# liudabao001/JABD-Joint-Attention-Based-Detector-for-small-face-detection

Hardware: AMD Instinct MI355X
Metric: images/sec at 1024x1024 bs32 (1/2/4/8 GPU); boxes/sec NMS (higher is better)
Workload: dtype fp32; 1 GPU; C2: JABD-MobileNetV3 RetinaFace (nets/retinaface_r.py) eval forward, weights_init weights; global_batch=32, image_size=1024, parallelism=replicas x1

## Files before the change

include/jabd.h:

```cpp
#ifndef JABD_H_
#define JABD_H_

#include <stddef.h>
#include <stdint.h>

#ifdef __cplusplus
extern "C" {
#endif

typedef void* jabd_stream_t;

enum {
  JABD_OK = 0,
  JABD_EINVAL = 1,
  JABD_EHIP = 2,
  JABD_EWS = 3,
};

const char* jabd_version(void);
int64_t jabd_abi_struct_size(int32_t which);
int jabd_last_error(char* buf, size_t len);

int jabd_launch_log_reset(void);
int64_t jabd_launch_log_count(void);
// ... 55 lines not shown
                          int64_t num_priors, float threshold, float var0,
                          float var1, float* loc_t, int64_t* conf_t,
                          float* landm_t, void* ws, size_t ws_bytes,
                          jabd_stream_t stream);

int jabd_match_iou_f32(const float* targets, const int64_t* offsets,
                       int64_t batch, int64_t max_gt, const float* priors,
                       int64_t num_priors, float threshold, float var0,
                       float var1, float* loc_t, int64_t* conf_t,
                       float* landm_t, void* ws, size_t ws_bytes,
                       jabd_stream_t stream);

int jabd_letterbox_f32(const float* src, int64_t batch, int ih, int iw,
                       float* dst, int h, int w, float fill,
                       const float* mean3, int nchw, jabd_stream_t stream);

int jabd_correct_boxes_f32(float* rows, int64_t n, int input_h, int input_w,
                           int image_h, int image_w, int letterbox,
                           int to_pixels, jabd_stream_t stream);

int jabd_augment_workspace_size(int ih, int nw, size_t* bytes);
int jabd_augment_u8(const uint8_t* src, int ih, int iw, int nw, int nh, int h,
                    int w, int dx, int dy, int flip, double hue, float sat,
                    float val, float* dst, void* ws, size_t ws_bytes,
                    jabd_stream_t stream);

int jabd_wider_eval_workspace_size(int64_t total_preds, int64_t total_gts,
                                   size_t* bytes);
int jabd_wider_eval_f64(const double* pred, const int64_t* pred_offsets,
                        const double* gt, const uint8_t* ignore,
                        const int64_t* gt_offsets, int64_t num_images,
                        int64_t total_preds, int64_t total_gts,
                        double iou_thresh, int thresh_num, double* pr_curve,
                        void* ws, size_t ws_bytes, jabd_stream_t stream);

int jabd_upsample_bicubic_ac_f32(const float* x, int64_t batch, int H, int W,
                                 int C, float* y, int OH, int OW,
                                 jabd_stream_t stream);
int jabd_upsample_bicubic_ac_bwd_f32(const float* grad_y, int64_t batch, int H,
                                     int W, int C, float* grad_x, int OH, int OW,
                                     jabd_stream_t stream);

int jabd_nlm_attn_fwd_f32(const float* q, const float* kp, const float* vp, int32_t B,
                          int32_t P, int32_t S, int32_t ch, float* ctx, float* lse,
                          jabd_stream_t stream);
int jabd_nlm_attn_bwd_f32(const float* q, const float* kp, const float* vp, const float* ctx,
                          const float* lse, const float* dctx, int32_t B, int32_t P, int32_t S,
                          int32_t ch, float* dq, float* pmat, float* dsmat,
                          jabd_stream_t stream);
int64_t jabd_nlm_attn_dkv_ws_floats(int32_t B, int32_t P, int32_t S, int32_t ch);
int jabd_nlm_attn_dkv_f32(const float* dsmat, const float* pmat, const float* q,
                          const float* dctx, int32_t B, int32_t P, int32_t S, int32_t ch,
                          float* ws, int64_t ws_floats, float* dk, float* dv,
                          jabd_stream_t stream);
int jabd_add3_f32(const float* a, const float* b, const float* c, int64_t n, float* y,
                  jabd_stream_t stream);

int64_t jabd_beca_ws_floats(int64_t batch, int64_t pixels, int C);
int jabd_beca_fwd_f32(const float* x, int64_t batch, int64_t pixels, int C,
                      const float* w, int k, float* y, float* stats, float* part,
                      int64_t part_floats, jabd_stream_t stream);
int jabd_beca_bwd_f32(const float* x, const float* grad_y, int64_t batch,
                      int64_t pixels, int C, const float* w, int k,
                      const float* stats, float* grad_x, float* grad_w, float* ws,
                      float* part, int64_t part_floats, jabd_stream_t stream);

int jabd_multibox_workspace_size(int64_t batch, int64_t num_priors, size_t* bytes);
int jabd_multibox_loss_fwd_f32(const float* loc, const float* conf,
                               const float* landm, const float* loc_t,
                               const int64_t* conf_t, const float* landm_t,
                               int64_t batch, int64_t num_priors, int neg_pos,
                               float* sums, int64_t* counts, uint8_t* sel,
                               void* ws, size_t ws_bytes, jabd_stream_t stream);
int jabd_multibox_loss_bwd_f32(const float* loc, const float* conf,
                               const float* landm, const float* loc_t,
                               const int64_t* conf_t, const float* landm_t,
                               const uint8_t* sel, int64_t batch,
                               int64_t num_priors, const float* gout,
                               const int64_t* counts,
                               float* grad_loc, float* grad_conf,
                               float* grad_landm, jabd_stream_t stream);
int jabd_multibox_diou_loss_fwd_f32(const float* loc, const float* conf,
                                    const float* landm, const float* loc_t,
                                    const int64_t* conf_t, const float* landm_t,
                                    const float* priors, float var0, float var1,
                                    int64_t batch, int64_t num_priors, int neg_pos,
                                    float* sums, int64_t* counts, uint8_t* sel,
                                    void* ws, size_t ws_bytes, jabd_stream_t stream);
int jabd_multibox_diou_loss_bwd_f32(const float* loc, const float* conf,
                                    const float* landm, const float* loc_t,
                                    const int64_t* conf_t, const float* landm_t,
                                    const float* priors, float var0, float var1,
                                    const uint8_t* sel, int64_t batch,
                                    int64_t num_priors, const float* gout,
                                    const int64_t* counts, float* grad_loc,
                                    float* grad_conf, float* grad_landm,
                                    jabd_stream_t stream);
int jabd_multibox_iou_loss_fwd_f32(const float* loc, const float* conf,
                                   const float* landm, const float* loc_t,
                                   const int64_t* conf_t, const float* landm_t,
                                   const float* priors, float var0, float var1,
                                   int64_t batch, int64_t num_priors, int neg_pos,
                                   float* sums, int64_t* counts, uint8_t* sel,
                                   void* ws, size_t ws_bytes, int32_t kind,
                                   jabd_stream_t stream);
int jabd_multibox_iou_loss_bwd_f32(const float* loc, const float* conf,
                                   const float* landm, const float* loc_t,
                                   const int64_t* conf_t, const float* landm_t,
                                   const float* priors, float var0, float var1,
                                   const uint8_t* sel, int64_t batch,
                                   int64_t num_priors, const float* gout,
                                   const int64_t* counts, float* grad_loc,
                                   float* grad_conf, float* grad_landm,
                                   int32_t kind, jabd_stream_t stream);
int jabd_iou_rows_fwd_f32(const float* pred, const float* priors,
                          const float* truth, int64_t n, float var0, float var1,
                          int32_t kind, float* val, jabd_stream_t stream);
int jabd_iou_rows_bwd_f32(const float* pred, const float* priors,
                          const float* truth, int64_t n, float var0, float var1,
                          int32_t kind, const float* gval, float* gpred,
                          jabd_stream_t stream);
int jabd_multibox_loss_finalize_f32(const float* sums, const int64_t* counts,
                                    float* loss, jabd_stream_t stream);

enum {
  JABD_ACT_NONE = 0,
  JABD_ACT_RELU = 1,
  JABD_ACT_LEAKY = 2,
  JABD_ACT_HSWISH = 3,
  JABD_ACT_HSIGMOID = 4,
  JABD_ACT_SIGMOID = 5,
};

typedef struct jabd_conv_args {
  const float* x; int64_t x_bs; int32_t x_ps, x_c0;
  int32_t B, H, W, Cin;
  const float* x2; int64_t x2_bs; int32_t x2_ps, Cin2;
  int32_t x2_W, x2_stride;
  const float* ascale; int64_t ascale_bs;
  const void* w; const float* bias;
  const float* res; int64_t res_bs; int32_t res_ps, res_c0;
  float* y; int64_t y_bs; int32_t y_ps, y_c0;
  int32_t OH, OW, Cout, Ntiles, tn, Kc;
  int32_t KH, KW, stride, pad;
  int32_t act; float slope;
  int32_t nchw_in, tconv;
  int32_t flags, reserved1;
  int64_t M;
  const void* w32; int32_t ntiles32, tn32;
  float* y2; int64_t y2_bs; int32_t y2_ps, y2_c0, nsplit, act2; float slope2; int32_t reserved2;
  void* ws; int64_t ws_bytes;
} jabd_conv_args;
int64_t jabd_conv_workspace_size(const jabd_conv_args* args);
int jabd_conv_pack_tn(int cout);
int jabd_conv_pack_tn32(int cout);
int jabd_conv_pack_f32(const float* w, int32_t cout, int32_t cin, int32_t kh, int32_t kw,
                       int32_t transposed, int32_t Kc, int32_t Ntiles, float* wp, int32_t K8,
                       int32_t NT32, float* wp32, jabd_stream_t stream);
int jabd_conv_pack_multi_f32(const int64_t* jobs, const int64_t* starts, int32_t njobs,
                             int64_t total, jabd_stream_t stream);
int jabd_conv2d_nhwc_f32(const jabd_conv_args* args, jabd_stream_t stream);
int64_t jabd_conv1x1_bn_stats_nblk(const jabd_conv_args* args);
int64_t jabd_conv_bn_bwd_part_floats(const jabd_conv_args* args);
int jabd_conv_bn_bwd_sums_f32(const jabd_conv_args* args, const float* x, int32_t x_ps,
                              const float* mean, const float* invstd, const float* gamma,
                              const float* beta, int32_t act, float slope, float* part,
                              int64_t part_floats, jabd_stream_t stream);
int jabd_conv_bn_bwd_sums_res_f32(const jabd_conv_args* args, const float* x, int32_t x_ps,
                                  const float* mask, int32_t mask_ps, const float* mean,
                                  const float* invstd, float* part, int64_t part_floats,
                                  jabd_stream_t stream);
int jabd_bn_act_bwd_rows_f32(float* part, const float* dy, const float* x, int64_t M,
                             int32_t C, const float* mean, const float* invstd,
                             const float* gamma, const float* beta, int32_t act, float slope,
                             float* dgamma, float* dbeta, float* dx, jabd_stream_t stream);
int64_t jabd_conv_bn_stats_part_floats(const jabd_conv_args* args);
int jabd_conv_bn_stats_f32(const jabd_conv_args* args, float* part, int64_t part_floats,
                           float* mean, float* invstd, float* running_mean, float* running_var,
                           float momentum, float eps, jabd_stream_t stream);
int jabd_conv1x1_bn_stats_f32(const jabd_conv_args* args, float* part, int64_t nblk,
                              float* shift, jabd_stream_t stream);

int jabd_stem_nchw_f32(const float* x, int32_t B, int32_t H, int32_t W, const float* w,
                       const float* bias, int32_t act, float* y, jabd_stream_t stream);

typedef struct jabd_dw_args {
  const float* x; int64_t x_bs; int32_t x_ps, reserved0;
  int32_t B, H, W, C;
  const float* w; const float* bias;
  float* y; int64_t y_bs; int32_t y_ps, reserved1;
  int32_t OH, OW, k, stride, pad, act;
  float slope; int32_t nblk;
  float* part;
} jabd_dw_args;
int64_t jabd_dw_nblk(int64_t B, int64_t OH, int64_t OW, int64_t C);
int jabd_dwconv_nhwc_f32(const jabd_dw_args* args, jabd_stream_t stream);
int64_t jabd_dwconv_stats_nblk(int64_t B, int64_t OH, int64_t OW, int64_t C);
int jabd_dwconv_stats_f32(const jabd_dw_args* args, float* stats_part, float* shift,
                          jabd_stream_t stream);
int jabd_dwconv_bnin_stats_f32(const jabd_dw_args* args, const float* mean, const float* invstd,
                               const float* gamma, const float* beta, int32_t act, float slope,
                               float* stats_part, float* shift, jabd_stream_t stream);

typedef struct jabd_expdw_args {
  const float* x; int64_t x_bs; int32_t x_ps, Cin;
  int32_t B, H, W, E;
  const void* we; const float* be; int32_t Ntiles, Kc;
  const float* wd; const float* bd;
  int32_t k, stride, act, nblk;
  float* y; int64_t y_bs; int32_t y_ps, OH, OW, reserved0;
  float* part;
  const float* sw; const float* sb; float* sy; int64_t sy_bs; int32_t sy_ps, reserved1;
  const void* pw; const float* pb; const float* pg; const float* pres; int32_t pg_bs, pact;
} jabd_expdw_args;
int64_t jabd_expand_dw_nblk(int32_t OH, int32_t OW, int32_t k, int32_t stride);
int jabd_expand_dw_nhwc_f32(const jabd_expdw_args* args, jabd_stream_t stream);
int jabd_expand_dw_select(int32_t form);

int jabd_channel_sum_f32(const float* x, int64_t x_bs, int32_t x_ps, int64_t B, int64_t HW,
                         int64_t C, int64_t nblk, float* part, jabd_stream_t stream);
int jabd_partial_reduce_f32(const float* part, int64_t nblk, int64_t B, int64_t C, int64_t nsplit,
                            float* out, jabd_stream_t stream);
int jabd_eca_gate_f32(const float* part, int64_t nblk, int64_t B, int64_t C, int64_t hw,
                      const float* w1d, int32_t k, int32_t gate, float* scale, float* mean_out,
                      jabd_stream_t stream);

int jabd_nlm_pool_f32(const float* src, int64_t src_bs, int32_t src_ps, int32_t B, int32_t hs,
                      int32_t ws, int32_t C, int32_t h, int32_t w, const float* wk,
                      const float* bk, const float* wv, const float* bv, int32_t ch,
                      const int32_t* sizes, int32_t nsizes, float* kpool, float* vpool,
                      float* kv_ws, jabd_stream_t stream);
int jabd_nlm_apply_f32(const float* src, int64_t src_bs, int32_t src_ps, int32_t B, int32_t hs,
                       int32_t ws, int32_t C, int32_t h, int32_t w, const float* wq,
                       const float* bq, const float* kpool, const float* vpool, int32_t S,
                       int32_t ch, const float* wW, const float* bW, const float* lateral,
                       float* out, float* q_out, float* ctx_out, jabd_stream_t stream);

int jabd_maxpool_nhwc_f32(const float* x, int32_t B, int32_t H, int32_t W, int32_t C,
                          int32_t k, int32_t stride, int32_t pad, float* y,
                          jabd_stream_t stream);
int64_t jabd_ssh_tail_weight_floats(void);
int jabd_ssh_tail_heads_f32(const float* c33, int64_t c33_bs, int32_t c33_ps, const float* t,
                            int64_t t_bs, int32_t B, int32_t H, int32_t W, const float* wb,
                            float leaky, int64_t A, int64_t a_off, int32_t softmax, float* loc,
                            float* conf, float* landm, jabd_stream_t stream);
int jabd_heads_f32(const float* x, int64_t x_bs, int32_t x_ps, int32_t B, int32_t HW,
                   int32_t C, const float* wt, const float* bias, int64_t A, int64_t a_off,
                   int32_t softmax, float* loc, float* conf, float* landm,
                   jabd_stream_t stream);
int jabd_heads_scatter_f32(const float* y, int32_t B, int64_t HW, int64_t A, int64_t a_off,
                           int32_t softmax, float* loc, float* conf, float* landm,
                           jabd_stream_t stream);

#define JABD_WINDOW_MAX 32
typedef struct jabd_window_copy {
  const float* src;
  float* dst;
  int32_t s0, s1, s2;
  int32_t d0, d1, d2;
  int32_t off2;
  float fill;
  float scale;
  int32_t reserved;
} jabd_window_copy;
int jabd_window_copy_multi_f32(int32_t n, const jabd_window_copy* descs, jabd_stream_t stream);
int jabd_transpose_f32(const float* src, int32_t rows, int32_t cols, float* dst,
                       jabd_stream_t stream);
int jabd_colsum_f32(const float* part, int64_t rows, int32_t C, float* out,
                    jabd_stream_t stream);
#define JABD_SUM_MAX 8
int jabd_sum_multi_f32(int32_t n_in, const float* const* in, int64_t n, float* out,
                       jabd_stream_t stream);
int jabd_weighted_sum3_f32(const float* a, const float* b, const float* c, float wa, float* out,
                           jabd_stream_t stream);
int jabd_conv_w2d_f32(const float* w, int32_t cout, int32_t cin, int32_t taps, float* out,
                      jabd_stream_t stream);
int jabd_heads_wpack_f32(float* wb, float* wc, float* wl, const float* bb, const float* bc,
                         const float* bl, int32_t C, int32_t half, int32_t q, int32_t qp,
                         float* wt, int32_t Cf, float* bias, int32_t dir, jabd_stream_t stream);

int64_t jabd_bn_nblk(int64_t M, int32_t C);
int jabd_bn_stats_final_f32(const float* shift, const float* part, int64_t nblk, int64_t M,
                            int32_t C, float* mean, float* invstd, float* running_mean,
                            float* running_var, float momentum, float eps, jabd_stream_t stream);
int jabd_bn_stats_f32(const float* x, int32_t ldx, int64_t M, int32_t C, float* part,
                      float* mean, float* invstd, float* running_mean, float* running_var,
                      float momentum, float eps, jabd_stream_t stream);
int jabd_bn_act_fwd_f32(const float* x, int32_t ldx, int64_t M, int32_t C, const float* mean,
                        const float* invstd, const float* gamma, const float* beta,
                        const float* res, int32_t ldr, int32_t act, float slope, float* y,
                        int32_t ldy, int32_t yc0, jabd_stream_t stream);
int jabd_bn_act_bwd_f32(const float* dy, int32_t lddy, int32_t dyc0, const float* x, int32_t ldx,
                        const float* res, int32_t ldr, int64_t M, int32_t C, const float* mean,
                        const float* invstd, const float* gamma, const float* beta, int32_t act,
                        float slope, float* part, float* dgamma, float* dbeta, float* dx,
                        float* dres, jabd_stream_t stream);
int64_t jabd_bn_sum_nblk(int64_t hw, int32_t C);
int jabd_bn_act_fwd_sum_f32(const float* x, int64_t M, int32_t C, const float* mean,
                            const float* invstd, const float* gamma, const float* beta,
                            int32_t act, float slope, float* y, int64_t hw, float* part,
                            jabd_stream_t stream);
int jabd_bn_act_bwd_ex_f32(const float* dy, int32_t lddy, int32_t dyc0, const float* x,
                           int32_t ldx, const float* res, int32_t ldr, int64_t M, int32_t C,
                           const float* mean, const float* invstd, const float* gamma,
                           const float* beta, int32_t act, float slope, const float* dys,
                           const float* dya, int64_t hw, float* part, float* dgamma,
// ... 102 lines not shown
```

jabd-joint-attention-based-detector-for-small-face-detection_amd/csrc/abi.cpp:

```cpp
#include <string.h>

#include "common.h"

namespace jabd {
static thread_local char g_err[512] = {0};

void set_error(const char* fmt, ...) {
  va_list ap;
  va_start(ap, fmt);
  vsnprintf(g_err, sizeof(g_err), fmt, ap);
  va_end(ap);
}

thread_local LaunchLog g_launch_log = {};
}

extern "C" int jabd_launch_log_reset(void) {
  jabd::g_launch_log.count = 0;
  return JABD_OK;
}

extern "C" int64_t jabd_launch_log_count(void) { return jabd::g_launch_log.count; }

static bool launch_log_kept(int32_t i) {
  const int64_t n = jabd::g_launch_log.count;
  return i >= 0 && i < n && i >= n - jabd::kLaunchLogCap;
}

extern "C" const char* jabd_launch_log_name(int32_t i) {
  return launch_log_kept(i) ? jabd::g_launch_log.name[i & (jabd::kLaunchLogCap - 1)] : nullptr;
}

extern "C" int jabd_launch_log_tag(int32_t i) {
  return launch_log_kept(i) ? jabd::g_launch_log.tag[i & (jabd::kLaunchLogCap - 1)] : 0;
}

extern "C" const char* jabd_version(void) { return "jabd-mi355x 0.1.0 (gfx950)"; }

extern "C" int jabd_last_error(char* buf, size_t len) {
  if (!buf || len == 0) return JABD_EINVAL;
  strncpy(buf, jabd::g_err, len - 1);
  buf[len - 1] = 0;
  return JABD_OK;
}

extern "C" int64_t jabd_abi_struct_size(int32_t which) {
  switch (which) {
    case 0: return (int64_t)sizeof(jabd_conv_args);
    case 1: return (int64_t)sizeof(jabd_dw_args);
    case 2: return (int64_t)sizeof(jabd_expdw_args);
    case 3: return (int64_t)sizeof(jabd_window_copy);
    default: return -1;
  }
}
```

jabd-joint-attention-based-detector-for-small-face-detection_amd/csrc/conv.hip:

```cpp
#include <limits.h>
#include <stdlib.h>

#include <algorithm>

#include "common.h"
#include "conv_args.h"

namespace jabd {

typedef float f32x4 __attribute__((ext_vector_type(4)));

__device__ __forceinline__ float act_apply(float v, int act, float slope) {
  switch (act) {
    case ACT_RELU: return relu_f(v);
    case ACT_LEAKY: return v > 0.f ? v : v * slope;
    case ACT_HSWISH: return hswish_f(v);
    case ACT_HSIGMOID: return hsigmoid_f(v);
    case ACT_SIGMOID: return 1.f / (1.f + expf(-v));
    default: return v;
  }
}

__device__ __forceinline__ void wave_lds_sync() {
  asm volatile("s_waitcnt lgkmcnt(0)" ::: "memory");
// ... 504 lines not shown
  constexpr int LDW = 16 * TN + 4;
  float* sm = c3_lds + wave * 16 * LDW;
#pragma unroll
  for (int t = 0; t < TM; ++t) {
    const int oh = oh0 + wave * TM + t, ow = ow0 + j;
    const bool pv = oh < p.OH && ow < p.OW;
#pragma unroll
    for (int u = 0; u < TN; ++u)
      *reinterpret_cast<f32x4*>(sm + j * LDW + 16 * u + 4 * g) = acc[t][u];
    const int64_t pix = (int64_t)oh * p.OW + ow;
    const long long yoff = pv ? (long long)((int64_t)b * p.y_bs + pix * p.y_ps + p.y_c0) : -1;
    const long long y2off = p.y2 ? (long long)((int64_t)b * p.y2_bs + pix * p.y2_ps + p.y2_c0) : 0;
    wave_lds_sync();
#pragma unroll
    for (int f0 = 0; f0 < 16 * 4 * TN; f0 += 64) {
      const int f = f0 + lane;
      const int q = f / (4 * TN), c4 = f - q * (4 * TN);
      const long long yo = __shfl(yoff, q);
      const long long y2o = __shfl(y2off, q);
      const int n0 = nb * TN * 16 + 4 * c4;
      if (yo >= 0 && n0 < p.Cout) {
        float4 v = *reinterpret_cast<const float4*>(sm + q * LDW + 4 * c4);
        if (p.bias) {
          const float4 bb = *reinterpret_cast<const float4*>(p.bias + n0);
          v.x += bb.x; v.y += bb.y; v.z += bb.z; v.w += bb.w;
        }
        if (p.y2 && n0 >= p.nsplit) {
          v.x = act_apply(v.x, p.act2, p.slope2);
          v.y = act_apply(v.y, p.act2, p.slope2);
          v.z = act_apply(v.z, p.act2, p.slope2);
          v.w = act_apply(v.w, p.act2, p.slope2);
          *reinterpret_cast<float4*>(p.y2 + y2o + (n0 - p.nsplit)) = v;
        } else {
          v.x = act_apply(v.x, p.act, p.slope);
          v.y = act_apply(v.y, p.act, p.slope);
          v.z = act_apply(v.z, p.act, p.slope);
          v.w = act_apply(v.w, p.act, p.slope);
          *reinterpret_cast<float4*>(p.y + yo + n0) = v;
        }
      }
    }
    wave_lds_sync();
  }
}

static size_t conv3x3_lds(const ConvArgs& a, int tm) {
  const size_t lds_in = (size_t)(4 * tm + 2) * k3IC * (a.Cin + 4) * sizeof(float);
  const size_t lds_epi = (size_t)4 * 16 * (16 * a.tn + 4) * sizeof(float);
  return std::max(lds_in, lds_epi);
}

static bool conv3x3_tile_pick(const ConvLayer& L, int& tm) {
  static const int on = env_digit("JABD_CONV3X3_TILE", 1);
  static const int rows = env_digit("JABD_CONV3X3_TM") == 4 ? 4 : 2;
  const ConvArgs& a = L.a;
  if (on == 0 || (on == 2 && a.tconv)) return false;
  if (L.is1x1 || a.KH != 3 || a.KW != 3 || a.stride != 1 || a.pad != 1 || a.nchw_in || a.x2 ||
      a.res || !L.vec4 || !L.v4out || a.Cin > 64 || a.tn > 3 || (a.ascale && a.ascale_bs % 4))
    return false;
  tm = rows;
  if (tm == 4 && (int64_t)a.B * cdiv(a.OH, 16) * cdiv(a.OW, k3Cols) < 1024) tm = 2;
  return conv3x3_lds(a, tm) <= 64 * 1024;
}

static int launch_conv3x3_tile(const ConvArgs& a, int tm, hipStream_t st) {
  const int tn = a.tn;
  const int rows = 4 * tm;
  const int tiles_w = (int)cdiv(a.OW, k3Cols), tiles_h = (int)cdiv(a.OH, rows);
  const int tiles_img = tiles_w * tiles_h;
  const int64_t grid = (int64_t)a.B * tiles_img * (a.Ntiles / tn);
  JABD_REQUIRE(grid < (int64_t)0x7fffffff, "conv3x3: grid too large");
  const size_t lds = conv3x3_lds(a, tm);
#define C3_CASE(TN_, TM_)                                                                    \
  if (tn == TN_ && tm == TM_) {                                                              \
    conv3x3_tile_kernel<TN_, TM_><<<(unsigned)grid, 256, lds, st>>>(a, tiles_w, tiles_img);  \
    return check_launch("conv3x3_tile", 100 * TM_ + TN_);                                    \
  }
  C3_CASE(1, 2) C3_CASE(2, 2) C3_CASE(3, 2) C3_CASE(1, 4) C3_CASE(2, 4) C3_CASE(3, 4)
#undef C3_CASE
  return -1;
}

template <int TM, int TN>
static int launch_1x1(const ConvArgs& a, hipStream_t st) {
  const int64_t grid = cdiv(a.M, (int64_t)4 * 16 * TM) * (a.Ntiles / TN);
  JABD_REQUIRE(grid < (int64_t)0x7fffffff, "conv: grid too large");
  const int x2 = !a.x2 ? 0 : (a.x2_stride == 1 ? 1 : 2);
  const bool as = a.ascale != nullptr;
#define C1_CASE(X2_, AS_)                                                    \
  if (x2 == X2_ && as == AS_) {                                              \
    conv1x1_kernel<TM, TN, X2_, AS_><<<(unsigned)grid, 256, 0, st>>>(a);     \
    return check_launch("conv1x1", 100 * TM + TN);                           \
  }
  C1_CASE(0, false) C1_CASE(0, true) C1_CASE(1, false) C1_CASE(1, true)
  C1_CASE(2, false) C1_CASE(2, true)
#undef C1_CASE
  return JABD_EINVAL;
}

template <int TM, int TN>
static int launch_conv(const ConvArgs& a, bool vec4, hipStream_t st) {
  const int64_t rows_per_blk = 4 * 16 * TM;
  const int64_t mblk = cdiv(a.M, rows_per_blk);
  const int64_t nblk = a.Ntiles / TN;
  const int64_t grid = mblk * nblk;
  JABD_REQUIRE(grid < (int64_t)0x7fffffff, "conv: grid too large");
  if (vec4)
    conv_gemm_kernel<TM, TN, true><<<(unsigned)grid, 256, 0, st>>>(a);
  else
    conv_gemm_kernel<TM, TN, false><<<(unsigned)grid, 256, 0, st>>>(a);
  return check_launch("conv_gemm", 100 * TM + TN);
}

}

using namespace jabd;

namespace jabd {
template <bool FAST>
static int dispatch_conv(const ConvArgs& a, int tn, int tm, bool vec4, hipStream_t st) {
#define DC(TM_, TN_)                                                         \
  if (tm == TM_ && tn == TN_)                                                \
    return FAST ? launch_1x1<TM_, TN_>(a, st) : launch_conv<TM_, TN_>(a, vec4, st);
  DC(4, 1) DC(2, 1) DC(1, 1) DC(4, 2) DC(2, 2) DC(1, 2) DC(4, 3) DC(2, 3) DC(1, 3)
  DC(4, 4) DC(2, 4) DC(1, 4) DC(4, 5) DC(2, 5) DC(1, 5) DC(2, 8) DC(1, 8)
#undef DC
  return -1;
}
}

extern "C" int jabd_conv_pack_tn(int cout) {
  int tiles = (cout + 15) / 16;
  if (tiles <= 5) return tiles;
  int best = 4, waste = 1 << 30;
  for (int tn : {4, 5, 8}) {
    int grp = (tiles + tn - 1) / tn;
    int w = grp * tn - tiles;
    if (w < waste || (w == waste && tn > best)) { waste = w; best = tn; }
  }
  return best;
}

static bool conv_generic_only() {
  static const bool v = env_digit("JABD_CONV_GENERIC") == 1;
  return v;
}

namespace jabd {
bool stem7_ok(const ConvArgs& a);
int stem7_fwd_launch(const ConvArgs& a, hipStream_t st);
bool m32s_pick(const ConvLayer& L, int form, int& TN, int& KS);
bool m32_tile_pick(const ConvLayer& L, int& tm, int& tn, int& ks);
int conv_m32s_launch(const ConvLayer& L, const ConvRoute& r, hipStream_t st);
int conv_m32_tile_launch(const ConvLayer& L, const ConvRoute& r, hipStream_t st);
int64_t conv_m32_ksplit_bytes(const ConvArgs& a, int ks);
int conv_m32_stats_dispatch(const ConvLayer& L, bool kxk, float* part, const BnEpi& bb,
                            hipStream_t st);
int64_t bn_rows_sum_doubles(int64_t M, int C);
int64_t bn_rows_chunk_doubles(int64_t M, int C);
int bn_rows_final_launch(const float* rows, int ldc, int64_t M, int C, double* chunks,
                         float* mean, float* invstd, float* rmean, float* rvar, float momentum,
                         float eps, hipStream_t st);
bool conv1x1_stream_serves(const ConvArgs& a, bool stats);
int conv1x1_stream_dispatch(const ConvArgs& a, hipStream_t st, StreamStats* ss = nullptr);
}

static bool use_conv32(const ConvLayer& L) {
  static const int v = env_digit("JABD_CONV32");
  const ConvArgs& a = L.a;
  if (!L.w32(1, INT_MAX)) return false;
  if (v == 0 || v == 1) return v == 1;
  if (L.is1x1 && !a.x2 && !a.ascale && !a.y2 && !a.tconv && (a.Cin == 64 || a.Cin == 128) &&
      a.Cout >= 64)
    return true;
  if (a.KH * a.KW > 1) return a.Cout >= 64 && L.Ktot >= 288;
  return a.Cout >= 96 && L.Ktot >= 96;
}

static int conv_setup(const jabd_conv_args* args, ConvLayer& L) {
  JABD_REQUIRE(args, "conv: null args");
  ConvArgs& a = L.a;
  a = *args;
  JABD_REQUIRE(a.x && a.w && a.y, "conv: null pointer");
  JABD_REQUIRE(a.B > 0 && a.Cin > 0 && a.Cout > 0 && a.KH > 0 && a.KW > 0 && a.stride > 0,
               "conv: bad shape");
  if (a.tconv) {
    JABD_REQUIRE(a.H == (a.OH + 2 * a.pad - a.KH) / a.stride + 1 &&
                     a.W == (a.OW + 2 * a.pad - a.KW) / a.stride + 1 && !a.nchw_in && !a.x2,
                 "conv: transposed-conv size mismatch");
  } else {
    JABD_REQUIRE(a.OH == (a.H + 2 * a.pad - a.KH) / a.stride + 1 &&
                     a.OW == (a.W + 2 * a.pad - a.KW) / a.stride + 1,
                 "conv: output size mismatch");
  }
  L.is1x1 = a.KH == 1 && a.KW == 1 && a.stride == 1 && a.pad == 0;
  JABD_REQUIRE(!a.y2 || (a.nsplit > 0 && a.nsplit % 4 == 0 && a.nsplit < a.Cout &&
                         a.y2_ps % 4 == 0 && a.y2_c0 % 4 == 0 && a.y2_bs % 4 == 0 &&
                         (reinterpret_cast<uintptr_t>(a.y2) & 15) == 0 && !a.res && !a.tconv),
               "conv: split output needs nsplit %% 4 == 0, 16-byte aligned y2, no residual");
  JABD_REQUIRE(!a.x2 || ((a.KH * a.KW * a.Cin) % 4 == 0 && a.Cin2 % 4 == 0 && a.x2_ps % 4 == 0 &&
                         a.x2_stride > 0 && !a.nchw_in),
               "conv: K-concat needs K and Cin2 multiples of 4");
  L.Ktot = a.KH * a.KW * a.Cin + (a.x2 ? a.Cin2 : 0);
  JABD_REQUIRE(a.Kc == (L.Ktot + 15) / 16, "conv: Kc=%d, expected %d", a.Kc, (L.Ktot + 15) / 16);
  const int tiles = (a.Cout + 15) / 16;
  JABD_REQUIRE(a.Ntiles >= tiles, "conv: Ntiles=%d < %d", a.Ntiles, tiles);
  a.M = (int64_t)a.B * a.OH * a.OW;
  JABD_REQUIRE(a.M < (int64_t)0x7fffffff, "conv: B*OH*OW must be < 2^31");
  {
    const uintptr_t al = reinterpret_cast<uintptr_t>(a.y) | reinterpret_cast<uintptr_t>(a.bias) |
                         reinterpret_cast<uintptr_t>(a.res);
    L.v4out = a.Cout % 4 == 0 && a.y_ps % 4 == 0 && a.y_c0 % 4 == 0 && a.y_bs % 4 == 0 &&
              (!a.res || (a.res_ps % 4 == 0 && a.res_c0 % 4 == 0 && a.res_bs % 4 == 0)) &&
              (al & 15) == 0;
    a.flags = L.v4out ? 1 : 0;
    JABD_REQUIRE(!a.y2 || L.v4out, "conv: split output needs the vector epilogue layout");
  }
  L.vec4 = !a.nchw_in && a.Cin % 4 == 0 && a.x_ps % 4 == 0 && a.x_c0 % 4 == 0 &&
           (reinterpret_cast<uintptr_t>(a.x) & 15) == 0;
  JABD_REQUIRE(a.tn > 0 && a.Ntiles % a.tn == 0, "conv: Ntiles %% tn != 0");
  const int64_t OHW = L.OHW = (int64_t)a.OH * a.OW;
  L.rows_contig = a.y_bs == OHW * a.y_ps && (!a.res || a.res_bs == OHW * a.res_ps);
  const int64_t maxps = std::max<int64_t>(std::max<int64_t>(a.x_ps, a.y_ps),
                                          std::max<int64_t>(a.res ? a.res_ps : 0,
                                                            a.x2 ? a.x2_ps : 0));
  L.fast1x1 =
      L.is1x1 && !a.tconv && L.vec4 && L.v4out && !a.y2 && a.x_bs == OHW * a.x_ps &&
      L.rows_contig && (!a.ascale || a.ascale_bs % 4 == 0) &&
      (!a.x2 || (a.x2_stride == 1 ? (a.x2_W == a.OW && a.x2_bs == OHW * a.x2_ps)
                                  : (a.x2_stride > 1 && a.x2_bs % a.x2_ps == 0 &&
                                     a.x2_bs * a.B < ((int64_t)1 << 31)))) &&
      (a.M + 64) * (maxps + 16) < ((int64_t)1 << 31) && !conv_generic_only();
  return 0;
}

static int conv_generic_tm(const ConvLayer& L) {
  const ConvArgs& a = L.a;
  const int tn = a.tn;
  const int64_t nblk_n = a.Ntiles / tn;
  auto grid_for = [&](int tm) { return cdiv(a.M, (int64_t)64 * tm) * nblk_n; };
  const int K = L.Ktot;
  const int tm_max = tn == 8 ? 2 : (K <= 32 ? 2 : (K <= 160 ? 1 : (K <= 400 ? 2 : 4)));
  int tm = tm_max;
  while (tm > 1 && grid_for(tm) < 1024) tm >>= 1;
  static const int ftm = (int)env_int("JABD_CONV_TM", 0);
  if (ftm == 1 || ftm == 2 || (ftm == 4 && tn != 8)) tm = ftm;
  return tm;
}

static ConvRoute conv_route(const ConvLayer& L) {
  const ConvArgs& a = L.a;
  ConvRoute r{kFamGemm, 0, a.tn, 1};
  static const bool stem7_on = env_digit("JABD_STEM7") != 0;
  if (stem7_on && stem7_ok(a) && L.v4out && (a.act == ACT_NONE || a.act == ACT_RELU) &&
      a.Ntiles >= 4 && !conv_generic_only()) {
    r.family = kFamStem7;
    return r;
  }
  if (use_conv32(L)) {
    if (L.fast1x1 && m32s_pick(L, 0, r.tn, r.ks)) {
      r.family = kFamM32Stream;
      return r;
    }
    if (m32_tile_pick(L, r.tm, r.tn, r.ks)) {
      r.family = L.is1x1 ? kFamM32Tile : kFamM32Kxk;
      return r;
    }
    r = ConvRoute{kFamGemm, 0, a.tn, 1};
  }
  if (L.fast1x1 && !a.reserved1 && conv1x1_stream_serves(a, false)) {
    r.family = kFamStream;
    return r;
  }
  if (conv3x3_tile_pick(L, r.tm)) {
    r.family = kFamTile3x3;
    return r;
  }
  r.tm = conv_generic_tm(L);
  r.family = L.fast1x1 ? kFamConv1x1 : kFamGemm;
  return r;
}

extern "C" int64_t jabd_conv_workspace_size(const jabd_conv_args* args) {
  ConvLayer L;
  if (!args || conv_setup(args, L) != JABD_OK) return 0;
  const ConvRoute r = conv_route(L);
  const bool tile = r.family == kFamM32Tile || r.family == kFamM32Kxk;
  return tile ? conv_m32_ksplit_bytes(L.a, r.ks) : 0;
}

static bool conv_stats_form(const ConvLayer& L) {
  const ConvArgs& a = L.a;
  return !a.ascale && !a.x2 && !a.res && conv_route(L).family == kFamStream &&
         conv1x1_stream_serves(a, true);
}

extern "C" int64_t jabd_conv1x1_bn_stats_nblk(const jabd_conv_args* args) {
  ConvLayer L;
  if (conv_setup(args, L) != JABD_OK || !conv_stats_form(L)) return 0;
  jabd::StreamStats ss{nullptr, nullptr, 0, true};
  if (jabd::conv1x1_stream_dispatch(L.a, nullptr, &ss) != 0) return 0;
  return ss.nblk;
}

extern "C" int jabd_conv1x1_bn_stats_f32(const jabd_conv_args* args, float* part, int64_t nblk,
                                         float* shift, jabd_stream_t stream) {
  ConvLayer L;
  if (const int e = conv_setup(args, L)) return e;
  JABD_REQUIRE(conv_stats_form(L),
               "conv1x1_bn_stats: layer not served by the streaming statistics form");
  jabd::StreamStats ss{part, shift, nblk, false};
  const int r = jabd::conv1x1_stream_dispatch(L.a, as_stream(stream), &ss);
  JABD_REQUIRE(r >= 0, "conv1x1_bn_stats: no streaming kernel for this shape");
  return r;
}

static bool conv_m32_epi_form(const ConvLayer& L, bool kxk) {
  const ConvArgs& a = L.a;
  if (conv_generic_only() || a.bias || a.ascale || a.x2 || a.y2 || a.act != ACT_NONE ||
      a.nchw_in || !L.v4out || !L.w32(1, 4))
    return false;
  return kxk ? L.kxk32() : L.fast1x1;
}

static bool conv_m32_stats_form(const ConvLayer& L, bool& kxk) {
  static const bool on = env_digit("JABD_CONV_STATS32") != 0;
  kxk = !L.is1x1;
  return on && !L.a.res && !L.a.tconv && L.a.Cout % 4 == 0 && conv_m32_epi_form(L, kxk);
}

static int64_t conv_stats_rows_floats(const ConvArgs& a) {
  return (cdiv(a.M, (int64_t)32) * 2 * a.ntiles32 * 32 + 1) & ~(int64_t)1;
}
static int64_t conv_stats_part_floats(const ConvArgs& a) {
  return conv_stats_rows_floats(a) + 2 * bn_rows_chunk_doubles(a.M, a.Cout);
}

extern "C" int64_t jabd_conv_bn_stats_part_floats(const jabd_conv_args* args) {
  ConvLayer L;
  bool kxk = false;
  if (conv_setup(args, L) != JABD_OK || !conv_m32_stats_form(L, kxk)) return 0;
  return conv_stats_part_floats(L.a);
}

extern "C" int jabd_conv_bn_stats_f32(const jabd_conv_args* args, float* part, int64_t part_floats,
                                      float* mean, float* invstd, float* running_mean,
                                      float* running_var, float momentum, float eps,
                                      jabd_stream_t stream) {
  ConvLayer L;
  bool kxk = false;
  if (const int e = conv_setup(args, L)) return e;
  const ConvArgs& a = L.a;
  JABD_REQUIRE(conv_m32_stats_form(L, kxk),
               "conv_bn_stats: layer not served by the 32x32 statistics form");
  JABD_REQUIRE(part && mean && invstd && part_floats >= conv_stats_part_floats(a),
               "conv_bn_stats: part holds %lld floats, %lld needed", (long long)part_floats,
               (long long)conv_stats_part_floats(a));
  JABD_REQUIRE(((uintptr_t)part & 15) == 0, "conv_bn_stats: part must be 16-byte aligned");
  hipStream_t st = as_stream(stream);
  const int r = conv_m32_stats_dispatch(L, kxk, part, BnEpi{}, st);
  if (r != JABD_OK) return r < 0 ? JABD_EINVAL : r;
  return bn_rows_final_launch(part, a.ntiles32 * 32, a.M, a.Cout,
                              reinterpret_cast<double*>(part + conv_stats_rows_floats(a)), mean,
                              invstd, running_mean, running_var, momentum, eps, st);
}

static bool conv_m32_bb_form(const ConvLayer& L, bool with_res, bool& kxk) {
  static const bool on = env_digit("JABD_CONV_BNBWD32") != 0;
  const ConvArgs& a = L.a;
  kxk = !(L.is1x1 && !a.tconv);
  if (!on || (with_res ? kxk : a.res != nullptr) || a.Cout % 32 || a.ntiles32 * 32 != a.Cout ||
      (a.tconv && a.stride != 1))
    return false;
  return conv_m32_epi_form(L, kxk);
}

static int64_t conv_bb_part_floats(const ConvArgs& a) {
  return cdiv(a.M, (int64_t)32) * 2 * a.Cout + 2 * bn_rows_sum_doubles(a.M, a.Cout);
}

static int conv_bb_check(const ConvLayer& L, bool with_res, const char* who, const float* part,
                         int64_t part_floats, bool& kxk) {
  JABD_REQUIRE(conv_m32_bb_form(L, with_res, kxk),
               "%s: layer not served by the 32x32 BatchNorm-backward form%s", who,
               with_res ? " (1x1 / stride-1 only)" : "");
  const int64_t need = conv_bb_part_floats(L.a);
  JABD_REQUIRE(part && part_floats >= need && ((uintptr_t)part & 15) == 0,
               "%s: part holds %lld floats, %lld needed (16-byte aligned)", who,
               (long long)part_floats, (long long)need);
  return JABD_OK;
}

extern "C" int64_t jabd_conv_bn_bwd_part_floats(const jabd_conv_args* args) {
  ConvLayer L;
  bool kxk = false;
  if (conv_setup(args, L) != JABD_OK || !conv_m32_bb_form(L, false, kxk)) return 0;
  return conv_bb_part_floats(L.a);
}

extern "C" int jabd_conv_bn_bwd_sums_f32(const jabd_conv_args* args, const float* x, int32_t x_ps,
                                         const float* mean, const float* invstd,
                                         const float* gamma, const float* beta, int32_t act,
                                         float slope, float* part, int64_t part_floats,
                                         jabd_stream_t stream) {
  ConvLayer L;
  bool kxk = false;
  if (const int e = conv_setup(args, L)) return e;
  if (const int e = conv_bb_check(L, false, "conv_bn_bwd_sums", part, part_floats, kxk)) return e;
  JABD_REQUIRE(x && mean && invstd && gamma && beta && x_ps % 4 == 0 && x_ps >= L.a.Cout &&
                   (act == ACT_NONE || act == ACT_RELU || act == ACT_LEAKY),
               "conv_bn_bwd_sums: bad BatchNorm arguments");
  BnEpi bb{x, mean, invstd, gamma, beta, part, x_ps, act, slope};
  const int r = conv_m32_stats_dispatch(L, kxk, nullptr, bb, as_stream(stream));
  return r < 0 ? JABD_EINVAL : r;
}

extern "C" int jabd_conv_bn_bwd_sums_res_f32(const jabd_conv_args* args, const float* x,
                                             int32_t x_ps, const float* mask, int32_t mask_ps,
                                             const float* mean, const float* invstd, float* part,
                                             int64_t part_floats, jabd_stream_t stream) {
  ConvLayer L;
  bool kxk = false;
  if (const int e = conv_setup(args, L)) return e;
  if (const int e = conv_bb_check(L, true, "conv_bn_bwd_sums_res", part, part_floats, kxk))
    return e;
  JABD_REQUIRE(x && mask && mean && invstd && x_ps % 4 == 0 && x_ps >= L.a.Cout &&
                   mask_ps % 4 == 0 && mask_ps >= L.a.Cout,
               "conv_bn_bwd_sums_res: bad BatchNorm arguments");
  BnEpi bb{x, mean, invstd, nullptr, nullptr, part, x_ps, ACT_NONE, 0.f, mask, mask_ps};
  const int r = conv_m32_stats_dispatch(L, false, nullptr, bb, as_stream(stream));
  return r < 0 ? JABD_EINVAL : r;
}

extern "C" int jabd_conv2d_nhwc_f32(const jabd_conv_args* args, jabd_stream_t stream) {
  ConvLayer L;
  if (const int e = conv_setup(args, L)) return e;
  const ConvArgs& a = L.a;
  hipStream_t st = as_stream(stream);
  ConvRoute r = conv_route(L);
  int e = -1;
  switch (r.family) {
    case kFamStem7: return stem7_fwd_launch(a, st);
    case kFamM32Stream: e = conv_m32s_launch(L, r, st); break;
    case kFamM32Tile:
    case kFamM32Kxk: e = conv_m32_tile_launch(L, r, st); break;
    case kFamStream: e = conv1x1_stream_dispatch(a, st); break;
    case kFamTile3x3: e = launch_conv3x3_tile(a, r.tm, st); break;
    case kFamConv1x1:
    case kFamGemm: break;
  }
  if (e >= 0) return e;
  if (r.family != kFamConv1x1 && r.family != kFamGemm) r.tm = conv_generic_tm(L);
  e = L.fast1x1 ? dispatch_conv<true>(a, a.tn, r.tm, L.vec4, st) : -1;
  if (e < 0) e = dispatch_conv<false>(a, a.tn, r.tm, L.vec4, st);
  if (e >= 0) return e;
  set_error("conv: unsupported tn=%d", a.tn);
  return JABD_EINVAL;
}

namespace jabd {
constexpr int kStemOut = 16;
constexpr int kStemThreads = 128;
#ifndef STEM_ROWS
#define STEM_ROWS 2
#endif
constexpr int kStemRows = STEM_ROWS;

template <int ACT>
__global__ __launch_bounds__(kStemThreads) void stem_kernel(const float* __restrict__ x, int H,
                                                            int W, int OH, int OW,
                                                            const float* __restrict__ w,
                                                            const float* __restrict__ bias,
                                                            float* __restrict__ y) {
  __shared__ float4 st[kStemThreads / 64][64 * kStemOut / 4 + 64 / 8];
  const int b = blockIdx.z, oh0 = blockIdx.y * kStemRows;
  const int lane = threadIdx.x & 63, wave = threadIdx.x >> 6;
  const int ow0 = blockIdx.x * kStemThreads + wave * 64;
  const int ow = ow0 + lane;
  const bool pv = ow < OW;
  const float* xb = x + (int64_t)b * 3 * H * W;
  const int64_t HW = (int64_t)H * W;
  constexpr int IR = 2 * kStemRows + 1;
  float v[IR][9];
#pragma unroll
  for (int r = 0; r < IR; ++r) {
    const int ih = 2 * oh0 - 1 + r;
#pragma unroll
    for (int kw = 0; kw < 3; ++kw) {
      const int iw = 2 * ow - 1 + kw;
      const bool ok = pv && ih >= 0 && ih < H && iw >= 0 && iw < W;
      const float* xp = xb + (ok ? (int64_t)ih * W + iw : 0);
#pragma unroll
      for (int ci = 0; ci < 3; ++ci) {
        const float t = xp[ci * HW];
        v[r][kw * 3 + ci] = ok ? t : 0.f;
      }
    }
  }
  auto f = [](float u) {
    return ACT == ACT_HSWISH ? hswish_f(u) : ACT == ACT_RELU ? relu_f(u) : u;
  };
  float4* sw = st[wave];
#pragma unroll
  for (int ro = 0; ro < kStemRows; ++ro) {
    const int oh = oh0 + ro;
    if (oh >= OH) break;
    float o[kStemOut];
#pragma unroll
    for (int n = 0; n < kStemOut; ++n) o[n] = bias[n];
#pragma unroll
    for (int tp = 0; tp < 27; ++tp) {
      asm volatile("" ::: "memory");
      const float* wr = w + tp * kStemOut;
      const float xv = v[2 * ro + tp / 9][tp % 9];
#pragma unroll
      for (int n = 0; n < kStemOut; ++n) o[n] = fmaf(wr[n], xv, o[n]);
    }
#pragma unroll
    for (int q = 0; q < kStemOut / 4; ++q)
      sw[4 * lane + (lane >> 3) + q] =
          make_float4(f(o[4 * q]), f(o[4 * q + 1]), f(o[4 * q + 2]), f(o[4 * q + 3]));
    asm volatile("s_waitcnt lgkmcnt(0)" ::: "memory");
    float4* yw = reinterpret_cast<float4*>(y + (((int64_t)b * OH + oh) * OW + ow0) * kStemOut);
    const int npx = min(64, OW - ow0);
#pragma unroll
    for (int q = 0; q < kStemOut / 4; ++q) {
      const int i = q * 64 + lane;
      const int p = i >> 2;
      if (p < npx) yw[i] = sw[i + (p >> 3)];
    }
    asm volatile("s_waitcnt lgkmcnt(0)" ::: "memory");
  }
}
}

extern "C" int jabd_stem_nchw_f32(const float* x, int32_t B, int32_t H, int32_t W,
                                  const float* w, const float* bias, int32_t act, float* y,
                                  jabd_stream_t stream) {
  JABD_REQUIRE(x && w && bias && y && B > 0 && H > 0 && W > 0, "stem: bad args");
  const int OH = (H + 2 - 3) / 2 + 1, OW = (W + 2 - 3) / 2 + 1;
  dim3 g((unsigned)cdiv(OW, kStemThreads), (unsigned)cdiv(OH, kStemRows), (unsigned)B);
  JABD_REQUIRE(act == ACT_HSWISH || act == ACT_RELU || act == ACT_NONE, "stem: act %d", act);
  hipStream_t st = as_stream(stream);
  if (act == ACT_HSWISH)
    stem_kernel<ACT_HSWISH><<<g, kStemThreads, 0, st>>>(x, H, W, OH, OW, w, bias, y);
  else if (act == ACT_RELU)
    stem_kernel<ACT_RELU><<<g, kStemThreads, 0, st>>>(x, H, W, OH, OW, w, bias, y);
  else
    stem_kernel<ACT_NONE><<<g, kStemThreads, 0, st>>>(x, H, W, OH, OW, w, bias, y);
  return check_launch("stem");
}
```

jabd-joint-attention-based-detector-for-small-face-detection_amd/csrc/conv32.hip:

```cpp
#include <stdlib.h>

#include <algorithm>
#include <type_traits>

#include "common.h"
#include "conv_args.h"

namespace jabd {

typedef float f32x16 __attribute__((ext_vector_type(16)));

__device__ __forceinline__ float act32(float v, int act, float slope) {
  switch (act) {
    case ACT_RELU: return relu_f(v);
    case ACT_LEAKY: return v > 0.f ? v : v * slope;
    case ACT_HSWISH: return hswish_f(v);
    case ACT_HSIGMOID: return hsigmoid_f(v);
    case ACT_SIGMOID: return 1.f / (1.f + expf(-v));
    default: return v;
  }
}

constexpr int kBK = 32;

__device__ __forceinline__ void wave_lds_sync32() {
  asm volatile("s_waitcnt lgkmcnt(0)" ::: "memory");
  __builtin_amdgcn_wave_barrier();
}
constexpr int kG = kBK / 8;
constexpr int kGateLds = 1024;

constexpr int kEpiPitch = 36;
enum { kEpiRt = 0, kEpiNone = 1, kEpiRes = 2 };
template <int TN, bool ST, bool BB, int EPI = kEpiRt>
__device__ __forceinline__ void m32_epilogue_tm1(const ConvArgs& p, const f32x16 (&acc)[TN],
                                                 int pm, int om, int nb, int srow, float* ep,
                                                 float* __restrict__ part, const BnEpi& bb,
                                                 int lane, int ch0 = 0) {
  const bool has_bias = EPI == kEpiRt && p.bias;
  const bool has_res = EPI == kEpiRes || (EPI == kEpiRt && p.res);
  const int h = lane >> 5, j = lane & 31;
  const int ep_px = lane >> 3, ep_q = lane & 7;
  int mrow[4], prow[4];
#pragma unroll
  for (int r = 0; r < 4; ++r) {
    prow[r] = __shfl(pm, ep_px + 8 * r);
    mrow[r] = __shfl(om, ep_px + 8 * r);
  }
#pragma unroll
  for (int u = 0; u < TN; ++u) {
    const int nb0 = (nb * TN + u) * 32 + ch0;
    if (nb0 >= p.Cout) break;
    const int n = nb0 + 4 * ep_q;
    float4 ss = make_float4(0.f, 0.f, 0.f, 0.f), sq = ss, sh = ss;
    float4 bmu = sh, bis = sh, bgm = sh, bbt = sh;
    float4 bx[4], bmk[4];
    if constexpr (BB) {
      if (n < p.Cout) {
        bmu = *reinterpret_cast<const float4*>(bb.mean + n);
        bis = *reinterpret_cast<const float4*>(bb.invstd + n);
        if (!bb.mask) {
          bgm = *reinterpret_cast<const float4*>(bb.gamma + n);
          bbt = *reinterpret_cast<const float4*>(bb.beta + n);
        }
      }
#pragma unroll
      for (int r = 0; r < 4; ++r)
        bx[r] = (prow[r] >= 0 && n < p.Cout)
                    ? *reinterpret_cast<const float4*>(bb.x + (int64_t)mrow[r] * bb.x_ps + n)
                    : sh;
      if (bb.mask) {
#pragma unroll
        for (int r = 0; r < 4; ++r)
          bmk[r] = (prow[r] >= 0 && n < p.Cout)
                       ? *reinterpret_cast<const float4*>(bb.mask + (int64_t)mrow[r] * bb.mask_ps + n)
                       : sh;
      }
    }
#pragma unroll
    for (int c = 0; c < 4; ++c)
      *reinterpret_cast<float4*>(ep + j * kEpiPitch + 8 * c + 4 * h) =
          make_float4(acc[u][4 * c], acc[u][4 * c + 1], acc[u][4 * c + 2],
                      acc[u][4 * c + 3]);
    wave_lds_sync32();
    if constexpr (ST) sh = *reinterpret_cast<const float4*>(ep + 4 * ep_q);
#pragma unroll
    for (int r = 0; r < 4; ++r) {
      const int px = ep_px + 8 * r;
      if (prow[r] < 0 || n >= p.Cout) continue;
      float4 v = *reinterpret_cast<const float4*>(ep + px * kEpiPitch + 4 * ep_q);
      if (BB && bb.mask) {
        if (p.res) {
          const float4 rr = *reinterpret_cast<const float4*>(p.res + (int64_t)mrow[r] * p.res_ps +
                                                             p.res_c0 + n);
          v.x += rr.x; v.y += rr.y; v.z += rr.z; v.w += rr.w;
        }
        v.x *= bmk[r].x > 0.f ? 1.f : 0.f;
        v.y *= bmk[r].y > 0.f ? 1.f : 0.f;
        v.z *= bmk[r].z > 0.f ? 1.f : 0.f;
        v.w *= bmk[r].w > 0.f ? 1.f : 0.f;
        const float xh0 = (bx[r].x - bmu.x) * bis.x, xh1 = (bx[r].y - bmu.y) * bis.y;
        const float xh2 = (bx[r].z - bmu.z) * bis.z, xh3 = (bx[r].w - bmu.w) * bis.w;
        ss.x += v.x; ss.y += v.y; ss.z += v.z; ss.w += v.w;
        sq.x += v.x * xh0; sq.y += v.y * xh1; sq.z += v.z * xh2; sq.w += v.w * xh3;
        *reinterpret_cast<float4*>(p.y + (int64_t)mrow[r] * p.y_ps + p.y_c0 + n) = v;
        continue;
      }
      if constexpr (BB) {
        const float xv[4] = {bx[r].x, bx[r].y, bx[r].z, bx[r].w};
        const float mu[4] = {bmu.x, bmu.y, bmu.z, bmu.w}, is[4] = {bis.x, bis.y, bis.z, bis.w};
        const float gm[4] = {bgm.x, bgm.y, bgm.z, bgm.w}, bt[4] = {bbt.x, bbt.y, bbt.z, bbt.w};
        const float gv[4] = {v.x, v.y, v.z, v.w};
        float dzs[4], dzx[4];
#pragma unroll
        for (int e = 0; e < 4; ++e) {
          const float xh = (xv[e] - mu[e]) * is[e];
          const float z = fmaf(xh, gm[e], bt[e]);
          const float d = bb.act == ACT_RELU ? (z > 0.f ? 1.f : 0.f)
                          : bb.act == ACT_LEAKY ? (z > 0.f ? 1.f : bb.slope) : 1.f;
          dzs[e] = gv[e] * d;
          dzx[e] = dzs[e] * xh;
        }
        ss.x += dzs[0]; ss.y += dzs[1]; ss.z += dzs[2]; ss.w += dzs[3];
        sq.x += dzx[0]; sq.y += dzx[1]; sq.z += dzx[2]; sq.w += dzx[3];
      }
      if constexpr (ST) {
        const float dx = v.x - sh.x, dy = v.y - sh.y, dz = v.z - sh.z, dw = v.w - sh.w;
        ss.x += dx; ss.y += dy; ss.z += dz; ss.w += dw;
        sq.x = fmaf(dx, dx, sq.x); sq.y = fmaf(dy, dy, sq.y);
        sq.z = fmaf(dz, dz, sq.z); sq.w = fmaf(dw, dw, sq.w);
      }
      if (has_bias) {
        const float4 bb = *reinterpret_cast<const float4*>(p.bias + n);
        v.x += bb.x; v.y += bb.y; v.z += bb.z; v.w += bb.w;
      }
      if (has_res) {
        const float4 rr = *reinterpret_cast<const float4*>(p.res + (int64_t)mrow[r] * p.res_ps +
                                                           p.res_c0 + n);
        v.x += rr.x; v.y += rr.y; v.z += rr.z; v.w += rr.w;
      }
      if constexpr (EPI == kEpiRt) {
        v.x = act32(v.x, p.act, p.slope);
        v.y = act32(v.y, p.act, p.slope);
        v.z = act32(v.z, p.act, p.slope);
        v.w = act32(v.w, p.act, p.slope);
      }
      *reinterpret_cast<float4*>(p.y + (int64_t)mrow[r] * p.y_ps + p.y_c0 + n) = v;
    }
    if constexpr (BB) {
#pragma unroll
      for (int off = 8; off <= 32; off <<= 1) {
        ss.x += __shfl_xor(ss.x, off); ss.y += __shfl_xor(ss.y, off);
        ss.z += __shfl_xor(ss.z, off); ss.w += __shfl_xor(ss.w, off);
        sq.x += __shfl_xor(sq.x, off); sq.y += __shfl_xor(sq.y, off);
        sq.z += __shfl_xor(sq.z, off); sq.w += __shfl_xor(sq.w, off);
      }
      if (ep_px == 0 && (int64_t)srow * 32 < p.M && n < p.Cout) {
        const int ldc = p.Ntiles * 32;
        float* pr = bb.rows + (int64_t)srow * 2 * ldc + n;
// ... 84 lines not shown
  if constexpr (KXK) {
#pragma unroll
    for (int t = 0; t < TM; ++t) {
      const int m = pm[t] >= 0 ? pm[t] : 0;
      const int SHW = SH * SW;
      const int b = m / SHW, r = m - b * SHW;
      const int i = r / SW, jj = r - i * SW;
      poh[t] = phase >= 0 ? 2 * i + ph : i;
      pow_[t] = phase >= 0 ? 2 * jj + pw : jj;
      pbase[t] = (int64_t)b * p.x_bs + p.x_c0;
      if (pm[t] >= 0) om[t] = (b * p.OH + poh[t]) * p.OW + pow_[t];
    }
  }
  const int cps = p.Cin / kBK;
  const int x2_pix = (p.x2 && p.x2_stride != 1) ? (int)(p.x2_bs / p.x2_ps) : 0;
  const float4* wg = reinterpret_cast<const float4*>(p.w);
  const float* sc = AS ? p.ascale + (int64_t)img * p.ascale_bs : nullptr;

  const float* xa[TM];
  const float* xb[TM];
  if constexpr (FAST) {
#pragma unroll
    for (int t = 0; t < TM; ++t) {
      const int ml = pm[t] >= 0 ? pm[t] : m_lo;
      xa[t] = p.x + (int64_t)ml * p.x_ps + p.x_c0;
      xb[t] = SRC == kSrcTwo ? p.x2 + (int64_t)ml * p.x2_ps - p.Cin : xa[t];
    }
  }
  auto load_a = [&](int s, float4 (&a)[TM][kG]) {
    if constexpr (FAST) {
#pragma unroll
      for (int t = 0; t < TM; ++t)
#pragma unroll
        for (int q = 0; q < kG; ++q) {
          const int k4 = min(s * kBK + 8 * q + 4 * h, Kt - 4);
          const float* src = (SRC == kSrcTwo && k4 >= p.Cin) ? xb[t] + k4 : xa[t] + k4;
          a[t][q] = *reinterpret_cast<const float4*>(src);
        }
      return;
    }
    if constexpr (KXK) {
      const int tl = s / cps, ci0 = (s - tl * cps) * kBK;
      const int khi = tl / nkw;
      const int kh = kh0 + (phase >= 0 ? 2 : 1) * khi;
      const int kw = kw0 + (phase >= 0 ? 2 : 1) * (tl - khi * nkw);
#pragma unroll
      for (int t = 0; t < TM; ++t) {
        const int ih = p.tconv ? (poh[t] + p.pad - kh) >> (phase >= 0 ? 1 : 0)
                               : poh[t] * p.stride - p.pad + kh;
        const int iw = p.tconv ? (pow_[t] + p.pad - kw) >> (phase >= 0 ? 1 : 0)
                               : pow_[t] * p.stride - p.pad + kw;
        const bool ok = pm[t] >= 0 && ih >= 0 && ih < p.H && iw >= 0 && iw < p.W;
        const float* src = p.x + pbase[t] + ((int64_t)ih * p.W + iw) * p.x_ps + ci0 + 4 * h;
#pragma unroll
        for (int q = 0; q < kG; ++q)
          a[t][q] = ok ? *reinterpret_cast<const float4*>(src + 8 * q)
                       : make_float4(0.f, 0.f, 0.f, 0.f);
      }
      return;
    }
#pragma unroll
    for (int t = 0; t < TM; ++t)
#pragma unroll
      for (int q = 0; q < kG; ++q) {
        const int k4 = s * kBK + 8 * q + 4 * h;
        const int m = pm[t];
        float4 r = make_float4(0.f, 0.f, 0.f, 0.f);
        if (m >= 0) {
          if (k4 < p.Cin) {
            r = *reinterpret_cast<const float4*>(p.x + (int64_t)m * p.x_ps + p.x_c0 + k4);
          } else if (k4 < Kt) {
            int qq = m;
            if (p.x2_stride != 1) {
              const int b = m / OHW, rr = m - b * OHW;
              const int oh = rr / p.OW, ow = rr - oh * p.OW;
              qq = b * x2_pix + (oh * p.x2_stride) * p.x2_W + ow * p.x2_stride;
            }
            r = *reinterpret_cast<const float4*>(p.x2 + (int64_t)qq * p.x2_ps + (k4 - p.Cin));
          }
        }
        a[t][q] = r;
      }
  };
  const bool gate_lds = FAST || (AS && p.Cin <= kGateLds);
  auto zero_tail = [&](int s, float4 (&a)[TM][kG]) {
    if (!FAST || (s + 1) * kBK <= Kt) return;
#pragma unroll
    for (int t = 0; t < TM; ++t)
#pragma unroll
      for (int q = 0; q < kG; ++q)
        if (s * kBK + 8 * q + 4 * h >= Kt) a[t][q] = make_float4(0.f, 0.f, 0.f, 0.f);
  };
  auto load_b = [&](int s, float4 (&b)[NBT]) {
    if (KXK && phase >= 0) {
      const int tl = s / cps, khi = tl / nkw;
      const int tap = (kh0 + 2 * khi) * p.KW + kw0 + 2 * (tl - khi * nkw);
      s = tap * cps + (s - tl * cps);
    }
#pragma unroll
    for (int i = 0; i < NBT; ++i) {
      const int f = i * 256 + threadIdx.x;
      float4 v = make_float4(0.f, 0.f, 0.f, 0.f);
      if (f < NB4) {
        const int g = f / (TN * 64), rem = f - g * (TN * 64);
        const int u = rem >> 6, l = rem & 63;
        const int k8 = s * kG + g;
        v = wg[((int64_t)k8 * p.Ntiles + nb * TN + u) * 64 + l];
        if (!FAST && sc && !gate_lds) {
          int k0 = 8 * k8 + 4 * (l >> 5);
          if (KXK) k0 -= (s / cps) * p.Cin;
          if (k0 < p.Cin) {
            const float4 s4 = *reinterpret_cast<const float4*>(sc + k0);
            v.x *= s4.x; v.y *= s4.y; v.z *= s4.z; v.w *= s4.w;
          }
        }
      }
      b[i] = v;
    }
  };
  auto store_b = [&](int buf, int s, const float4 (&b)[NBT]) {
    if (KXK && phase >= 0) {
      const int tl = s / cps, khi = tl / nkw;
      const int tap = (kh0 + 2 * khi) * p.KW + kw0 + 2 * (tl - khi * nkw);
      s = tap * cps + (s - tl * cps);
    }
#pragma unroll
    for (int i = 0; i < NBT; ++i) {
      const int f = i * 256 + threadIdx.x;
      if (f < NB4) {
        float4 v = b[i];
        if (gate_lds) {
          const int g = f / (TN * 64), l = f & 63;
          int k0 = 8 * (s * kG + g) + 4 * (l >> 5);
          if (KXK) k0 -= (s / cps) * p.Cin;
          if (k0 < p.Cin) {
            const float4 s4 = *reinterpret_cast<const float4*>(sGate + k0);
            v.x *= s4.x; v.y *= s4.y; v.z *= s4.z; v.w *= s4.w;
          }
        }
        sB[buf][f] = v;
      }
    }
  };

  f32x16 acc[TM][TN];
#pragma unroll
  for (int t = 0; t < TM; ++t)
#pragma unroll
    for (int u = 0; u < TN; ++u)
#pragma unroll
      for (int r = 0; r < 16; ++r) acc[t][u][r] = 0.f;

  float4 a_cur[TM][kG], a_nxt[TM][kG], b_nxt[NBT];
  if (gate_lds) {
    for (int i = threadIdx.x; i < p.Cin; i += 256) sGate[i] = sc[i];
    __syncthreads();
  }
  if (S > s_beg) {
    load_a(s_beg, a_cur);
    load_b(s_beg, b_nxt);
    store_b(s_beg & 1, s_beg, b_nxt);
    zero_tail(s_beg, a_cur);
  }
  __syncthreads();
  for (int s = s_beg; s < S; ++s) {
    const bool more = s + 1 < S;
    if (more) {
      load_a(s + 1, a_nxt);
      load_b(s + 1, b_nxt);
    }
    const float4* bs = sB[s & 1];
#pragma unroll
    for (int q = 0; q < kG; ++q) {
      float4 bw[TN];
#pragma unroll
      for (int u = 0; u < TN; ++u) bw[u] = bs[(q * TN + u) * 64 + lane];
#pragma unroll
      for (int t = 0; t < TM; ++t)
#pragma unroll
        for (int u = 0; u < TN; ++u)
          acc[t][u] = __builtin_amdgcn_mfma_f32_32x32x2f32(bw[u].x, a_cur[t][q].x, acc[t][u], 0, 0, 0);
#pragma unroll
      for (int t = 0; t < TM; ++t)
#pragma unroll
        for (int u = 0; u < TN; ++u)
          acc[t][u] = __builtin_amdgcn_mfma_f32_32x32x2f32(bw[u].y, a_cur[t][q].y, acc[t][u], 0, 0, 0);
#pragma unroll
      for (int t = 0; t < TM; ++t)
#pragma unroll
        for (int u = 0; u < TN; ++u)
          acc[t][u] = __builtin_amdgcn_mfma_f32_32x32x2f32(bw[u].z, a_cur[t][q].z, acc[t][u], 0, 0, 0);
#pragma unroll
      for (int t = 0; t < TM; ++t)
#pragma unroll
        for (int u = 0; u < TN; ++u)
          acc[t][u] = __builtin_amdgcn_mfma_f32_32x32x2f32(bw[u].w, a_cur[t][q].w, acc[t][u], 0, 0, 0);
    }
    if (more) {
      store_b((s + 1) & 1, s + 1, b_nxt);
#pragma unroll
      for (int t = 0; t < TM; ++t)
#pragma unroll
        for (int q = 0; q < kG; ++q) a_cur[t][q] = a_nxt[t][q];
      zero_tail(s + 1, a_cur);
    }
    __syncthreads();
  }

  if (ks > 1) {
    const int npad = p.Ntiles * 32;
    float* pb = part + (int64_t)blockIdx.y * p.M * npad;
#pragma unroll
    for (int t = 0; t < TM; ++t) {
      if (pm[t] < 0) continue;
      float* prow = pb + (int64_t)om[t] * npad;
#pragma unroll
      for (int u = 0; u < TN; ++u)
#pragma unroll
        for (int c = 0; c < 4; ++c) {
          const int n = (nb * TN + u) * 32 + 8 * c + 4 * h;
          *reinterpret_cast<float4*>(prow + n) = make_float4(
              acc[t][u][4 * c], acc[t][u][4 * c + 1], acc[t][u][4 * c + 2], acc[t][u][4 * c + 3]);
        }
    }
    return;
  }
  if constexpr (TM == 1) {
    float* ep = reinterpret_cast<float*>(sB_) + wave * 32 * kEpiPitch;
    const int srow = mb * 4 + wave;
    m32_epilogue_tm1<TN, ST, BB, (ST || BB) ? kEpiNone : EPI>(p, acc[0], pm[0], om[0], nb, srow,
                                                                ep, part, bb, lane);
    return;
  }
#pragma unroll
  for (int t = 0; t < TM; ++t) {
    const int m = om[t];
    if (pm[t] < 0) continue;
    float* yrow = p.y + (int64_t)m * p.y_ps + p.y_c0;
    const float* rrow = p.res ? p.res + (int64_t)m * p.res_ps + p.res_c0 : nullptr;
#pragma unroll
    for (int u = 0; u < TN; ++u)
#pragma unroll
      for (int c = 0; c < 4; ++c) {
        const int n = (nb * TN + u) * 32 + 8 * c + 4 * h;
        if (n >= p.Cout) continue;
        float4 v = make_float4(acc[t][u][4 * c], acc[t][u][4 * c + 1], acc[t][u][4 * c + 2],
                               acc[t][u][4 * c + 3]);
        if (p.bias) {
          const float4 bb = *reinterpret_cast<const float4*>(p.bias + n);
          v.x += bb.x; v.y += bb.y; v.z += bb.z; v.w += bb.w;
        }
        if (rrow) {
          const float4 rr = *reinterpret_cast<const float4*>(rrow + n);
          v.x += rr.x; v.y += rr.y; v.z += rr.z; v.w += rr.w;
        }
        v.x = act32(v.x, p.act, p.slope);
        v.y = act32(v.y, p.act, p.slope);
        v.z = act32(v.z, p.act, p.slope);
        v.w = act32(v.w, p.act, p.slope);
        *reinterpret_cast<float4*>(yrow + n) = v;
      }
  }

}

__global__ __launch_bounds__(256) void m32_ksplit_reduce(const ConvArgs p, int ks,
                                                         const float* __restrict__ part) {
  const int npad = p.Ntiles * 32, c4n = (p.Cout + 3) >> 2;
  const int64_t i = blockIdx.x * (int64_t)blockDim.x + threadIdx.x;
  if (i >= p.M * c4n) return;
  const int64_t m = i / c4n;
  const int n = (int)(i - m * c4n) * 4;
  float4 v = *reinterpret_cast<const float4*>(part + m * npad + n);
  for (int y = 1; y < ks; ++y) {
    const float4 q = *reinterpret_cast<const float4*>(part + ((int64_t)y * p.M + m) * npad + n);
    v.x += q.x; v.y += q.y; v.z += q.z; v.w += q.w;
  }
  if (p.bias) {
    const float4 bb = *reinterpret_cast<const float4*>(p.bias + n);
    v.x += bb.x; v.y += bb.y; v.z += bb.z; v.w += bb.w;
  }
  if (p.res) {
    const float4 rr = *reinterpret_cast<const float4*>(p.res + m * p.res_ps + p.res_c0 + n);
    v.x += rr.x; v.y += rr.y; v.z += rr.z; v.w += rr.w;
  }
  v.x = act32(v.x, p.act, p.slope);
  v.y = act32(v.y, p.act, p.slope);
  v.z = act32(v.z, p.act, p.slope);
  v.w = act32(v.w, p.act, p.slope);
  *reinterpret_cast<float4*>(p.y + m * p.y_ps + p.y_c0 + n) = v;
}

template <int TN, bool AS, bool X2>
__global__ __launch_bounds__(512) void conv1x1_m32w8_kernel(const ConvArgs p, int mtiles_img,
                                                            int per_img) {
  constexpr int TNL = (TN + 1) / 2, TNH = TN - TNL;
  constexpr int NB4 = kG * TN * 64;
  constexpr int NBT = (NB4 + 511) / 512;
  constexpr int kEpi4 = 8 * 32 * kEpiPitch / 4;
  constexpr int SB4 = kEpi4 > 2 * NB4 ? kEpi4 : 2 * NB4;
  __shared__ float4 sB_[SB4];
  float4 (*sB)[NB4] = reinterpret_cast<float4 (*)[NB4]>(sB_);
  __shared__ __attribute__((aligned(16))) float sGate[AS ? kGateLds : 4];
  const int lane = threadIdx.x & 63;
  const int wave = __builtin_amdgcn_readfirstlane(threadIdx.x >> 6);
  const int row = wave & 3, half = wave >> 2;
  const int h = lane >> 5, j = lane & 31;
  const int nblk_n = p.Ntiles / TN;
  const int bid = blockIdx.x;
  const int nb = bid % nblk_n, mb = bid / nblk_n;
  const int OHW = p.OH * p.OW;
  int img = 0, m_lo, m_hi;
  if (per_img) {
    img = mb / mtiles_img;
    m_lo = img * OHW + (mb - img * mtiles_img) * 128;
    m_hi = min(img * OHW + OHW, (int)p.M);
  } else {
    m_lo = mb * 128;
    m_hi = (int)p.M;
  }
  const int m = m_lo + row * 32 + j;
  const int pm = m < m_hi ? m : -1;
  const int ml = pm >= 0 ? m : m_lo;
  const int Kt = p.Cin + (X2 ? p.Cin2 : 0);
  const int S = (Kt + kBK - 1) / kBK;
  const float4* wg = reinterpret_cast<const float4*>(p.w) + (int64_t)nb * TN * 64;
  const float* xa = p.x + (int64_t)ml * p.x_ps + p.x_c0;
  const float* xb = X2 ? p.x2 + (int64_t)ml * p.x2_ps - p.Cin : xa;

  auto load_a = [&](int s, float4 (&a)[kG]) {
#pragma unroll
    for (int q = 0; q < kG; ++q) {
      const int k4 = min(s * kBK + 8 * q + 4 * h, Kt - 4);
      const float* src = (X2 && k4 >= p.Cin) ? xb + k4 : xa + k4;
      a[q] = *reinterpret_cast<const float4*>(src);
    }
  };
  auto load_b = [&](int s, float4 (&b)[NBT]) {
#pragma unroll
    for (int i = 0; i < NBT; ++i) {
      const int f = i * 512 + threadIdx.x;
      if ((i + 1) * 512 <= NB4 || wave < (NB4 - i * 512) / 64) {
        const int g = f / (TN * 64), rem = f - g * (TN * 64);
        b[i] = wg[(int64_t)(s * kG + g) * p.Ntiles * 64 + rem];
      }
    }
  };
  auto store_b = [&](int buf, int s, const float4 (&b)[NBT]) {
#pragma unroll
    for (int i = 0; i < NBT; ++i) {
      const int f = i * 512 + threadIdx.x;
      if ((i + 1) * 512 <= NB4 || wave < (NB4 - i * 512) / 64) {
        float4 v = b[i];
        if constexpr (AS) {
          const int g = f / (TN * 64), l = f & 63;
          const int k0 = 8 * (s * kG + g) + 4 * (l >> 5);
          if (k0 < p.Cin) {
            const float4 s4 = *reinterpret_cast<const float4*>(sGate + k0);
            v.x *= s4.x; v.y *= s4.y; v.z *= s4.z; v.w *= s4.w;
          }
        }
        sB[buf][f] = v;
      }
    }
  };

  f32x16 acc[TNL];
#pragma unroll
  for (int u = 0; u < TNL; ++u)
#pragma unroll
    for (int r = 0; r < 16; ++r) acc[u][r] = 0.f;

  float4 a_cur[kG], a_nxt[kG], b_nxt[NBT];
  load_a(0, a_cur);
  load_b(0, b_nxt);
  if constexpr (AS) {
    const float* sc = p.ascale + (int64_t)img * p.ascale_bs;
    for (int i = threadIdx.x; i < p.Cin; i += 512) sGate[i] = sc[i];
    __syncthreads();
  }
  store_b(0, 0, b_nxt);
  auto zero_tail = [&](int s, float4 (&a)[kG]) {
    if ((s + 1) * kBK <= Kt) return;
#pragma unroll
    for (int q = 0; q < kG; ++q)
      if (s * kBK + 8 * q + 4 * h >= Kt) a[q] = make_float4(0.f, 0.f, 0.f, 0.f);
  };
  zero_tail(0, a_cur);
  __syncthreads();
  for (int s = 0; s < S; ++s) {
    const bool more = s + 1 < S;
    if (more) {
      load_a(s + 1, a_nxt);
      load_b(s + 1, b_nxt);
    }
    const float4* bs = sB[s & 1];
    auto mma = [&](auto nu_, auto u0_) {
      constexpr int NU = decltype(nu_)::value, U0 = decltype(u0_)::value;
#pragma unroll
      for (int q = 0; q < kG; ++q) {
        float4 bw[NU];
#pragma unroll
        for (int u = 0; u < NU; ++u) bw[u] = bs[(q * TN + U0 + u) * 64 + lane];
#pragma unroll
        for (int u = 0; u < NU; ++u)
          acc[u] = __builtin_amdgcn_mfma_f32_32x32x2f32(bw[u].x, a_cur[q].x, acc[u], 0, 0, 0);
#pragma unroll
        for (int u = 0; u < NU; ++u)
          acc[u] = __builtin_amdgcn_mfma_f32_32x32x2f32(bw[u].y, a_cur[q].y, acc[u], 0, 0, 0);
#pragma unroll
        for (int u = 0; u < NU; ++u)
          acc[u] = __builtin_amdgcn_mfma_f32_32x32x2f32(bw[u].z, a_cur[q].z, acc[u], 0, 0, 0);
#pragma unroll
        for (int u = 0; u < NU; ++u)
          acc[u] = __builtin_amdgcn_mfma_f32_32x32x2f32(bw[u].w, a_cur[q].w, acc[u], 0, 0, 0);
      }
    };
    if (half == 0)
      mma(std::integral_constant<int, TNL>{}, std::integral_constant<int, 0>{});
    else
      mma(std::integral_constant<int, TNH>{}, std::integral_constant<int, TNL>{});
    if (more) {
      store_b((s + 1) & 1, s + 1, b_nxt);
#pragma unroll
      for (int q = 0; q < kG; ++q) a_cur[q] = a_nxt[q];
      zero_tail(s + 1, a_cur);
    }
    __syncthreads();
  }

  float* ep = reinterpret_cast<float*>(sB_) + wave * 32 * kEpiPitch;
  if (half == 0)
    m32_epilogue_tm1<TNL, false, false, kEpiRt>(
        p, reinterpret_cast<const f32x16(&)[TNL]>(acc), pm, pm, 0, 0, ep, nullptr, BnEpi{}, lane,
        nb * TN * 32);
  else
    m32_epilogue_tm1<TNH, false, false, kEpiRt>(
        p, reinterpret_cast<const f32x16(&)[TNH]>(acc), pm, pm, 0, 0, ep, nullptr, BnEpi{}, lane,
        (nb * TN + TNL) * 32);
}

template <int TN, int KS, bool ST, bool BB, int EPI>
__global__ __launch_bounds__(256) void conv1x1_m32s_kernel(const ConvArgs p, int nblk_n,
                                                            float* __restrict__ part,
                                                            const BnEpi bb) {
  constexpr int NW4 = KS * kG * TN * 64;
  extern __shared__ __attribute__((aligned(16))) float4 m32s_lds[];
  const int lane = threadIdx.x & 63;
  const int wave = __builtin_amdgcn_readfirstlane(threadIdx.x >> 6);
  const int h = lane >> 5, j = lane & 31;
  const int xcd = blockIdx.x & 7, rr = blockIdx.x >> 3;
  const int nb = rr % nblk_n, wgm = (rr / nblk_n) * 8 + xcd;
  const int gm = gridDim.x / nblk_n;
  {
    const float4* wg = reinterpret_cast<const float4*>(p.w);
    for (int f = threadIdx.x; f < NW4; f += 256) {
      const int k8 = f / (TN * 64), rem = f - k8 * (TN * 64);
      m32s_lds[f] = wg[((int64_t)k8 * p.Ntiles + nb * TN + (rem >> 6)) * 64 + (rem & 63)];
    }
  }
  __syncthreads();
  float* ep = reinterpret_cast<float*>(m32s_lds + NW4) + wave * 32 * kEpiPitch;
  const int64_t ntiles = (p.M + 31) >> 5;
  const int64_t step = (int64_t)gm * 4;
  const float* xb = p.x + p.x_c0 + 4 * h;
  auto load = [&](int64_t T, int s, int q) {
    const int64_t m = T * 32 + j;
    return m < p.M ? *reinterpret_cast<const float4*>(xb + m * p.x_ps + s * kBK + 8 * q)
                   : make_float4(0.f, 0.f, 0.f, 0.f);
  };
  float4 a[KS][kG];
  int64_t T = (int64_t)wgm * 4 + wave;
#pragma unroll
  for (int s = 0; s < KS; ++s)
#pragma unroll
    for (int q = 0; q < kG; ++q) a[s][q] = load(T, s, q);
  for (; T < ntiles; T += step) {
    const int64_t Tn = T + step;
    f32x16 acc[TN];
#pragma unroll
    for (int u = 0; u < TN; ++u)
#pragma unroll
      for (int r = 0; r < 16; ++r) acc[u][r] = 0.f;
#pragma unroll
    for (int s = 0; s < KS; ++s)
#pragma unroll
      for (int q = 0; q < kG; ++q) {
        float4 bw[TN];
#pragma unroll
        for (int u = 0; u < TN; ++u) bw[u] = m32s_lds[((s * kG + q) * TN + u) * 64 + lane];
#pragma unroll
        for (int u = 0; u < TN; ++u)
          acc[u] = __builtin_amdgcn_mfma_f32_32x32x2f32(bw[u].x, a[s][q].x, acc[u], 0, 0, 0);
#pragma unroll
        for (int u = 0; u < TN; ++u)
          acc[u] = __builtin_amdgcn_mfma_f32_32x32x2f32(bw[u].y, a[s][q].y, acc[u], 0, 0, 0);
#pragma unroll
        for (int u = 0; u < TN; ++u)
          acc[u] = __builtin_amdgcn_mfma_f32_32x32x2f32(bw[u].z, a[s][q].z, acc[u], 0, 0, 0);
#pragma unroll
        for (int u = 0; u < TN; ++u)
          acc[u] = __builtin_amdgcn_mfma_f32_32x32x2f32(bw[u].w, a[s][q].w, acc[u], 0, 0, 0);
        a[s][q] = load(Tn, s, q);
      }
    const int64_t m = T * 32 + j;
    const int pm = m < p.M ? (int)m : -1;
    m32_epilogue_tm1<TN, ST, BB, EPI>(p, acc, pm, pm, nb, (int)T, ep, part, bb, lane);
  }
}

static int m32_ksplit(const ConvArgs& a, bool kxk, int64_t grid) {
  if (a.tconv || a.Cout % 4 || a.Cin % kBK || grid >= 256) return 1;
  const int Kt = kxk ? a.KH * a.KW * a.Cin : a.Cin + (a.x2 ? a.Cin2 : 0);
  const int S = (Kt + kBK - 1) / kBK;
  int ks = (int)std::min<int64_t>(8, (512 + grid - 1) / grid);
  ks = std::min(ks, S / 4);
  return ks >= 2 ? ks : 1;
}
static int64_t m32_ksplit_bytes(const ConvArgs& a, int ks) {
  return ks > 1 ? (int64_t)ks * a.B * a.OH * a.OW * a.ntiles32 * 32 * (int64_t)sizeof(float) : 0;
}
static int64_t m32_grid(const ConvArgs& a, int TM, int TN) {
  const int64_t BM = 4 * 32 * TM;
  const int64_t OHW = (int64_t)a.OH * a.OW;
  const int64_t mtiles = a.ascale ? cdiv(OHW, BM) * a.B : cdiv(a.M, BM);
  return mtiles * (a.ntiles32 / TN);
}

static bool m32_w8(const ConvArgs& a, int64_t grid) {
  static const bool off = env_digit("JABD_M32_W8") == 0;
  if (off || a.tconv || (a.ascale && a.Cin > kGateLds) || (a.x2 && a.x2_stride != 1))
    return false;
  static int ncu = 0;
  if (ncu <= 0) {
    int dev = 0;
    if (hipGetDevice(&dev) != hipSuccess ||
        hipDeviceGetAttribute(&ncu, hipDeviceAttributeMultiprocessorCount, dev) != hipSuccess)
      ncu = 0;
  }
  return grid < 2 * (int64_t)ncu;
}

template <int TM, int TN, bool KXK, bool AS>
static int launch_m32_as(const ConvArgs& a, int ks, hipStream_t st) {
  constexpr int BM = 4 * 32 * TM;
  const int64_t OHW = (int64_t)a.OH * a.OW;
  const int per_img = a.ascale != nullptr;
  const int64_t mt_img = cdiv(OHW, BM);
  if (KXK && a.tconv && a.stride == 2) {
    JABD_REQUIRE(!per_img, "conv32: phase mode without ascale");
    for (int ph = 0; ph < 2; ++ph)
      for (int pw = 0; pw < 2; ++pw) {
        const int64_t Mp = (int64_t)a.B * ((a.OH - ph + 1) / 2) * ((a.OW - pw + 1) / 2);
        if (Mp <= 0) continue;
        const int64_t grid = cdiv(Mp, BM) * (a.Ntiles / TN);
        JABD_REQUIRE(grid < (int64_t)0x7fffffff, "conv32: grid too large");
        conv1x1_m32_kernel<TM, TN, KXK, AS><<<(unsigned)grid, 256, 0, st>>>(a, (int)mt_img, 0,
                                                                        2 * ph + pw, 1, nullptr,
                                                                        BnEpi{});
        if (int e = check_launch("conv1x1_m32", 100 * TM + TN)) return e;
      }
    return JABD_OK;
  }
  const int64_t grid = m32_grid(a, TM, TN);
  JABD_REQUIRE(grid < (int64_t)0x7fffffff, "conv32: grid too large");
  if (ks > 1 && a.ws && a.ws_bytes >= m32_ksplit_bytes(a, ks)) {
    float* part = static_cast<float*>(a.ws);
    conv1x1_m32_kernel<TM, TN, KXK, AS><<<dim3((unsigned)grid, (unsigned)ks), 256, 0, st>>>(
        a, (int)mt_img, per_img, -1, ks, part, BnEpi{});
    if (int e = check_launch("conv1x1_m32 (split K)", 100 * TM + TN)) return e;
    const int64_t n4 = a.M * ((a.Cout + 3) / 4);
    m32_ksplit_reduce<<<(unsigned)cdiv(n4, 256), 256, 0, st>>>(a, ks, part);
    return check_launch("m32_ksplit_reduce");
  }
  if constexpr (TM == 1 && TN >= 5 && !KXK) {
    if (m32_w8(a, grid)) {
      if (a.x2)
        conv1x1_m32w8_kernel<TN, AS, true><<<(unsigned)grid, 512, 0, st>>>(a, (int)mt_img, per_img);
      else
        conv1x1_m32w8_kernel<TN, AS, false><<<(unsigned)grid, 512, 0, st>>>(a, (int)mt_img, per_img);
      return check_launch("conv1x1_m32", 100 * TM + TN);
    }
  }
  auto kern = conv1x1_m32_kernel<TM, TN, KXK, AS>;
  if constexpr (TM == 1 && !AS) {
    if (!a.bias && a.act == ACT_NONE)
      kern = a.res ? conv1x1_m32_kernel<1, TN, KXK, false, false, false, kEpiRes>
                   : conv1x1_m32_kernel<1, TN, KXK, false, false, false, kEpiNone>;
  }
  if constexpr (AS && !KXK) {
    if (a.Cin <= kGateLds && (!a.x2 || a.x2_stride == 1))
      kern = a.x2 ? conv1x1_m32_kernel<TM, TN, false, true, false, false, kEpiRt, kSrcTwo>
                  : conv1x1_m32_kernel<TM, TN, false, true, false, false, kEpiRt, kSrcOne>;
  }
  kern<<<(unsigned)grid, 256, 0, st>>>(a, (int)mt_img, per_img, -1, 1, nullptr, BnEpi{});
  return check_launch("conv1x1_m32", 100 * TM + TN);
}

template <int TM, int TN, bool KXK>
static int launch_m32(const ConvArgs& a, int ks, hipStream_t st) {
  if (a.ascale) return launch_m32_as<TM, TN, KXK, true>(a, ks, st);
  return launch_m32_as<TM, TN, KXK, false>(a, ks, st);
}

static bool m32s_on() {
  static const bool on = env_digit("JABD_M32S") != 0;
  return on;
}

template <int TN, int KS, bool ST, bool BB, int EPI>
static int launch_m32s(const ConvArgs& a, float* part, const BnEpi& bb, hipStream_t st) {
  auto kern = conv1x1_m32s_kernel<TN, KS, ST, BB, EPI>;
  const size_t lds = (size_t)KS * kG * TN * 64 * 16 + (size_t)4 * 32 * kEpiPitch * 4;
  static int slots = 0;
  if (slots <= 0) {
    int dev = 0, ncu = 0, occ = 0;
    JABD_HIP(hipGetDevice(&dev));
    JABD_HIP(hipDeviceGetAttribute(&ncu, hipDeviceAttributeMultiprocessorCount, dev));
    JABD_HIP(hipOccupancyMaxActiveBlocksPerMultiprocessor(&occ, kern, 256, lds));
    JABD_REQUIRE(occ >= 1, "conv32 stream: no resident workgroup (%zu B LDS)", lds);
    slots = ncu * occ;
  }
  const int nblk_n = a.Ntiles / TN;
  const int64_t ntiles = cdiv(a.M, (int64_t)32);
  int64_t gm = std::min<int64_t>(cdiv(ntiles, 4), slots / nblk_n);
  gm = std::max<int64_t>(8, gm / 8 * 8);
  kern<<<(unsigned)(gm * nblk_n), 256, lds, st>>>(a, nblk_n, part, bb);
  return check_launch("conv1x1_m32s", 100 * KS + TN);
}

bool m32s_pick(const ConvLayer& L, int form, int& TN, int& KS) {
  const ConvArgs& a = L.a;
  if (!m32s_on() || !L.is1x1 || a.tconv || a.nchw_in || a.x2 || a.ascale || a.y2 ||
      a.Cin % kBK || a.M >= ((int64_t)1 << 31) - 64)
    return false;
  KS = a.Cin / kBK;
  if (KS != 2 && KS != 4) return false;
  static const int ks4 = (int)env_int("JABD_M32S_KS4", 1);
  static const int ks2 = (int)env_int("JABD_M32S_KS2", 7);
  if (!(((KS == 4 ? ks4 : ks2) >> form) & 1)) return false;
  TN = a.tn32;
  while (KS * TN > 8 && TN % 2 == 0) TN /= 2;
  return TN >= 1 && KS * TN <= 8 && a.ntiles32 % TN == 0;
}

static int m32s_launch(const ConvArgs& a, int TN, int KS, int form, float* part, const BnEpi& bb,
                       hipStream_t st) {
  const bool plain_none = !a.bias && !a.res && a.act == ACT_NONE;
  const bool plain_res = !a.bias && a.res && a.act == ACT_NONE;
#define M32S(TN_, KS_)                                                                 \
  if (TN == TN_ && KS == KS_)                                                          \
  return form == 1   ? launch_m32s<TN_, KS_, true, false, kEpiNone>(a, part, bb, st)   \
         : form == 2 ? launch_m32s<TN_, KS_, false, true, kEpiNone>(a, part, bb, st)   \
         : plain_none ? launch_m32s<TN_, KS_, false, false, kEpiNone>(a, part, bb, st) \
         : plain_res  ? launch_m32s<TN_, KS_, false, false, kEpiRes>(a, part, bb, st)  \
                      : launch_m32s<TN_, KS_, false, false, kEpiRt>(a, part, bb, st);
  M32S(1, 2) M32S(2, 2) M32S(3, 2) M32S(4, 2) M32S(1, 4) M32S(2, 4)
#undef M32S
  return -1;
}

template <int TN, bool KXK>
static int launch_m32_stats(const ConvArgs& a, float* part, const BnEpi& bb, hipStream_t st) {
  const int64_t grid = cdiv(a.M, (int64_t)128) * (a.Ntiles / TN);
  JABD_REQUIRE(grid < (int64_t)0x7fffffff, "conv32 stats: grid too large");
  if (bb.rows) {
    conv1x1_m32_kernel<1, TN, KXK, false, false, true><<<(unsigned)grid, 256, 0, st>>>(
        a, (int)cdiv((int64_t)a.OH * a.OW, 128), 0, -1, 1, nullptr, bb);
    return check_launch("conv1x1_m32 (BN backward sums)", 100 + TN);
  }
  conv1x1_m32_kernel<1, TN, KXK, false, true><<<(unsigned)grid, 256, 0, st>>>(
      a, (int)cdiv((int64_t)a.OH * a.OW, 128), 0, -1, 1, part, BnEpi{});
  return check_launch("conv1x1_m32 (BN statistics)", 100 + TN);
}

int conv_m32_stats_dispatch(const ConvLayer& L, bool kxk, float* part, const BnEpi& bb,
                            hipStream_t st) {
  const ConvArgs a = L.view32();
  const int form = bb.rows ? 2 : 1;
  int tn, ks;
  if (!kxk && m32s_pick(L, form, tn, ks)) return m32s_launch(a, tn, ks, form, part, bb, st);
#define MS(TN_) return kxk ? launch_m32_stats<TN_, true>(a, part, bb, st) : launch_m32_stats<TN_, false>(a, part, bb, st);
  switch (a.tn32) {
    case 1: MS(1)
    case 2: MS(2)
    case 3: MS(3)
    case 4: MS(4)
    default: return -1;
  }
#undef MS
}

}

using namespace jabd;

static int m32_tm(const ConvArgs& a) {
  static const int ftm = (int)env_int("JABD_M32_TM", 0);
  if (a.tn32 > 4) return 1;
  if (ftm == 1 || ftm == 2) return ftm;
  return (!a.ascale || a.M < 65536) ? 1 : 2;
}

static int m32_tn_launch(const ConvArgs& a) {
  static const bool off = env_digit("JABD_M32_TN1") == 0;
  if (off || a.tn32 <= 1 || a.tconv || !a.ascale) return a.tn32;
  return m32_grid(a, m32_tm(a), a.tn32) >= 256 ? a.tn32 : 1;
}

namespace jabd {
bool m32_tile_pick(const ConvLayer& L, int& tm, int& tn, int& ks) {
  const ConvArgs& a = L.a;
  if (!L.w32(1, 7)) return false;
  if (L.is1x1 ? !L.fast1x1
              : !(L.v4out && !a.x2 && !a.y2 && L.kxk32() &&
                  (!a.tconv || a.stride == 1 || (a.stride == 2 && !a.ascale))))
    return false;
  tn = m32_tn_launch(a);
  tm = (tn == 1 && a.tn32 > 1) ? 1 : m32_tm(a);
  ks = m32_ksplit(a, !L.is1x1, m32_grid(a, tm, tn));
  return true;
}

int64_t conv_m32_ksplit_bytes(const ConvArgs& a, int ks) { return m32_ksplit_bytes(a, ks); }

int conv_m32s_launch(const ConvLayer& L, const ConvRoute& r, hipStream_t st) {
  return m32s_launch(L.view32(), r.tn, r.ks, 0, nullptr, BnEpi{}, st);
}

int conv_m32_tile_launch(const ConvLayer& L, const ConvRoute& r, hipStream_t st) {
  const ConvArgs a = L.view32();
  const bool kxk = !L.is1x1;
#define M32(TM_, TN_)             \
  if (r.tm == TM_ && r.tn == TN_) \
    return kxk ? launch_m32<TM_, TN_, true>(a, r.ks, st) : launch_m32<TM_, TN_, false>(a, r.ks, st);
  M32(1, 1) M32(1, 2) M32(1, 3) M32(1, 4) M32(2, 1) M32(2, 2) M32(2, 3) M32(2, 4)
  M32(1, 5) M32(1, 6) M32(1, 7)
#undef M32
  return -1;
}
}

extern "C" int jabd_conv_pack_tn32(int cout) {
  const int nt = (cout + 31) / 32;
  if (nt <= 4) return nt;
  if (nt % 4 == 0) return 4;
  int best = 4, waste = (nt + 3) / 4 * 4 - nt;
  for (int tn : {5, 6, 7}) {
    const int w = (nt + tn - 1) / tn * tn - nt;
    if (w < waste) { waste = w; best = tn; }
  }
  return best;
}

namespace jabd {

__device__ __forceinline__ float w2d_at(const float* __restrict__ w, int cout, int cin, int khw,
                                        int transposed, int k, int n) {
  const int cinp = transposed ? cout : cin;
  const int ncols = transposed ? cin : cout;
  if (k >= khw * cinp || n >= ncols) return 0.f;
  const int tap = k / cinp, c = k - tap * cinp;
  const int co = transposed ? c : n, ci = transposed ? n : c;
  return w[((int64_t)co * cin + ci) * khw + tap];
}

__device__ __forceinline__ void pack_store16(const float* __restrict__ w, int cout, int cin,
                                             int khw, int tr, int Ntiles, float* __restrict__ wp,
                                             int64_t i) {
  const int lane = (int)(i & 63);
  const int64_t r = i >> 6;
  const int nt = (int)(r % Ntiles), kc = (int)(r / Ntiles);
  const int g = lane >> 4, j = lane & 15;
  float4 v;
  v.x = w2d_at(w, cout, cin, khw, tr, 16 * kc + 4 * g + 0, 16 * nt + j);
  v.y = w2d_at(w, cout, cin, khw, tr, 16 * kc + 4 * g + 1, 16 * nt + j);
  v.z = w2d_at(w, cout, cin, khw, tr, 16 * kc + 4 * g + 2, 16 * nt + j);
  v.w = w2d_at(w, cout, cin, khw, tr, 16 * kc + 4 * g + 3, 16 * nt + j);
  reinterpret_cast<float4*>(wp)[i] = v;
}

__device__ __forceinline__ void pack_store32(const float* __restrict__ w, int cout, int cin,
                                             int khw, int tr, int NT32, float* __restrict__ wp32,
                                             int64_t i) {
  const int lane = (int)(i & 63);
  const int64_t r = i >> 6;
  const int nt = (int)(r % NT32), k8 = (int)(r / NT32);
  const int h = lane >> 5, j = lane & 31;
  float4 v;
  v.x = w2d_at(w, cout, cin, khw, tr, 8 * k8 + 4 * h + 0, 32 * nt + j);
  v.y = w2d_at(w, cout, cin, khw, tr, 8 * k8 + 4 * h + 1, 32 * nt + j);
  v.z = w2d_at(w, cout, cin, khw, tr, 8 * k8 + 4 * h + 2, 32 * nt + j);
  v.w = w2d_at(w, cout, cin, khw, tr, 8 * k8 + 4 * h + 3, 32 * nt + j);
  reinterpret_cast<float4*>(wp32)[i] = v;
}

__global__ __launch_bounds__(256) void pack_w_kernel(const float* __restrict__ w, int cout,
                                                     int cin, int khw, int transposed, int Kc,
                                                     int Ntiles, float* __restrict__ wp, int K8,
                                                     int NT32, float* __restrict__ wp32) {
  const int64_t i = blockIdx.x * (int64_t)blockDim.x + threadIdx.x;
  const int64_t n16 = (int64_t)Kc * Ntiles * 64;
  if (i < n16)
    pack_store16(w, cout, cin, khw, transposed, Ntiles, wp, i);
  else if (wp32 && i - n16 < (int64_t)K8 * NT32 * 64)
    pack_store32(w, cout, cin, khw, transposed, NT32, wp32, i - n16);
}

constexpr int kPackMaxJobs = 1024;
__global__ __launch_bounds__(256) void pack_w_multi_kernel(const int64_t* __restrict__ jobs,
                                                           const int64_t* __restrict__ starts,
                                                           int njobs, int64_t total) {
  __shared__ int64_t st[kPackMaxJobs + 1];
  for (int t = threadIdx.x; t <= njobs; t += blockDim.x) st[t] = starts[t];
  __syncthreads();
  const int64_t i = blockIdx.x * (int64_t)blockDim.x + threadIdx.x;
  if (i >= total) return;
  int lo = 0, hi = njobs - 1;
  while (lo < hi) {
    const int mid = (lo + hi + 1) >> 1;
    if (st[mid] <= i) lo = mid; else hi = mid - 1;
  }
  const int64_t* jb = jobs + (int64_t)lo * 11;
  const float* w = reinterpret_cast<const float*>(jb[0]);
  float* wp = reinterpret_cast<float*>(jb[1]);
  float* wp32 = reinterpret_cast<float*>(jb[2]);
  const int cout = (int)jb[3], cin = (int)jb[4], khw = (int)jb[5], tr = (int)jb[6];
  const int Kc = (int)jb[7], Ntiles = (int)jb[8], NT32 = (int)jb[10];
  const int64_t r0 = i - st[lo];
  const int64_t n16 = (int64_t)Kc * Ntiles * 64;
  if (r0 < n16)
    pack_store16(w, cout, cin, khw, tr, Ntiles, wp, r0);
  else
    pack_store32(w, cout, cin, khw, tr, NT32, wp32, r0 - n16);
}

}

extern "C" int jabd_conv_pack_multi_f32(const int64_t* jobs, const int64_t* starts,
                                        int32_t njobs, int64_t total, jabd_stream_t stream) {
  using namespace jabd;
  if (njobs <= 0 || total <= 0) return JABD_OK;
  JABD_REQUIRE(jobs && starts && njobs <= kPackMaxJobs, "conv_pack_multi: bad args (njobs %d)",
               njobs);
  pack_w_multi_kernel<<<(unsigned)cdiv(total, 256), 256, 0, as_stream(stream)>>>(jobs, starts,
                                                                                njobs, total);
  return check_launch("conv_pack_multi");
}

extern "C" int jabd_conv_pack_f32(const float* w, int32_t cout, int32_t cin, int32_t kh,
                                  int32_t kw, int32_t transposed, int32_t Kc, int32_t Ntiles,
                                  float* wp, int32_t K8, int32_t NT32, float* wp32,
                                  jabd_stream_t stream) {
  using namespace jabd;
  JABD_REQUIRE(w && wp && cout > 0 && cin > 0 && kh > 0 && kw > 0 && Kc > 0 && Ntiles > 0 &&
                   (!wp32 || (K8 > 0 && NT32 > 0)),
               "conv_pack: bad args");
  const int cinp = transposed ? cout : cin, ncols = transposed ? cin : cout;
  JABD_REQUIRE(16 * Kc >= kh * kw * cinp && 16 * Ntiles >= ncols &&
                   (!wp32 || (8 * K8 >= kh * kw * cinp && 32 * NT32 >= ncols)),
               "conv_pack: tile counts do not cover the weight");
  const int64_t tot = (int64_t)Kc * Ntiles * 64 + (wp32 ? (int64_t)K8 * NT32 * 64 : 0);
  pack_w_kernel<<<(unsigned)cdiv(tot, 256), 256, 0, as_stream(stream)>>>(
      w, cout, cin, kh * kw, transposed, Kc, Ntiles, wp, K8, NT32, wp32);
  return check_launch("conv_pack");
}
```

jabd-joint-attention-based-detector-for-small-face-detection_amd/csrc/head.hip:

```cpp
#include <stdlib.h>

#include <algorithm>

#include "common.h"
#include "conv_args.h"

namespace jabd {

constexpr int kSumThreads = 256;

__device__ __forceinline__ void channel_sum_body(const float* __restrict__ x, int64_t x_bs,
                                                 int x_ps, int64_t HW, int C, int64_t per_blk,
                                                 int64_t nblk, float* __restrict__ part,
                                                 float* red) {
  const int b = blockIdx.y;
  const int64_t p0 = blockIdx.x * per_blk;
  const int64_t p1 = min(p0 + per_blk, HW);
  const float* xb = x + (int64_t)b * x_bs;
  const int rows = kSumThreads / C > 0 ? kSumThreads / C : 1;
  for (int c0 = 0; c0 < C; c0 += kSumThreads) {
    const int c = c0 + (threadIdx.x % min(C, kSumThreads));
    const int r = threadIdx.x / min(C, kSumThreads);
    const int nrows = C >= kSumThreads ? 1 : rows;
    float s = 0.f;
    if (r < nrows && c < C) {
      float s4[4] = {0.f, 0.f, 0.f, 0.f};
      int64_t q = p0 + r;
      for (; q + 3 * nrows < p1; q += 4 * nrows) {
#pragma unroll
        for (int u = 0; u < 4; ++u) s4[u] += xb[(q + u * nrows) * x_ps + c];
      }
      for (; q < p1; q += nrows) s4[0] += xb[q * x_ps + c];
      s = (s4[0] + s4[1]) + (s4[2] + s4[3]);
    }
    __syncthreads();
    if (r < nrows && c < C) red[r * min(C, kSumThreads) + (c - c0)] = s;
    __syncthreads();
    if (threadIdx.x < min(C - c0, kSumThreads)) {
      float t = 0.f;
      for (int q = 0; q < nrows; ++q) t += red[q * min(C, kSumThreads) + threadIdx.x];
      part[((int64_t)b * nblk + blockIdx.x) * C + c0 + threadIdx.x] = t;
    }
    __syncthreads();
  }
}

__global__ __launch_bounds__(kSumThreads) void channel_sum_kernel(
    const float* __restrict__ x, int64_t x_bs, int x_ps, int64_t HW, int C, int64_t per_blk,
    int64_t nblk, float* __restrict__ part) {
  __shared__ float red[kSumThreads];
  channel_sum_body(x, x_bs, x_ps, HW, C, per_blk, nblk, part, red);
}

struct CsumMulti {
  const float* x[4];
  int64_t x_bs[4], HW[4], per[4], nblk[4];
  int x_ps[4], C[4];
  float* part[4];
};
__global__ __launch_bounds__(kSumThreads) void channel_sum_multi_kernel(const CsumMulti d) {
  __shared__ float red[kSumThreads];
  const int z = blockIdx.z;
  if (blockIdx.x >= d.nblk[z]) return;
  channel_sum_body(d.x[z], d.x_bs[z], d.x_ps[z], d.HW[z], d.C[z], d.per[z], d.nblk[z], d.part[z],
                   red);
}

__global__ __launch_bounds__(256) void eca_gate_kernel(const float* __restrict__ part,
                                                       int64_t nblk, int C, float inv_hw,
                                                       const float* __restrict__ w1d, int k,
                                                       int gate, float* __restrict__ scale,
                                                       float* __restrict__ mean_out) {
  __shared__ float mean[256];
  const int h = (k - 1) / 2;
  const int oc = blockDim.x - 2 * h;
  const int b = blockIdx.y, t = threadIdx.x;
  const int c = blockIdx.x * oc - h + t;
  float m = 0.f;
  if (c >= 0 && c < C) {
    const float* pb = part + (int64_t)b * nblk * C + c;
    float s0 = 0.f, s1 = 0.f, s2 = 0.f, s3 = 0.f;
    int64_t r = 0;
    for (; r + 3 < nblk; r += 4) {
      s0 += pb[r * C];
      s1 += pb[(r + 1) * C];
      s2 += pb[(r + 2) * C];
      s3 += pb[(r + 3) * C];
    }
    for (; r < nblk; ++r) s0 += pb[r * C];
    m = ((s0 + s1) + (s2 + s3)) * inv_hw;
  }
  mean[t] = m;
  __syncthreads();
  if (t >= h && t < h + oc && c < C) {
    float y = 0.f;
    for (int q = 0; q < k; ++q) y = fmaf(w1d[q], mean[t - h + q], y);
    const float g = gate == ACT_SIGMOID ? 1.f / (1.f + expf(-y))
                                        : fminf(fmaxf(y + 3.f, 0.f), 6.f) * (1.f / 6.f);
    scale[(int64_t)b * C + c] = g;
    if (mean_out) mean_out[(int64_t)b * C + c] = m;
  }
}

constexpr int kGateOC = 248;
__device__ __forceinline__ void eca_gate4_body(const float* __restrict__ part, int nblk, int C,
                                               float inv_hw, const float* __restrict__ w1d,
                                               int k, int gate, float* __restrict__ scale,
                                               float* __restrict__ mean_out, float4* red,
                                               float* mean) {
  const int b = blockIdx.y, t = threadIdx.x;
  const int cs = blockIdx.x * kGateOC;
  const int ce = min(C, cs + kGateOC);
  const int nq = (ce - cs + 8) >> 2;
  const int RG = 256 / nq;
  const int rg = t / nq, q = t - rg * nq;
  const int c = cs - 4 + 4 * q;
  float4 s = make_float4(0.f, 0.f, 0.f, 0.f);
  if (rg < RG && c >= 0 && c < C) {
    const float* pb = part + (int64_t)b * nblk * C + c;
    float4 a[8];
#pragma unroll
    for (int u = 0; u < 8; ++u) a[u] = make_float4(0.f, 0.f, 0.f, 0.f);
    int r = rg;
    for (; r + 7 * RG < nblk; r += 8 * RG) {
#pragma unroll
      for (int u = 0; u < 8; ++u) {
        const float4 v = *reinterpret_cast<const float4*>(pb + (int64_t)(r + u * RG) * C);
        a[u].x += v.x; a[u].y += v.y; a[u].z += v.z; a[u].w += v.w;
      }
    }
    for (; r < nblk; r += RG) {
      const float4 v = *reinterpret_cast<const float4*>(pb + (int64_t)r * C);
      a[0].x += v.x; a[0].y += v.y; a[0].z += v.z; a[0].w += v.w;
    }
#pragma unroll
    for (int u = 0; u < 8; ++u) {
      s.x += a[u].x; s.y += a[u].y; s.z += a[u].z; s.w += a[u].w;
    }
  }
  red[t] = s;
  __syncthreads();
  if (t < nq) {
    float4 m = make_float4(0.f, 0.f, 0.f, 0.f);
    for (int g = 0; g < RG; ++g) {
      const float4 v = red[g * nq + t];
      m.x += v.x; m.y += v.y; m.z += v.z; m.w += v.w;
    }
    const bool in = c >= 0 && c < C;
    mean[4 * t + 0] = in ? m.x * inv_hw : 0.f;
    mean[4 * t + 1] = in ? m.y * inv_hw : 0.f;
    mean[4 * t + 2] = in ? m.z * inv_hw : 0.f;
    mean[4 * t + 3] = in ? m.w * inv_hw : 0.f;
  }
  __syncthreads();
  const int h = (k - 1) / 2;
  const int co = cs + t;
  if (co < ce) {
    float y = 0.f;
    for (int j = 0; j < k; ++j) y = fmaf(w1d[j], mean[t + 4 - h + j], y);
    const float g = gate == ACT_SIGMOID ? 1.f / (1.f + expf(-y))
                                        : fminf(fmaxf(y + 3.f, 0.f), 6.f) * (1.f / 6.f);
    scale[(int64_t)b * C + co] = g;
    if (mean_out) mean_out[(int64_t)b * C + co] = mean[t + 4];
  }
}

__global__ __launch_bounds__(256) void eca_gate4_kernel(const float* __restrict__ part,
                                                        int nblk, int C, float inv_hw,
                                                        const float* __restrict__ w1d, int k,
                                                        int gate, float* __restrict__ scale,
                                                        float* __restrict__ mean_out) {
  __shared__ float4 red[256];
  __shared__ float mean[kGateOC + 8];
  eca_gate4_body(part, nblk, C, inv_hw, w1d, k, gate, scale, mean_out, red, mean);
}

struct GateMulti {
  const float* part[4];
  const float* w1d[4];
  float* scale[4];
  int nblk[4], C[4], k[4];
  float inv_hw[4];
  int gate;
};
__global__ __launch_bounds__(256) void eca_gate4_multi_kernel(const GateMulti d) {
  __shared__ float4 red[256];
  __shared__ float mean[kGateOC + 8];
  const int z = blockIdx.z;
  if ((int)blockIdx.x * kGateOC >= d.C[z]) return;
  eca_gate4_body(d.part[z], d.nblk[z], d.C[z], d.inv_hw[z], d.w1d[z], d.k[z], d.gate,
                 d.scale[z], nullptr, red, mean);
}

__global__ __launch_bounds__(256) void partial_reduce_kernel(const float* __restrict__ part,
                                                             int nblk, int C, int R,
                                                             float* __restrict__ out) {
  const int s = blockIdx.x, b = blockIdx.y, nsplit = gridDim.x;
  const int r0 = s * R, r1 = min(nblk, r0 + R);
  const float* pb = part + (int64_t)b * nblk * C;
  float* ob = out + ((int64_t)b * nsplit + s) * C;
  if ((C & 3) == 0) {
    const int C4 = C >> 2;
    for (int c4 = threadIdx.x; c4 < C4; c4 += blockDim.x) {
      float4 a = make_float4(0.f, 0.f, 0.f, 0.f);
      for (int r = r0; r < r1; ++r) {
        const float4 v = reinterpret_cast<const float4*>(pb + (int64_t)r * C)[c4];
        a.x += v.x; a.y += v.y; a.z += v.z; a.w += v.w;
      }
      reinterpret_cast<float4*>(ob)[c4] = a;
    }
  } else {
    for (int c = threadIdx.x; c < C; c += blockDim.x) {
      float a = 0.f;
      for (int r = r0; r < r1; ++r) a += pb[(int64_t)r * C + c];
      ob[c] = a;
    }
  }
}

__device__ __forceinline__ int nearest_src(int dst, int in, int out) {
  if (out == in) return dst;
  if (out == 2 * in) return dst >> 1;
  const float scale = (float)in / (float)out;
  const int s = (int)floorf((float)dst * scale);
  return s < in - 1 ? s : in - 1;
}

struct NlmSizes {
  int n;
  int v[8];
};

template <int CH>
__global__ __launch_bounds__(256) void nlm_kv_kernel(const float* __restrict__ src, int64_t src_bs,
                                                     int src_ps, int hsws, int C,
                                                     const float* __restrict__ wk,
                                                     const float* __restrict__ bk,
                                                     const float* __restrict__ wv,
                                                     const float* __restrict__ bv,
                                                     float* __restrict__ kv) {
  extern __shared__ float sw[];
  for (int t = threadIdx.x; t < CH * C; t += blockDim.x) {
    sw[t] = wk[t];
    sw[CH * C + t] = wv[t];
  }
  __syncthreads();
  const int b = blockIdx.y;
  const int pix = blockIdx.x * blockDim.x + threadIdx.x;
  if (pix >= hsws) return;
  const float* xp = src + (int64_t)b * src_bs + (int64_t)pix * src_ps;
  float o[2 * CH];
#pragma unroll
  for (int q = 0; q < CH; ++q) { o[q] = bk[q]; o[CH + q] = bv[q]; }
  for (int c = 0; c < C; c += 4) {
    const float4 x = *reinterpret_cast<const float4*>(xp + c);
#pragma unroll
    for (int q = 0; q < 2 * CH; ++q) {
      const float* w = sw + q * C + c;
      o[q] = fmaf(w[0], x.x, o[q]);
      o[q] = fmaf(w[1], x.y, o[q]);
      o[q] = fmaf(w[2], x.z, o[q]);
      o[q] = fmaf(w[3], x.w, o[q]);
    }
  }
  float* dst = kv + ((int64_t)b * hsws + pix) * (2 * CH);
#pragma unroll
  for (int q = 0; q < 2 * CH; ++q) dst[q] = o[q];
}

template <int CH>
__global__ __launch_bounds__(256) void nlm_pool_kernel(const float* __restrict__ kv, int hs, int ws,
                                                       int h, int w, const NlmSizes sizes, int S,
                                                       float* __restrict__ kpool,
                                                       float* __restrict__ vpool) {
  const int s = blockIdx.x, b = blockIdx.y;
  int base = 0, lvl = 0;
  for (; lvl < sizes.n; ++lvl) {
    const int n = sizes.v[lvl] * sizes.v[lvl];
    if (s < base + n) break;
    base += n;
  }
  const int sz = sizes.v[lvl];
  const int bi = (s - base) / sz, bj = (s - base) % sz;
  const int h0 = (bi * h) / sz, h1 = ((bi + 1) * h + sz - 1) / sz;
  const int w0 = (bj * w) / sz, w1 = ((bj + 1) * w + sz - 1) / sz;
  const int rw = w1 - w0;
  const int npix = (h1 - h0) * rw;
  const float* kb = kv + (int64_t)b * hs * ws * (2 * CH);
  float a[2 * CH];
#pragma unroll
  for (int q = 0; q < 2 * CH; ++q) a[q] = 0.f;
  for (int p = threadIdx.x; p < npix; p += blockDim.x) {
    const int i = h0 + p / rw, jx = w0 + p % rw;
    const float* v = kb + ((int64_t)nearest_src(i, hs, h) * ws + nearest_src(jx, ws, w)) * (2 * CH);
#pragma unroll
    for (int q = 0; q < 2 * CH; ++q) a[q] += v[q];
  }
#pragma unroll
  for (int q = 0; q < 2 * CH; ++q)
#pragma unroll
    for (int m = 32; m >= 1; m >>= 1) a[q] += __shfl_xor(a[q], m);
  __shared__ float red[4][2 * CH];
  const int lane = threadIdx.x & 63, wave = threadIdx.x >> 6;
  if (lane < 2 * CH) {
    float v = a[0];
#pragma unroll
    for (int q = 1; q < 2 * CH; ++q) v = lane == q ? a[q] : v;
    red[wave][lane] = v;
  }
  __syncthreads();
  if (threadIdx.x < 2 * CH) {
    const int q = threadIdx.x;
    const float t = (red[0][q] + red[1][q]) + (red[2][q] + red[3][q]);
    const float avg = t / (float)npix;
    if (q < CH) kpool[((int64_t)b * S + s) * CH + q] = avg;
    else vpool[((int64_t)b * S + s) * CH + (q - CH)] = avg;
  }
// ... 480 lines not shown
```

jabd-joint-attention-based-detector-for-small-face-detection_amd/jabd_amd/_lib.py:

```python
import ctypes
import os
import threading

import torch

_HERE = os.path.dirname(os.path.abspath(__file__))
LIB_PATH = os.environ.get("JABD_LIB") or os.path.join(_HERE, "libjabd.so")

c_i64 = ctypes.c_int64
c_int = ctypes.c_int
c_f32 = ctypes.c_float
c_f64 = ctypes.c_double
c_size = ctypes.c_size_t
c_vp = ctypes.c_void_p
c_sizep = ctypes.POINTER(ctypes.c_size_t)

c_i32 = ctypes.c_int32
c_fp = ctypes.POINTER(ctypes.c_float)


class ConvArgs(ctypes.Structure):
    _fields_ = [
        ("x", c_vp), ("x_bs", c_i64), ("x_ps", c_i32), ("x_c0", c_i32),
        ("B", c_i32), ("H", c_i32), ("W", c_i32), ("Cin", c_i32),
        ("x2", c_vp), ("x2_bs", c_i64), ("x2_ps", c_i32), ("Cin2", c_i32),
        ("x2_W", c_i32), ("x2_stride", c_i32),
        ("ascale", c_vp), ("ascale_bs", c_i64),
        ("w", c_vp), ("bias", c_vp),
        ("res", c_vp), ("res_bs", c_i64), ("res_ps", c_i32), ("res_c0", c_i32),
        ("y", c_vp), ("y_bs", c_i64), ("y_ps", c_i32), ("y_c0", c_i32),
        ("OH", c_i32), ("OW", c_i32), ("Cout", c_i32), ("Ntiles", c_i32), ("tn", c_i32),
        ("Kc", c_i32),
        ("KH", c_i32), ("KW", c_i32), ("stride", c_i32), ("pad", c_i32),
        ("act", c_i32), ("slope", c_f32),
        ("nchw_in", c_i32), ("tconv", c_i32),
        ("flags", c_i32), ("reserved1", c_i32),
        ("M", c_i64),
        ("w32", c_vp), ("ntiles32", c_i32), ("tn32", c_i32),
        ("y2", c_vp), ("y2_bs", c_i64), ("y2_ps", c_i32), ("y2_c0", c_i32), ("nsplit", c_i32),
        ("act2", c_i32), ("slope2", c_f32), ("reserved2", c_i32),
        ("ws", c_vp), ("ws_bytes", c_i64),
    ]


class DwArgs(ctypes.Structure):
    _fields_ = [
        ("x", c_vp), ("x_bs", c_i64), ("x_ps", c_i32), ("reserved0", c_i32),
        ("B", c_i32), ("H", c_i32), ("W", c_i32), ("C", c_i32),
        ("w", c_vp), ("bias", c_vp),
        ("y", c_vp), ("y_bs", c_i64), ("y_ps", c_i32), ("reserved1", c_i32),
        ("OH", c_i32), ("OW", c_i32), ("k", c_i32), ("stride", c_i32), ("pad", c_i32),
        ("act", c_i32),
        ("slope", c_f32), ("nblk", c_i32),
        ("part", c_vp),
    ]


class ExpDwArgs(ctypes.Structure):
    _fields_ = [
        ("x", c_vp), ("x_bs", c_i64), ("x_ps", c_i32), ("Cin", c_i32),
        ("B", c_i32), ("H", c_i32), ("W", c_i32), ("E", c_i32),
        ("we", c_vp), ("be", c_vp), ("Ntiles", c_i32), ("Kc", c_i32),
        ("wd", c_vp), ("bd", c_vp),
        ("k", c_i32), ("stride", c_i32), ("act", c_i32), ("nblk", c_i32),
        ("y", c_vp), ("y_bs", c_i64), ("y_ps", c_i32), ("OH", c_i32), ("OW", c_i32),
        ("reserved0", c_i32),
        ("part", c_vp),
        ("sw", c_vp), ("sb", c_vp), ("sy", c_vp), ("sy_bs", c_i64), ("sy_ps", c_i32),
        ("reserved1", c_i32),
        ("pw", c_vp), ("pb", c_vp), ("pg", c_vp), ("pres", c_vp), ("pg_bs", c_i32), ("pact", c_i32),
    ]


class WindowCopy(ctypes.Structure):
    _fields_ = [
        ("src", c_vp), ("dst", c_vp),
        ("s0", c_i32), ("s1", c_i32), ("s2", c_i32),
        ("d0", c_i32), ("d1", c_i32), ("d2", c_i32),
        ("off2", c_i32), ("fill", c_f32), ("scale", c_f32), ("reserved", c_i32),
    ]


WINDOW_MAX = 32


SIGNATURES = {
    "jabd_version": [],
    "jabd_abi_struct_size": [c_i32],
    "jabd_last_error": [ctypes.c_char_p, c_size],
    "jabd_launch_log_reset": [],
    "jabd_launch_log_count": [],
    "jabd_launch_log_name": [c_i32],
    "jabd_launch_log_tag": [c_i32],
    "jabd_decode_f32": [c_vp, c_vp, c_i64, c_i64, c_f32, c_f32, c_vp, c_vp],
    "jabd_decode_landm_f32": [c_vp, c_vp, c_i64, c_i64, c_f32, c_vp, c_vp],
    "jabd_nms_workspace_size": [c_i64, c_i64, c_sizep],
    "jabd_batched_nms_f32": [c_vp, c_i64, c_i64, c_vp, c_i64, c_i64, c_vp, c_i64, c_i64,
                             c_f64, c_f32, c_vp, c_vp, c_vp, c_size, c_vp],
    "jabd_batched_nms_ex_f32": [c_vp, c_i64, c_i64, c_vp, c_i64, c_i64, c_vp, c_i64, c_i64,
                                c_f64, c_f32, c_vp, c_vp, c_vp, c_size, c_vp,
                                c_i32, c_f64, c_i64],
    "jabd_nms_pair_stats": [c_vp, c_size, c_i64, c_i64, c_vp, c_vp, c_vp, c_vp],
    "jabd_sort_workspace_size": [c_i64, c_i32, c_sizep],
    "jabd_sort_u64": [c_vp, c_vp, c_vp, c_vp, c_i64, c_i32, c_i32, c_i32, c_vp, c_size, c_vp],
    "jabd_scan_workspace_size": [c_i64, c_sizep],
    "jabd_scan_excl_i32": [c_vp, c_vp, c_i64, c_vp, c_size, c_vp],
    "jabd_detect_workspace_size": [c_i64, c_i64, c_sizep],
    "jabd_detect_f32": [c_vp, c_vp, c_vp, c_vp, c_i64, c_i64, c_f32, c_f32, c_f32, c_f64,
                        c_vp, c_vp, c_vp, c_size, c_vp],
    "jabd_detect_ex_f32": [c_vp, c_vp, c_vp, c_vp, c_i64, c_i64, c_f32, c_f32, c_f32, c_f64,
                           c_vp, c_vp, c_vp, c_size, c_vp, c_i32, c_f64, c_i64],
    "jabd_match_workspace_size": [c_i64, c_i64, c_sizep],
    "jabd_match_encode_f32": [c_vp, c_vp, c_i64, c_i64, c_vp, c_i64, c_f32, c_f32, c_f32,
                              c_vp, c_vp, c_vp, c_vp, c_size, c_vp],
    "jabd_multibox_workspace_size": [c_i64, c_i64, c_sizep],
    "jabd_multibox_loss_fwd_f32": [c_vp, c_vp, c_vp, c_vp, c_vp, c_vp, c_i64, c_i64, c_int,
                                   c_vp, c_vp, c_vp, c_vp, c_size, c_vp],
    "jabd_multibox_loss_bwd_f32": [c_vp, c_vp, c_vp, c_vp, c_vp, c_vp, c_vp, c_i64, c_i64,
                                   c_vp, c_vp, c_vp, c_vp, c_vp, c_vp],
    "jabd_multibox_loss_finalize_f32": [c_vp, c_vp, c_vp, c_vp],
    "jabd_letterbox_f32": [c_vp, c_i64, c_int, c_int, c_vp, c_int, c_int, c_f32, c_vp, c_int,
                           c_vp],
    "jabd_correct_boxes_f32": [c_vp, c_i64, c_int, c_int, c_int, c_int, c_int, c_int, c_vp],
    "jabd_augment_workspace_size": [c_int, c_int, c_sizep],
    "jabd_augment_u8": [c_vp, c_int, c_int, c_int, c_int, c_int, c_int, c_int, c_int, c_int,
                        c_f64, c_f32, c_f32, c_vp, c_vp, c_size, c_vp],
    "jabd_wider_eval_workspace_size": [c_i64, c_i64, c_sizep],
    "jabd_wider_eval_f64": [c_vp, c_vp, c_vp, c_vp, c_vp, c_i64, c_i64, c_i64, c_f64, c_int,
                            c_vp, c_vp, c_size, c_vp],
    "jabd_upsample_bicubic_ac_f32": [c_vp, c_i64, c_int, c_int, c_int, c_vp, c_int, c_int, c_vp],
    "jabd_upsample_bicubic_ac_bwd_f32": [c_vp, c_i64, c_int, c_int, c_int, c_vp, c_int, c_int,
                                         c_vp],
    "jabd_nlm_attn_fwd_f32": [c_vp, c_vp, c_vp, c_i32, c_i32, c_i32, c_i32, c_vp, c_vp, c_vp],
    "jabd_nlm_attn_bwd_f32": [c_vp, c_vp, c_vp, c_vp, c_vp, c_vp, c_i32, c_i32, c_i32, c_i32,
                              c_vp, c_vp, c_vp, c_vp],
    "jabd_window_copy_multi_f32": [c_i32, ctypes.POINTER(WindowCopy), c_vp],
    "jabd_transpose_f32": [c_vp, c_i32, c_i32, c_vp, c_vp],
    "jabd_colsum_f32": [c_vp, c_i64, c_i32, c_vp, c_vp],
    "jabd_sum_multi_f32": [c_i32, ctypes.POINTER(c_vp), c_i64, c_vp, c_vp],
    "jabd_weighted_sum3_f32": [c_vp, c_vp, c_vp, c_f32, c_vp, c_vp],
    "jabd_conv_w2d_f32": [c_vp, c_i32, c_i32, c_i32, c_vp, c_vp],
    "jabd_heads_wpack_f32": [c_vp, c_vp, c_vp, c_vp, c_vp, c_vp, c_i32, c_i32, c_i32, c_i32,
                             c_vp, c_i32, c_vp, c_i32, c_vp],
    "jabd_nlm_attn_dkv_ws_floats": [c_i32, c_i32, c_i32, c_i32],
    "jabd_nlm_attn_dkv_f32": [c_vp, c_vp, c_vp, c_vp, c_i32, c_i32, c_i32, c_i32, c_vp, c_i64,
                              c_vp, c_vp, c_vp],
    "jabd_add3_f32": [c_vp, c_vp, c_vp, c_i64, c_vp, c_vp],
    "jabd_beca_ws_floats": [c_i64, c_i64, c_int],
    "jabd_conv_pack_multi_f32": [c_vp, c_vp, c_i32, c_i64, c_vp],
    "jabd_ssh_tail_weight_floats": [],
    "jabd_ssh_tail_heads_f32": [c_vp, c_i64, c_i32, c_vp, c_i64, c_i32, c_i32, c_i32, c_vp, c_f32,
                                c_i64, c_i64, c_i32, c_vp, c_vp, c_vp, c_vp],
    "jabd_conv_pack_f32": [c_vp, c_i32, c_i32, c_i32, c_i32, c_i32, c_i32, c_i32, c_vp, c_i32,
                           c_i32, c_vp, c_vp],
    "jabd_beca_fwd_f32": [c_vp, c_i64, c_i64, c_int, c_vp, c_int, c_vp, c_vp, c_vp, c_i64, c_vp],
    "jabd_beca_bwd_f32": [c_vp, c_vp, c_i64, c_i64, c_int, c_vp, c_int, c_vp, c_vp, c_vp, c_vp,
                          c_vp, c_i64, c_vp],
    "jabd_match_iou_f32": [c_vp, c_vp, c_i64, c_i64, c_vp, c_i64, c_f32, c_f32, c_f32,
                           c_vp, c_vp, c_vp, c_vp, c_size, c_vp],
    "jabd_multibox_diou_loss_fwd_f32": [c_vp, c_vp, c_vp, c_vp, c_vp, c_vp, c_vp, c_f32, c_f32,
                                        c_i64, c_i64, c_int, c_vp, c_vp, c_vp, c_vp, c_size,
                                        c_vp],
    "jabd_multibox_diou_loss_bwd_f32": [c_vp, c_vp, c_vp, c_vp, c_vp, c_vp, c_vp, c_f32, c_f32,
                                        c_vp, c_i64, c_i64, c_vp, c_vp, c_vp, c_vp, c_vp, c_vp],
    "jabd_multibox_iou_loss_fwd_f32": [c_vp, c_vp, c_vp, c_vp, c_vp, c_vp, c_vp, c_f32, c_f32,
                                       c_i64, c_i64, c_int, c_vp, c_vp, c_vp, c_vp, c_size,
                                       c_i32, c_vp],
    "jabd_multibox_iou_loss_bwd_f32": [c_vp, c_vp, c_vp, c_vp, c_vp, c_vp, c_vp, c_f32, c_f32,
                                       c_vp, c_i64, c_i64, c_vp, c_vp, c_vp, c_vp, c_vp, c_i32,
                                       c_vp],
    "jabd_iou_rows_fwd_f32": [c_vp, c_vp, c_vp, c_i64, c_f32, c_f32, c_i32, c_vp, c_vp],
    "jabd_iou_rows_bwd_f32": [c_vp, c_vp, c_vp, c_i64, c_f32, c_f32, c_i32, c_vp, c_vp, c_vp],
    "jabd_conv_pack_tn": [c_int],
    "jabd_conv_pack_tn32": [c_int],
    "jabd_conv2d_nhwc_f32": [ctypes.POINTER(ConvArgs), c_vp],
    "jabd_conv1x1_bn_stats_nblk": [ctypes.POINTER(ConvArgs)],
    "jabd_conv1x1_bn_stats_f32": [ctypes.POINTER(ConvArgs), c_vp, c_i64, c_vp, c_vp],
    "jabd_conv_workspace_size": [ctypes.POINTER(ConvArgs)],
    "jabd_conv_bn_stats_part_floats": [ctypes.POINTER(ConvArgs)],
    "jabd_conv_bn_bwd_part_floats": [ctypes.POINTER(ConvArgs)],
    "jabd_conv_bn_bwd_sums_f32": [ctypes.POINTER(ConvArgs), c_vp, c_i32, c_vp, c_vp, c_vp, c_vp,
                                  c_i32, c_f32, c_vp, c_i64, c_vp],
    "jabd_conv_bn_bwd_sums_res_f32": [ctypes.POINTER(ConvArgs), c_vp, c_i32, c_vp, c_i32, c_vp,
                                      c_vp, c_vp, c_i64, c_vp],
    "jabd_bn_act_bwd_rows_f32": [c_vp, c_vp, c_vp, c_i64, c_i32, c_vp, c_vp, c_vp, c_vp, c_i32,
                                 c_f32, c_vp, c_vp, c_vp, c_vp],
    "jabd_conv_bn_stats_f32": [ctypes.POINTER(ConvArgs), c_vp, c_i64, c_vp, c_vp, c_vp, c_vp,
                               c_f32, c_f32, c_vp],
    "jabd_stem_nchw_f32": [c_vp, c_i32, c_i32, c_i32, c_vp, c_vp, c_i32, c_vp, c_vp],
    "jabd_dw_nblk": [c_i64, c_i64, c_i64, c_i64],
    "jabd_dwconv_nhwc_f32": [ctypes.POINTER(DwArgs), c_vp],
    "jabd_dwconv_stats_nblk": [c_i64, c_i64, c_i64, c_i64],
    "jabd_dwconv_stats_f32": [ctypes.POINTER(DwArgs), c_vp, c_vp, c_vp],
    "jabd_dwconv_bnin_stats_f32": [ctypes.POINTER(DwArgs), c_vp, c_vp, c_vp, c_vp, c_i32, c_f32,
                                   c_vp, c_vp, c_vp],
    "jabd_bn_stats_final_f32": [c_vp, c_vp, c_i64, c_i64, c_i32, c_vp, c_vp, c_vp, c_vp, c_f32,
                                c_f32, c_vp],
    "jabd_expand_dw_nblk": [c_i32, c_i32, c_i32, c_i32],
    "jabd_expand_dw_nhwc_f32": [ctypes.POINTER(ExpDwArgs), c_vp],
    "jabd_expand_dw_select": [c_i32],
    "jabd_channel_sum_f32": [c_vp, c_i64, c_i32, c_i64, c_i64, c_i64, c_i64, c_vp, c_vp],
    "jabd_partial_reduce_f32": [c_vp, c_i64, c_i64, c_i64, c_i64, c_vp, c_vp],
    "jabd_eca_gate_f32": [c_vp, c_i64, c_i64, c_i64, c_i64, c_vp, c_i32, c_i32, c_vp, c_vp,
                          c_vp],
    "jabd_nlm_pool_f32": [c_vp, c_i64, c_i32, c_i32, c_i32, c_i32, c_i32, c_i32, c_i32, c_vp,
                          c_vp, c_vp, c_vp, c_i32, ctypes.POINTER(c_i32), c_i32, c_vp, c_vp,
                          c_vp, c_vp],
    "jabd_nlm_apply_f32": [c_vp, c_i64, c_i32, c_i32, c_i32, c_i32, c_i32, c_i32, c_i32, c_vp,
                           c_vp, c_vp, c_vp, c_i32, c_i32, c_vp, c_vp, c_vp, c_vp, c_vp, c_vp,
                           c_vp],
    "jabd_maxpool_nhwc_f32": [c_vp, c_i32, c_i32, c_i32, c_i32, c_i32, c_i32, c_i32, c_vp, c_vp],
    "jabd_heads_scatter_f32": [c_vp, c_i32, c_i64, c_i64, c_i64, c_i32, c_vp, c_vp, c_vp, c_vp],
    "jabd_heads_f32": [c_vp, c_i64, c_i32, c_i32, c_i32, c_i32, c_vp, c_vp, c_i64, c_i64, c_i32,
                       c_vp, c_vp, c_vp, c_vp],
    "jabd_bn_nblk": [c_i64, c_i32],
    "jabd_bn_stats_f32": [c_vp, c_i32, c_i64, c_i32, c_vp, c_vp, c_vp, c_vp, c_vp, c_f32, c_f32,
                          c_vp],
    "jabd_bn_act_fwd_f32": [c_vp, c_i32, c_i64, c_i32, c_vp, c_vp, c_vp, c_vp, c_vp, c_i32,
                            c_i32, c_f32, c_vp, c_i32, c_i32, c_vp],
    "jabd_bn_act_bwd_f32": [c_vp, c_i32, c_i32, c_vp, c_i32, c_vp, c_i32, c_i64, c_i32, c_vp,
                            c_vp, c_vp, c_vp, c_i32, c_f32, c_vp, c_vp, c_vp, c_vp, c_vp, c_vp],
    "jabd_conv_wgrad_part_floats": [ctypes.POINTER(ConvArgs)],
    "jabd_conv_wgrad_f32": [ctypes.POINTER(ConvArgs), c_vp, c_vp, c_vp],
    "jabd_eca_pool_gate_multi_f32": [c_i32, c_i64, c_vp, c_vp, c_vp, c_vp, c_vp, c_vp, c_vp, c_vp,
                                     c_vp, c_i32, c_vp, c_vp],
    "jabd_bn_sum_nblk": [c_i64, c_i32],
    "jabd_bn_act_fwd_sum_f32": [c_vp, c_i64, c_i32, c_vp, c_vp, c_vp, c_vp, c_i32, c_f32, c_vp,
                                c_i64, c_vp, c_vp],
    "jabd_conv_wgrad_eca_part_floats": [ctypes.POINTER(ConvArgs)],
    "jabd_conv_wgrad_eca_f32": [ctypes.POINTER(ConvArgs), c_vp, c_vp, c_vp, c_vp, c_vp, c_vp],
    "jabd_eca_gate_bwd_f32": [c_vp, c_i32, c_i64, c_i64, c_i32, c_vp, c_vp, c_vp, c_i32, c_i32,
                              c_vp, c_vp, c_vp, c_vp],
    "jabd_dw_dgrad_f32": [c_vp, c_vp, c_i32, c_i32, c_i32, c_i32, c_i32, c_i32, c_i32, c_i32,
                          c_i32, c_vp, c_vp],
    "jabd_dw_wgrad_part_floats": [c_i64, c_i32, c_i32],
    "jabd_dw_dgrad_bn_part_floats": [c_i32, c_i32, c_i32, c_i32],
    "jabd_dw_dgrad_bn_bwd_f32": [c_vp, c_vp, c_i32, c_i32, c_i32, c_i32, c_i32, c_i32, c_i32,
                                 c_i32, c_i32, c_vp, c_vp, c_vp, c_vp, c_vp, c_i32, c_f32, c_vp,
                                 c_vp, c_vp, c_vp, c_vp, c_vp],
    "jabd_dw_wgrad_f32": [c_vp, c_vp, c_i32, c_i32, c_i32, c_i32, c_i32, c_i32, c_i32, c_i32,
                          c_i32, c_vp, c_vp, c_vp],
    "jabd_dw_wgrad_bnin_f32": [c_vp, c_vp, c_i32, c_i32, c_i32, c_i32, c_i32, c_i32, c_i32,
                               c_i32, c_i32, c_vp, c_vp, c_vp, c_vp, c_i32, c_f32, c_vp, c_vp,
                               c_vp],
    "jabd_eca_bwd_f32": [c_vp, c_vp, c_i64, c_i64, c_i32, c_vp, c_vp, c_vp, c_i32, c_i32, c_vp,
                         c_i32, c_vp, c_vp, c_vp, c_vp, c_vp],
    "jabd_scale_bwd_f32": [c_vp, c_vp, c_i64, c_i64, c_i32, c_vp, c_vp, c_i32, c_vp, c_vp],
    "jabd_eca_bwd_terms_f32": [c_vp, c_vp, c_i64, c_i64, c_i32, c_vp, c_vp, c_vp, c_i32, c_i32,
                               c_vp, c_i32, c_vp, c_vp, c_vp, c_vp],
    "jabd_bn_act_bwd_ex_f32": [c_vp, c_i32, c_i32, c_vp, c_i32, c_vp, c_i32, c_i64, c_i32, c_vp,
                               c_vp, c_vp, c_vp, c_i32, c_f32, c_vp, c_vp, c_i64, c_vp, c_vp,
                               c_vp, c_vp, c_vp, c_vp],
    "jabd_heads_gather_f32": [c_vp, c_vp, c_vp, c_i32, c_i64, c_i64, c_i32, c_vp, c_vp],
    "jabd_nlm_bwd_attn_f32": [c_vp, c_i32, c_i32, c_i32, c_i32, c_vp, c_vp, c_vp, c_i32, c_vp,
                              c_vp, c_vp, c_vp, c_vp, c_vp, c_vp, c_vp],
    "jabd_nlm_bwd_proj_f32": [c_vp, c_vp, c_i32, c_i32, ctypes.POINTER(c_i32), c_i32, c_i32,
                              c_i32, c_i32, c_vp, c_vp, c_vp, c_vp, c_vp],
    "jabd_upsample_nearest_bwd_f32": [c_vp, c_i32, c_i32, c_i32, c_i32, c_i32, c_i32, c_i32,
                                      c_vp, c_vp],
    "jabd_upsample_nearest_f32": [c_vp, c_i32, c_i32, c_i32, c_i32, c_i32, c_i32, c_vp, c_vp],
    "jabd_maxpool_bwd_f32": [c_vp, c_vp, c_i32, c_i32, c_i32, c_i32, c_i32, c_i32, c_i32, c_vp,
                             c_vp],
    "jabd_maxpool_idx_nhwc_f32": [c_vp, c_i32, c_i32, c_i32, c_i32, c_i32, c_i32, c_i32, c_vp,
                                  c_vp, c_vp],
    "jabd_maxpool_bwd_idx_f32": [c_vp, c_vp, c_i32, c_i32, c_i32, c_i32, c_i32, c_i32, c_i32,
                                 c_vp, c_vp],
    "jabd_adam_num_chunks": [c_vp, c_i64],
    "jabd_adam_fill_chunks": [c_vp, c_i64, c_vp],
    "jabd_adam_step_f32": [c_vp, c_vp, c_i64, c_f64, c_f64, c_f64, c_f64, c_f64, c_f64, c_f64,
                           c_vp],
    "jabd_act_f32": [c_vp, c_i64, c_i32, c_f32, c_vp, c_vp],
    "jabd_act_bwd_f32": [c_vp, c_vp, c_i64, c_i32, c_f32, c_vp, c_vp],
    "jabd_bn_eval_f32": [c_vp, c_i64, c_i32, c_vp, c_vp, c_f32, c_vp, c_vp, c_i32, c_f32, c_vp,
                         c_vp],
    "jabd_channel_scale_f32": [c_vp, c_i64, c_i64, c_i32, c_vp, c_vp, c_vp],
    "jabd_adaptive_pool_ws_floats": [c_i32, c_i32, c_i32, ctypes.POINTER(c_i32), c_i32],
    "jabd_adaptive_pool_f32": [c_vp, c_i64, c_i32, c_i32, c_i32, c_i32, ctypes.POINTER(c_i32),
                               c_i32, c_vp, c_vp, c_i64, c_vp],
    "jabd_upsample_nearest_add_f32": [c_vp, c_i32, c_i32, c_i32, c_i32, c_i32, c_i32, c_vp, c_vp,
                                      c_vp],
    "jabd_adaptive_pool_bwd_f32": [c_vp, c_i32, c_i32, c_i32, c_i32, ctypes.POINTER(c_i32),
                                   c_i32, c_vp, c_vp],
}
_RESTYPE = {"jabd_version": ctypes.c_char_p, "jabd_dw_nblk": ctypes.c_int64,
            "jabd_launch_log_count": ctypes.c_int64, "jabd_launch_log_name": ctypes.c_char_p,
            "jabd_expand_dw_nblk": ctypes.c_int64,
            "jabd_bn_nblk": ctypes.c_int64, "jabd_conv_wgrad_part_floats": ctypes.c_int64,
            "jabd_conv_wgrad_eca_part_floats": ctypes.c_int64, "jabd_bn_sum_nblk": ctypes.c_int64,
            "jabd_dw_wgrad_part_floats": ctypes.c_int64,
            "jabd_dw_dgrad_bn_part_floats": ctypes.c_int64,
            "jabd_dwconv_stats_nblk": ctypes.c_int64,
            "jabd_conv1x1_bn_stats_nblk": ctypes.c_int64,
            "jabd_conv_bn_stats_part_floats": ctypes.c_int64,
            "jabd_conv_bn_bwd_part_floats": ctypes.c_int64,
            "jabd_adam_num_chunks": ctypes.c_int64, "jabd_beca_ws_floats": ctypes.c_int64,
            "jabd_adaptive_pool_ws_floats": ctypes.c_int64,
            "jabd_abi_struct_size": ctypes.c_int64, "jabd_conv_workspace_size": ctypes.c_int64,
            "jabd_ssh_tail_weight_floats": ctypes.c_int64,
            "jabd_nlm_attn_dkv_ws_floats": ctypes.c_int64}

_lock = threading.Lock()
_lib = None


def lib():
    global _lib
    if _lib is not None:
        return _lib
    with _lock:
        if _lib is None:
            if not os.path.exists(LIB_PATH):
                raise RuntimeError(
                    f"libjabd.so not built at {LIB_PATH}; run __graft_entry__.build() "
                    "(the HIP path has no CPU fallback)")
            h = ctypes.CDLL(LIB_PATH, mode=ctypes.RTLD_LOCAL)
            for name, args in SIGNATURES.items():
                fn = getattr(h, name)
                fn.argtypes = args
                fn.restype = _RESTYPE.get(name, ctypes.c_int)
            _lib = h
    return _lib


def last_error() -> str:
    buf = ctypes.create_string_buffer(512)
    lib().jabd_last_error(buf, 512)
    return buf.value.decode(errors="replace")


def call(name, *args):
    st = getattr(lib(), name)(*args)
# ... 20 lines not shown
```

jabd-joint-attention-based-detector-for-small-face-detection_amd/jabd_amd/engine.py:

```python
import os

import torch

from . import functional as F

NLM_SIZES_DEFAULT = (1, 4, 8, 12)
FUSE_EXPAND_DW = os.environ.get("JABD_FUSE_EXPAND_DW", "1") != "0"
FUSE_SKIP = os.environ.get("JABD_FUSE_SKIP", "1") != "0"
FUSE_PRE = os.environ.get("JABD_FUSE_PRE", "1") != "0"
EVAL_STREAMS = int(os.environ.get("JABD_EVAL_STREAMS", "1"))
EVAL_SPLIT_MIN = int(os.environ.get("JABD_EVAL_SPLIT_MIN", "8"))
CHUNK_ELEMS = (1 << 31) - 1
GATES_MULTI = os.environ.get("JABD_GATES_MULTI", "1") != "0"
HEADS_GEMM = os.environ.get("JABD_HEADS_GEMM", "1") != "0"
SSH_TAIL = os.environ.get("JABD_SSH_TAIL", "1") != "0"


def _w1d(eca):
    return eca.conv.weight.detach().reshape(-1).float().contiguous()


class SSHPack:

    def __init__(self, s):
# ... 154 lines not shown
    if wb.numel() != int(F.lib().jabd_ssh_tail_weight_floats()):
        raise RuntimeError("ssh_tail_pack: layout mismatch with libjabd")
    return wb


def heads_pack(m, i):
    convs = (m.BboxHead[i].conv1x1, m.ClassHead[i].conv1x1, m.LandmarkHead[i].conv1x1)
    w = torch.cat([c.weight.detach().float().reshape(c.weight.shape[0], -1) for c in convs])
    b = torch.cat([c.bias.detach().float() for c in convs])
    return w.contiguous(), b.contiguous()


class _Head:

    def __init__(self, m, eca_names, nlm_name, dev, gate="sigmoid"):
        self.gate = gate
        self.eca_in = [_w1d(getattr(m, n)) for n in eca_names]
        self.fpn = m.fpn._jabd_cached(dev, lambda: FPNPack(m.fpn, getattr(m.fpn, nlm_name)))
        self.eca_fpn = _w1d(m.eca_fpn)
        self.ssh = [s._jabd_cached(dev, lambda s=s: SSHPack(s)) for s in (m.ssh1, m.ssh2, m.ssh3)]
        self.heads = [heads_pack(m, i) for i in range(3)]
        self.tails = [ssh_tail_pack(s, self.heads[i]) if SSH_TAIL and p.split else None
                      for i, (s, p) in enumerate(zip((m.ssh1, m.ssh2, m.ssh3), self.ssh))]
        self.heads_gemm = [
            F.pack_conv_cat([(m.BboxHead[i].conv1x1, None, None), (m.ClassHead[i].conv1x1, None, None),
                             (m.LandmarkHead[i].conv1x1, None, None)])
            if HEADS_GEMM and m.BboxHead[i].conv1x1.in_channels >= 128 else None
            for i in range(3)]

    def _gate(self, f, w1d):
        if self.gate == "beca":
            from . import modules as M
            return M.beca_gate(f, w1d)
        return F.eca_gate(F.channel_sums(f), f.shape[1] * f.shape[2], w1d, "sigmoid")

    def _gates(self, fs, w1ds):
        if GATES_MULTI and self.gate == "sigmoid" and all(f.stride(3) == 1 for f in fs):
            sc = F.eca_gates_multi(list(fs), list(w1ds), "sigmoid")
            if sc is not None:
                return sc
        return [self._gate(f, w1d) for f, w1d in zip(fs, w1ds)]

    def forward(self, feats, softmax, out=None):
        B = feats[0].shape[0]
        scales = self._gates(feats, self.eca_in)
        levels = self.fpn.forward(feats, scales)
        A = sum(2 * o.shape[1] * o.shape[2] for o in levels)
        dev = levels[0].device
        if out is not None:
            loc, conf, landm = out
            if loc.shape[1] != A:
                raise RuntimeError(f"engine: anchor count {loc.shape[1]} != {A} of the levels")
        else:
            loc = torch.empty((B, A, 4), dtype=torch.float32, device=dev)
            conf = torch.empty((B, A, 2), dtype=torch.float32, device=dev)
            landm = torch.empty((B, A, 10), dtype=torch.float32, device=dev)
        a_off = 0
        scs = self._gates(levels, [self.eca_fpn] * len(levels))
        for i, o in enumerate(levels):
            _, h, w, C = o.shape
            if self.tails[i] is not None:
                c33, t = self.ssh[i].first(o, scs[i])
                F.ssh_tail_heads(c33, t, self.tails[i], self.ssh[i].leaky, loc, conf, landm,
                                 a_off, softmax)
                a_off += 2 * h * w
                continue
            feat = self.ssh[i].forward(o, scs[i])
            if self.heads_gemm[i] is not None:
                F.heads_scatter(F.conv(feat, self.heads_gemm[i]), loc, conf, landm, a_off, softmax)
            else:
                wt, bs = self.heads[i]
                F.heads(feat, wt, bs, loc, conf, landm, a_off, softmax)
            a_off += 2 * h * w
        return loc, conf, landm


class _MNv3Block:

    def __init__(self, blk):
        self.k, self.stride, self.act = blk.kernel_size, blk.stride, blk.act_name
        self.expand = F.pack_conv(blk.conv1, blk.bn1)
        self.dw_w, self.dw_b = F.pack_dw(blk.conv2, blk.bn2)
        self.gate = getattr(blk, "gate_kind", "eca")
        self.blk = blk
        if self.gate in ("eca", "beca"):
            self.eca = _w1d(blk.eca)
        sk = blk.skip
        self.skip_dw = None
        if sk is None:
            self.kind = "identity"
            self.project = F.pack_conv(blk.conv3, blk.bn3)
        elif blk.stride == 1:
            self.kind = "concat"
            s, t = F.bn_fold(sk[1])
            w2 = F.conv_weight_2d(sk[0].weight.detach().float()) * s[None, :]
            self.project = F.pack_conv(blk.conv3, blk.bn3, extra=(w2, t))
        elif len(sk) == 4:
            self.kind = "dw_concat"
            self.skip_dw = F.pack_dw(sk[0], sk[1])
            s, t = F.bn_fold(sk[3], sk[2].bias.detach().float())
            w2 = F.conv_weight_2d(sk[2].weight.detach().float()) * s[None, :]
            self.project = F.pack_conv(blk.conv3, blk.bn3, extra=(w2, t))
        else:
            self.kind = "dw_residual"
            self.skip_dw = F.pack_dw(sk[0], sk[1])
            self.project = F.pack_conv(blk.conv3, blk.bn3)

    def _scale(self, d, part):
        if self.gate == "eca":
            return F.eca_gate(part, d.shape[1] * d.shape[2], self.eca, "hsigmoid")
        from . import modules as M
        if self.gate == "se":
            return M.se_scale_eval(self.blk.se, d, self.blk)
        if self.gate == "beca":
            return M.beca_gate(d, self.eca)
        return None

    def can_defer(self):
        pk = self.project
        return (FUSE_PRE and FUSE_EXPAND_DW and self.gate == "eca" and self.kind == "identity" and
                pk.KH == 1 and pk.KW == 1 and pk.Cin == 16 and pk.Cout == 16 and not pk.Cin2 and
                pk.bias is not None)

    def takes_pre(self):
        return (FUSE_EXPAND_DW and FUSE_SKIP and self.stride == 2 and self.k == 3 and
                self.skip_dw is not None and self.kind in ("dw_concat", "dw_residual") and
                self.expand.Cin == 16 and self.expand.KH == 1 and not self.expand.Cin2)

    def front(self, x):
        d, part = F.expand_dw(x, self.expand, self.dw_w, self.dw_b, self.k, self.stride,
                              act=self.act, partials=True)
        return d, (self.project, self._scale(d, part), x, self.act)

    def forward(self, x, pre=None):
        t = None
        if pre is not None:
            d_prev, pspec = x, pre
            r = F.expand_dw(d_prev, self.expand, self.dw_w, self.dw_b, self.k, self.stride,
                            act=self.act, partials=self.gate == "eca", skip=self.skip_dw,
                            pre=pspec)
            d, part, t = r
        elif FUSE_EXPAND_DW:
            fuse_skip = FUSE_SKIP and self.skip_dw is not None and self.stride == 2
            r = F.expand_dw(x, self.expand, self.dw_w, self.dw_b, self.k, self.stride,
                            act=self.act, partials=self.gate == "eca",
                            skip=self.skip_dw if fuse_skip else None)
            d, part = r[0], r[1]
            if fuse_skip:
                t = r[2]
        else:
            e = F.conv(x, self.expand, act=self.act)
            d, part = F.dwconv(e, self.dw_w, self.dw_b, self.k, self.stride, act=self.act,
                               partials=self.gate == "eca")
        sc = self._scale(d, part)
        if self.kind == "identity":
            return F.conv(d, self.project, act=self.act, ascale=sc, res=x)
        if self.kind == "concat":
            return F.conv(d, self.project, act=self.act, ascale=sc, x2=x)
        if t is None:
            t, _ = F.dwconv(x, self.skip_dw[0], self.skip_dw[1], 3, 2)
        if self.kind == "dw_concat":
            return F.conv(d, self.project, act=self.act, ascale=sc, x2=t)
        return F.conv(d, self.project, act=self.act, ascale=sc, res=t)


class _R50Block:
    def __init__(self, blk):
        self.stride = blk.stride
        self.c1 = F.pack_conv(blk.conv1, blk.bn1)
        self.c2 = F.pack_conv(blk.conv2, blk.bn2)
        if blk.downsample is not None:
            s, t = F.bn_fold(blk.downsample[1])
            w2 = F.conv_weight_2d(blk.downsample[0].weight.detach().float()) * s[None, :]
            self.c3 = F.pack_conv(blk.conv3, blk.bn3, extra=(w2, t))
            self.down = True
        else:
            self.c3 = F.pack_conv(blk.conv3, blk.bn3)
            self.down = False

    def forward(self, x):
        t = F.conv(x, self.c1, act="relu")
        t = F.conv(t, self.c2, stride=self.stride, pad=1, act="relu")
        if self.down:
            return F.conv(t, self.c3, act="relu", x2=x, x2_stride=self.stride)
        return F.conv(t, self.c3, act="relu", res=x)


def mnv3_stages(body):
    if hasattr(body, "stages"):
        return body.stages()
    return [list(getattr(body, f"layer{i}")) for i in (1, 2, 3)]


class Engine:

    def __init__(self, model, kind, dev):
        m = model
        self.kind = kind
        if kind == "mnv3":
            s_, t_ = F.bn_fold(m.body.bn1)
            self.stem = ((F.conv_weight_2d(m.body.conv1.weight.detach().float())
                          * s_[None, :]).contiguous(), t_.detach().contiguous())
            self.layers = [[b._jabd_cached(dev, lambda b=b: _MNv3Block(b)) for b in stage]
                           for stage in mnv3_stages(m.body)]
            self.head = _Head(m, getattr(m, "eca_names", ("eca_40", "eca_80", "eca_160")), "nlm",
                              dev, gate=getattr(m, "head_gate", "sigmoid"))
            self.split_ok = (self.head.gate == "sigmoid" and
                             all(b.gate == "eca" for layer in self.layers for b in layer))
        else:
            self.stem = F.pack_conv(m.body.conv1, m.body.bn1)
            self.layers = [[b._jabd_cached(dev, lambda b=b: _R50Block(b))
                            for b in getattr(m.body, f"layer{i}")] for i in (1, 2, 3, 4)]
            self.head = _Head(m, ("eca_64", "eca_128", "eca_256"), "Nlm", dev)
            self.split_ok = False

    def run(self, x, softmax):
        B = x.shape[0]
        per_img = 16 * x.shape[2] * x.shape[3]
        chunk = max(1, CHUNK_ELEMS // per_img)
        if B > chunk:
            A = self.anchors(x.shape[2], x.shape[3])
            out = tuple(torch.empty((B, A, k), dtype=torch.float32, device=x.device)
                        for k in (4, 2, 10))
            for b0 in range(0, B, chunk):
                b1 = min(B, b0 + chunk)
                self._run(x[b0:b1], softmax, out=tuple(o[b0:b1] for o in out))
            return out
        n = min(EVAL_STREAMS, B) if B >= EVAL_SPLIT_MIN and self.split_ok else 1
        if n <= 1:
            return self._run(x, softmax)
        cur = torch.cuda.current_stream(x.device)
        if getattr(self, "_streams", None) is None or len(self._streams) < n:
            self._streams = [torch.cuda.Stream(device=x.device) for _ in range(n)]
        bounds = [B * i // n for i in range(n + 1)]
        with torch.no_grad():
            H, W = x.shape[2], x.shape[3]
            A = self.anchors(H, W)
            dev = x.device
            out = (torch.empty((B, A, 4), dtype=torch.float32, device=dev),
                   torch.empty((B, A, 2), dtype=torch.float32, device=dev),
                   torch.empty((B, A, 10), dtype=torch.float32, device=dev))
            for i in range(n):
                st = self._streams[i]
                st.wait_stream(cur)
                b0, b1 = bounds[i], bounds[i + 1]
                with torch.cuda.stream(st):
                    self._run(x[b0:b1], softmax, out=tuple(o[b0:b1] for o in out))
            for i in range(n):
                cur.wait_stream(self._streams[i])
        return out

    def anchors(self, H, W):
        def down(v, times):
            for _ in range(times):
                v = (v + 2 - 3) // 2 + 1
            return v
        if self.kind == "mnv3":
            sizes = [(down(H, t), down(W, t)) for t in (3, 4, 5)]
        else:
            h, w = (H + 6 - 7) // 2 + 1, (W + 6 - 7) // 2 + 1
            h, w = down(h, 1), down(w, 1)
            sizes = [(down(h, t), down(w, t)) for t in (1, 2, 3)]
        return sum(2 * a * b for a, b in sizes)

    def _run(self, x, softmax, out=None):
        with torch.no_grad():
            if self.kind == "mnv3":
                s = F.stem(x, self.stem[0], self.stem[1], "hswish")
                feats = []
                for layer in self.layers:
                    pre = None
                    for i, blk in enumerate(layer):
                        nxt = layer[i + 1] if i + 1 < len(layer) else None
                        if pre is None and nxt is not None and blk.can_defer() and \
                                nxt.takes_pre():
                            s, pre = blk.front(s)
                            continue
                        s = blk.forward(s, pre=pre)
                        pre = None
                    feats.append(s)
            else:
                s = F.conv(x, self.stem, stride=2, pad=3, act="relu", nchw_in=True)
                s = F.maxpool(s, 3, 2, 1)
                feats = []
                for li, layer in enumerate(self.layers):
                    for blk in layer:
                        s = blk.forward(s)
                    if li >= 1:
                        feats.append(s)
            return self.head.forward(feats, softmax=softmax, out=out)


def _check_input(x):
    if not isinstance(x, torch.Tensor) or not x.is_cuda or x.dtype != torch.float32:
        raise RuntimeError("RetinaFace.forward on the JABD HIP path needs a float32 GPU "
                           "tensor [B,3,H,W]; there is no CPU fallback")
    if x.dim() != 4 or x.shape[1] != 3:
        raise ValueError(f"expected input [B,3,H,W], got {tuple(x.shape)}")


def retinaface_forward(model, kind, x):
    _check_input(x)
    if model.training:
        from .train import train_forward
        return train_forward(model, kind, x)
    eng = model._jabd_cached(x.device, lambda: Engine(model, kind, x.device), tag="engine")
    return eng.run(x.contiguous(), softmax=(model.mode != "train"))
```

jabd-joint-attention-based-detector-for-small-face-detection_amd/jabd_amd/functional.py:

```python
import ctypes
import threading

import torch

from ._lib import ConvArgs, DwArgs, ExpDwArgs, call, lib

ACT = {"none": 0, "relu": 1, "leaky": 2, "hswish": 3, "hsigmoid": 4, "sigmoid": 5}

KINK_TAP = None

_KSPLIT = threading.local()


def ksplit_enabled():
    return getattr(_KSPLIT, "on", False)


class split_k:

    def __init__(self, enabled=True):
        self.enabled = enabled

    def __enter__(self):
        self.prev = ksplit_enabled()
        _KSPLIT.on = self.enabled
        return self

    def __exit__(self, *exc):
        _KSPLIT.on = self.prev


def tap(kind, *operands):
    if KINK_TAP is not None:
        KINK_TAP(kind, *operands)


def _stream():
    return ctypes.c_void_p(torch.cuda.current_stream().cuda_stream)


def _ptr(t):
    return t.data_ptr() if t is not None else None


def _check(name, t):
    if not t.is_cuda or t.dtype != torch.float32:
        raise RuntimeError(f"{name}: needs a float32 GPU tensor (no CPU fallback), got "
                           f"{t.dtype} on {t.device}")


class PackedConv:

    def __init__(self, w2d, bias, KH, KW, Cin, Cin2=0):
        K, cout = w2d.shape
        self.KH, self.KW, self.Cin, self.Cin2, self.Cout = KH, KW, Cin, Cin2, cout
        self.tn = int(lib().jabd_conv_pack_tn(cout))
        tiles = (cout + 15) // 16
        self.Ntiles = (tiles + self.tn - 1) // self.tn * self.tn
        self.Kc = (K + 15) // 16
        wp = torch.zeros((self.Kc * 16, self.Ntiles * 16), dtype=torch.float32, device=w2d.device)
        wp[:K, :cout] = w2d
        wp = wp.view(self.Kc, 4, 4, self.Ntiles, 16).permute(0, 3, 1, 4, 2).contiguous()
        self.w = wp
        self.bias = bias.contiguous().float() if bias is not None else None
        self.w32 = None
        if (KH == 1 and KW == 1) or (Cin % 32 == 0 and not Cin2):
            self._pack32(w2d)

    def _pack32(self, w2d):
        K, cout = w2d.shape
        self.tn32 = int(lib().jabd_conv_pack_tn32(cout))
        nt = (cout + 31) // 32
        self.ntiles32 = (nt + self.tn32 - 1) // self.tn32 * self.tn32
        k8 = (K + 31) // 32 * 4
        wp = torch.zeros((k8 * 8, self.ntiles32 * 32), dtype=torch.float32, device=w2d.device)
        wp[:K, :cout] = w2d
        self.w32 = wp.view(k8, 2, 4, self.ntiles32, 32).permute(0, 3, 1, 4, 2).contiguous()


def pack_weight_device(weight, transposed=False):
    w = weight.detach()
    if w.dtype != torch.float32 or not w.is_contiguous():
        w = w.float().contiguous()
    cout, cin, kh, kw = w.shape
    pcin, pcout = (cout, cin) if transposed else (cin, cout)
    pk = PackedConv.__new__(PackedConv)
    pk.KH, pk.KW, pk.Cin, pk.Cin2, pk.Cout = kh, kw, pcin, 0, pcout
    pk.tn = int(lib().jabd_conv_pack_tn(pcout))
    tiles = (pcout + 15) // 16
    pk.Ntiles = (tiles + pk.tn - 1) // pk.tn * pk.tn
    K = kh * kw * pcin
    pk.Kc = (K + 15) // 16
    pk.bias = None
    pk.w = torch.empty((pk.Kc, pk.Ntiles, 4, 16, 4), dtype=torch.float32, device=w.device)
    pk.w32 = None
    k8 = nt32 = 0
    if (kh == 1 and kw == 1) or pcin % 32 == 0:
        pk.tn32 = int(lib().jabd_conv_pack_tn32(pcout))
        nt = (pcout + 31) // 32
        pk.ntiles32 = (nt + pk.tn32 - 1) // pk.tn32 * pk.tn32
        k8 = (K + 31) // 32 * 4
        nt32 = pk.ntiles32
        pk.w32 = torch.empty((k8, nt32, 2, 32, 4), dtype=torch.float32, device=w.device)
    call("jabd_conv_pack_f32", w.data_ptr(), cout, cin, kh, kw, 1 if transposed else 0, pk.Kc,
         pk.Ntiles, pk.w.data_ptr(), k8, nt32, _ptr(pk.w32), _stream())
    return pk


def conv_weight_2d(weight):
    cout, cin, kh, kw = weight.shape
    return weight.permute(2, 3, 1, 0).reshape(kh * kw * cin, cout)


def bn_fold(bn, conv_bias=None):
    s = bn.weight / torch.sqrt(bn.running_var + bn.eps)
    t = bn.bias - bn.running_mean * s
    if conv_bias is not None:
        t = t + conv_bias * s
    return s, t


def pack_conv(conv, bn=None, extra=None, cin_pad=None, cout_pad=None):
    w2d, bias, kh, kw, cin, cin2 = _fold_conv(conv, bn, extra, cin_pad, cout_pad)
    return PackedConv(w2d, bias, kh, kw, cin, cin2)


def pack_conv_cat(parts, cin_pad=None):
    ws, bs = [], []
    for conv, bn, cout_pad in parts:
        w2d, bias, kh, kw, cin, _ = _fold_conv(conv, bn, None, cin_pad, cout_pad)
        ws.append(w2d)
        bs.append(bias if bias is not None else w2d.new_zeros(w2d.shape[1]))
    return PackedConv(torch.cat(ws, 1).contiguous(), torch.cat(bs).contiguous(), kh, kw, cin)


def _fold_conv(conv, bn, extra, cin_pad, cout_pad):
    wt = conv.weight.detach().float()
    cb = conv.bias.detach().float() if conv.bias is not None else None
    if bn is not None:
        s, t = bn_fold(bn, cb)
        wt = wt * s[:, None, None, None]
        bias = t
    else:
        bias = cb
    cout, cin = wt.shape[0], wt.shape[1]
    if cin_pad is not None and cin_pad > cin:
        wt = torch.cat([wt, wt.new_zeros((cout, cin_pad - cin) + tuple(wt.shape[2:]))], 1)
        cin = cin_pad
    if cout_pad is not None and cout_pad > cout:
        wt = torch.cat([wt, wt.new_zeros((cout_pad - cout,) + tuple(wt.shape[1:]))], 0)
        bias = torch.cat([bias if bias is not None else wt.new_zeros(cout),
                          wt.new_zeros(cout_pad - cout)])
    w2d = conv_weight_2d(wt)
    cin2 = 0
    if extra is not None:
        w2, t2 = extra
        cin2 = w2.shape[0]
        w2d = torch.cat([w2d, w2], 0)
        bias = t2 if bias is None else bias + t2
    kh, kw = conv.weight.shape[2], conv.weight.shape[3]
    return (w2d.detach(), bias.detach() if bias is not None else None, kh, kw, cin, cin2)


def pack_dw(conv, bn):
    c, _, k, _ = conv.weight.shape
    s, t = bn_fold(bn, conv.bias.detach().float() if conv.bias is not None else None)
    w = (conv.weight.detach().float().view(c, k * k) * s[:, None]).t().contiguous()
    return w, t.detach().contiguous()


_CONV_DBG = 0


def conv(x, pk, stride=1, pad=0, act="none", slope=0.0, ascale=None, x2=None, x2_stride=1,
         res=None, out=None, out_c0=0, nchw_in=False, x_c0=0, y2=None, y2_c0=0, nsplit=0,
         act2="none", slope2=0.0):
    _check("conv.x", x)
    if nchw_in:
        B, cin, H, W = x.shape
        x_bs, x_ps = cin * H * W, 1
    else:
        B, H, W, ctot = x.shape
        x_bs, x_ps = H * W * ctot, ctot
    OH = (H + 2 * pad - pk.KH) // stride + 1
    OW = (W + 2 * pad - pk.KW) // stride + 1
    if out is None:
        out = torch.empty((B, OH, OW, pk.Cout), dtype=torch.float32, device=x.device)
        out_c0 = 0
    a = ConvArgs()
    a.x, a.x_bs, a.x_ps, a.x_c0 = x.data_ptr(), x_bs, x_ps, x_c0
    a.B, a.H, a.W, a.Cin = B, H, W, pk.Cin
    if x2 is not None:
        a.x2, a.x2_bs, a.x2_ps, a.Cin2 = x2.data_ptr(), x2.stride(0), x2.shape[3], pk.Cin2
        a.x2_W, a.x2_stride = x2.shape[2], x2_stride
    if ascale is not None:
        a.ascale, a.ascale_bs = ascale.data_ptr(), ascale.shape[1]
    a.w = pk.w.data_ptr()
    a.bias = _ptr(pk.bias)
    if res is not None:
        a.res, a.res_bs, a.res_ps, a.res_c0 = res.data_ptr(), res.stride(0), res.shape[3], 0
    a.y, a.y_bs, a.y_ps, a.y_c0 = out.data_ptr(), out.stride(0), out.shape[3], out_c0
    a.OH, a.OW, a.Cout, a.Ntiles, a.tn, a.Kc = OH, OW, pk.Cout, pk.Ntiles, pk.tn, pk.Kc
    if pk.w32 is not None and not nchw_in:
        a.w32, a.ntiles32, a.tn32 = pk.w32.data_ptr(), pk.ntiles32, pk.tn32
    a.KH, a.KW, a.stride, a.pad = pk.KH, pk.KW, stride, pad
    a.act, a.slope = ACT[act], float(slope)
    a.nchw_in = 1 if nchw_in else 0
    a.reserved1 = _CONV_DBG
    ws = None
    if ksplit_enabled() and pk.w32 is not None and not nchw_in and y2 is None:
        nbytes = int(lib().jabd_conv_workspace_size(ctypes.byref(a)))
        if nbytes > 0:
            ws = torch.empty(nbytes // 4, dtype=torch.float32, device=x.device)
            a.ws, a.ws_bytes = ws.data_ptr(), nbytes
    if y2 is not None:
        _check("conv.y2", y2)
        a.y2, a.y2_bs, a.y2_ps, a.y2_c0 = y2.data_ptr(), y2.stride(0), y2.shape[3], y2_c0
        a.nsplit, a.act2, a.slope2 = nsplit, ACT[act2], float(slope2)
    call("jabd_conv2d_nhwc_f32", ctypes.byref(a), _stream())
    return out


def stem(x, w, bias, act):
    _check("stem.x", x)
    B, _, H, W = x.shape
    OH, OW = (H - 1) // 2 + 1, (W - 1) // 2 + 1
    y = torch.empty((B, OH, OW, 16), dtype=torch.float32, device=x.device)
    call("jabd_stem_nchw_f32", x.data_ptr(), B, H, W, w.data_ptr(), bias.data_ptr(), ACT[act],
         y.data_ptr(), _stream())
    return y


def dw_nblk(B, OH, OW, C):
    return int(lib().jabd_dw_nblk(B, OH, OW, C))


def dwconv(x, w, bias, k, stride, act="none", slope=0.0, partials=False):
    _check("dw.x", x)
    B, H, W, C = x.shape
    pad = k // 2
    OH = (H + 2 * pad - k) // stride + 1
    OW = (W + 2 * pad - k) // stride + 1
    y = torch.empty((B, OH, OW, C), dtype=torch.float32, device=x.device)
    part = None
    a = DwArgs()
    a.x, a.x_bs, a.x_ps = x.data_ptr(), x.stride(0), C
    a.B, a.H, a.W, a.C = B, H, W, C
    a.w, a.bias = w.data_ptr(), _ptr(bias)
    a.y, a.y_bs, a.y_ps = y.data_ptr(), y.stride(0), C
    a.OH, a.OW, a.k, a.stride, a.pad, a.act = OH, OW, k, stride, pad, ACT[act]
    a.slope = float(slope)
    if partials:
        nb = dw_nblk(B, OH, OW, C)
        part = torch.empty((B, nb, C), dtype=torch.float32, device=x.device)
        a.nblk, a.part = nb, part.data_ptr()
    call("jabd_dwconv_nhwc_f32", ctypes.byref(a), _stream())
    return y, part


def expand_dw(x, pk, w, bias, k, stride, act="none", partials=True, skip=None, pre=None):
    _check("expand_dw.x", x)
    B, H, W, C = x.shape
    if pk.KH != 1 or pk.KW != 1 or pk.Cin != C or pk.Cin2:
        raise ValueError("expand_dw: pk must be a plain 1x1 conv over all input channels")
    E = pk.Cout
    pad = k // 2
    OH = (H + 2 * pad - k) // stride + 1
    OW = (W + 2 * pad - k) // stride + 1
    y = torch.empty((B, OH, OW, E), dtype=torch.float32, device=x.device)
    a = ExpDwArgs()
    a.x, a.x_bs, a.x_ps, a.Cin = x.data_ptr(), x.stride(0), C, C
    a.B, a.H, a.W, a.E = B, H, W, E
    a.we, a.be, a.Ntiles, a.Kc = pk.w.data_ptr(), pk.bias.data_ptr(), pk.Ntiles, pk.Kc
    a.wd, a.bd = w.data_ptr(), bias.data_ptr()
    a.k, a.stride, a.act = k, stride, ACT[act]
    a.y, a.y_bs, a.y_ps, a.OH, a.OW = y.data_ptr(), y.stride(0), E, OH, OW
    part = None
    if partials:
        nb = int(lib().jabd_expand_dw_nblk(OH, OW, k, stride))
        part = torch.empty((B, nb, E), dtype=torch.float32, device=x.device)
        a.nblk, a.part = nb, part.data_ptr()
    t = None
    if skip is not None:
        t = torch.empty((B, OH, OW, C), dtype=torch.float32, device=x.device)
        a.sw, a.sb = skip[0].data_ptr(), skip[1].data_ptr()
        a.sy, a.sy_bs, a.sy_ps = t.data_ptr(), t.stride(0), C
    if pre is not None:
        ppk, pg, pres, pact = pre
        if (ppk.KH != 1 or ppk.KW != 1 or ppk.Cin != C or ppk.Cout != C or ppk.Cin2 or
                ppk.bias is None or ppk.Kc != 1 or ppk.Ntiles != 1):
            raise ValueError("expand_dw: pre must be a plain Cin -> Cin 1x1 conv with a bias")
        _check("expand_dw.pre.res", pres)
        if tuple(pres.shape) != tuple(x.shape) or pres.stride() != x.stride():
            raise ValueError("expand_dw: the pre residual must have x's shape and strides")
        if pg.shape != (B, C) or not pg.is_contiguous():
            raise ValueError("expand_dw: the pre gate must be a contiguous [B, Cin] tensor")
        a.pw, a.pb, a.pg, a.pres = ppk.w.data_ptr(), ppk.bias.data_ptr(), pg.data_ptr(), \
            pres.data_ptr()
        a.pg_bs, a.pact = pg.stride(0), ACT[pact]
    call("jabd_expand_dw_nhwc_f32", ctypes.byref(a), _stream())
    return (y, part, t) if skip is not None else (y, part)


_CSUM_PX = int(__import__("os").environ.get("JABD_CSUM_PX", "64"))


def channel_sums(x, nblk=None):
    B, H, W, C = x.shape
    HW = H * W
    if nblk is None:
        nblk = max(1, min(64, HW // _CSUM_PX))
    part = torch.empty((B, nblk, C), dtype=torch.float32, device=x.device)
    call("jabd_channel_sum_f32", x.data_ptr(), x.stride(0), C, B, HW, C, nblk, part.data_ptr(),
         _stream())
    return part


def dims3(shape):
    shape = tuple(shape)
    if len(shape) == 0:
        return (1, 1, 1)
    if len(shape) == 1:
        return (1, shape[0], 1)
    if len(shape) == 2:
        return (shape[0], shape[1], 1)
    n2 = 1
    for d in shape[2:]:
        n2 *= d
    return (shape[0], shape[1], n2)


def window_copies(items):
    from ._lib import WINDOW_MAX, WindowCopy
    for i in range(0, len(items), WINDOW_MAX):
        chunk = items[i:i + WINDOW_MAX]
        arr = (WindowCopy * len(chunk))()
        for d, it in zip(arr, chunk):
            src, dst, fill = it[:3]
            if not dst.is_contiguous() or (src is not None and not src.is_contiguous()):
                raise RuntimeError("window_copies: tensors must be contiguous")
            d.src = src.data_ptr() if src is not None else None
            d.dst = dst.data_ptr()
            d.s0, d.s1, d.s2 = dims3(src.shape) if src is not None else (0, 0, 0)
            d.d0, d.d1, d.d2 = dims3(dst.shape)
            d.off2 = int(it[3]) if len(it) > 3 else 0
            d.fill = float(fill)
            d.scale = float(it[4]) if len(it) > 4 else 1.0
        call("jabd_window_copy_multi_f32", len(chunk), arr, _stream())


def transpose(src, out=None):
    rows, cols = src.shape
    out = torch.empty((cols, rows), dtype=torch.float32, device=src.device) if out is None else out
    call("jabd_transpose_f32", src.data_ptr(), rows, cols, out.data_ptr(), _stream())
    return out


def channel_total(x):
    part = channel_sums(x)
    C = x.shape[3]
    out = torch.empty(C, dtype=torch.float32, device=x.device)
# ... 157 lines not shown
```

Before: 5082 images/sec.

## Fuse ECA gate computation from pool partials into project 1x1 conv prologue

The ECA attention gate (pool reduction, 1D conv over channels, sigmoid or hsigmoid) is now computed inside the m32 1x1 projection kernel. Each block reduces the depthwise pool partials into LDS instead of the gate coming from a separate eca_gate kernel launch plus a global scale buffer. This removes one kernel launch and a round trip per gated bottleneck block. In exchange every conv block redundantly re-reduces the partials for its image, and the prologue ordering changes. Unsupported shapes fall back to the separate gate kernel.

After: 5099 images/sec (median of 6 runs). No clear change (+0.3%).

```diff
diff --git a/include/jabd.h b/include/jabd.h
--- a/include/jabd.h
+++ b/include/jabd.h
@@ -231,6 +231,13 @@
   void* ws; int64_t ws_bytes;
 } jabd_conv_args;
 int64_t jabd_conv_workspace_size(const jabd_conv_args* args);
+typedef struct jabd_pool_gate {
+  const float* part; int64_t nblk; int64_t hw;
+  const float* w1d; int32_t k; int32_t gate;
+} jabd_pool_gate;
+int jabd_conv_pool_gate_served(const jabd_conv_args* args, const jabd_pool_gate* gate_src);
+int jabd_conv2d_pool_gate_nhwc_f32(const jabd_conv_args* args, const jabd_pool_gate* gate_src,
+                                   jabd_stream_t stream);
 int jabd_conv_pack_tn(int cout);
 int jabd_conv_pack_tn32(int cout);
 int jabd_conv_pack_f32(const float* w, int32_t cout, int32_t cin, int32_t kh, int32_t kw,
diff --git a/jabd-joint-attention-based-detector-for-small-face-detection_amd/csrc/abi.cpp b/jabd-joint-attention-based-detector-for-small-face-detection_amd/csrc/abi.cpp
--- a/jabd-joint-attention-based-detector-for-small-face-detection_amd/csrc/abi.cpp
+++ b/jabd-joint-attention-based-detector-for-small-face-detection_amd/csrc/abi.cpp
@@ -50,6 +50,7 @@
     case 1: return (int64_t)sizeof(jabd_dw_args);
     case 2: return (int64_t)sizeof(jabd_expdw_args);
     case 3: return (int64_t)sizeof(jabd_window_copy);
+    case 4: return (int64_t)sizeof(jabd_pool_gate);
     default: return -1;
   }
 }
diff --git a/jabd-joint-attention-based-detector-for-small-face-detection_amd/csrc/conv.hip b/jabd-joint-attention-based-detector-for-small-face-detection_amd/csrc/conv.hip
--- a/jabd-joint-attention-based-detector-for-small-face-detection_amd/csrc/conv.hip
+++ b/jabd-joint-attention-based-detector-for-small-face-detection_amd/csrc/conv.hip
@@ -680,7 +680,9 @@
 bool m32s_pick(const ConvLayer& L, int form, int& TN, int& KS);
 bool m32_tile_pick(const ConvLayer& L, int& tm, int& tn, int& ks);
 int conv_m32s_launch(const ConvLayer& L, const ConvRoute& r, hipStream_t st);
-int conv_m32_tile_launch(const ConvLayer& L, const ConvRoute& r, hipStream_t st);
+int conv_m32_tile_launch(const ConvLayer& L, const ConvRoute& r, hipStream_t st,
+                         const jabd_pool_gate* g = nullptr);
+bool conv_m32_pool_gate_serves(const ConvLayer& L, const ConvRoute& r, const jabd_pool_gate& g);
 int64_t conv_m32_ksplit_bytes(const ConvArgs& a, int ks);
 int conv_m32_stats_dispatch(const ConvLayer& L, bool kxk, float* part, const BnEpi& bb,
                             hipStream_t st);
@@ -986,6 +988,36 @@
   return JABD_EINVAL;
 }
 
+static int conv_pool_gate_setup(const jabd_conv_args* args, const jabd_pool_gate* g, ConvLayer& L) {
+  JABD_REQUIRE(args && g, "conv_pool_gate: null args");
+  JABD_REQUIRE(!args->ascale, "conv_pool_gate: ascale and a gate source are exclusive");
+  JABD_REQUIRE(g->part && g->w1d, "conv_pool_gate: null gate source");
+  jabd_conv_args v = *args;
+  v.ascale = g->part;
+  v.ascale_bs = v.Cin;
+  return conv_setup(&v, L);
+}
+
+extern "C" int jabd_conv_pool_gate_served(const jabd_conv_args* args,
+                                          const jabd_pool_gate* gate_src) {
+  ConvLayer L;
+  if (!args || !gate_src || args->ascale || !gate_src->part || !gate_src->w1d) return 0;
+  if (conv_pool_gate_setup(args, gate_src, L) != JABD_OK) return 0;
+  return conv_m32_pool_gate_serves(L, conv_route(L), *gate_src) ? 1 : 0;
+}
+
+extern "C" int jabd_conv2d_pool_gate_nhwc_f32(const jabd_conv_args* args,
+                                              const jabd_pool_gate* gate_src,
+                                              jabd_stream_t stream) {
+  ConvLayer L;
+  if (const int e = conv_pool_gate_setup(args, gate_src, L)) return e;
+  const ConvRoute r = conv_route(L);
+  JABD_REQUIRE(conv_m32_pool_gate_serves(L, r, *gate_src),
+               "conv_pool_gate: layer not served (jabd_conv_pool_gate_served)");
+  const int e = conv_m32_tile_launch(L, r, as_stream(stream), gate_src);
+  return e < 0 ? JABD_EINVAL : e;
+}
+
 namespace jabd {
 constexpr int kStemOut = 16;
 constexpr int kStemThreads = 128;
diff --git a/jabd-joint-attention-based-detector-for-small-face-detection_amd/csrc/conv32.hip b/jabd-joint-attention-based-detector-for-small-face-detection_amd/csrc/conv32.hip
--- a/jabd-joint-attention-based-detector-for-small-face-detection_amd/csrc/conv32.hip
+++ b/jabd-joint-attention-based-detector-for-small-face-detection_amd/csrc/conv32.hip
@@ -5,6 +5,7 @@
 
 #include "common.h"
 #include "conv_args.h"
+#include "eca_gate_shared.h"
 
 namespace jabd {
 
@@ -395,15 +396,28 @@
       for (int r = 0; r < 16; ++r) acc[t][u][r] = 0.f;
 
   float4 a_cur[TM][kG], a_nxt[TM][kG], b_nxt[NBT];
-  if (gate_lds) {
-    for (int i = threadIdx.x; i < p.Cin; i += 256) sGate[i] = sc[i];
+  if constexpr (FAST) {
+    load_a(0, a_cur);
+    load_b(0, b_nxt);
+    const PoolGate gs = pool_gate_of(bb);
+    if (gs.part)
+      pool_gate_to_lds(gs, p.Cin, img, threadIdx.x, sGate, sB_);
+    else
+      for (int i = threadIdx.x; i < p.Cin; i += 256) sGate[i] = sc[i];
     __syncthreads();
-  }
-  if (S > s_beg) {
-    load_a(s_beg, a_cur);
-    load_b(s_beg, b_nxt);
-    store_b(s_beg & 1, s_beg, b_nxt);
-    zero_tail(s_beg, a_cur);
+    store_b(0, 0, b_nxt);
+    zero_tail(0, a_cur);
+  } else {
+    if (gate_lds) {
+      for (int i = threadIdx.x; i < p.Cin; i += 256) sGate[i] = sc[i];
+      __syncthreads();
+    }
+    if (S > s_beg) {
+      load_a(s_beg, a_cur);
+      load_b(s_beg, b_nxt);
+      store_b(s_beg & 1, s_beg, b_nxt);
+      zero_tail(s_beg, a_cur);
+    }
   }
   __syncthreads();
   for (int s = s_beg; s < S; ++s) {
@@ -471,8 +485,12 @@
   if constexpr (TM == 1) {
     float* ep = reinterpret_cast<float*>(sB_) + wave * 32 * kEpiPitch;
     const int srow = mb * 4 + wave;
-    m32_epilogue_tm1<TN, ST, BB, (ST || BB) ? kEpiNone : EPI>(p, acc[0], pm[0], om[0], nb, srow,
-                                                                ep, part, bb, lane);
+    if constexpr (FAST)
+      m32_epilogue_tm1<TN, false, false, EPI>(p, acc[0], pm[0], om[0], nb, srow, ep, nullptr,
+                                              BnEpi{}, lane);
+    else
+      m32_epilogue_tm1<TN, ST, BB, (ST || BB) ? kEpiNone : EPI>(p, acc[0], pm[0], om[0], nb, srow,
+                                                                  ep, part, bb, lane);
     return;
   }
 #pragma unroll
@@ -536,7 +554,7 @@
 
 template <int TN, bool AS, bool X2>
 __global__ __launch_bounds__(512) void conv1x1_m32w8_kernel(const ConvArgs p, int mtiles_img,
-                                                            int per_img) {
+                                                            int per_img, const PoolGate gs) {
   constexpr int TNL = (TN + 1) / 2, TNH = TN - TNL;
   constexpr int NB4 = kG * TN * 64;
   constexpr int NBT = (NB4 + 511) / 512;
@@ -618,8 +636,12 @@
   load_a(0, a_cur);
   load_b(0, b_nxt);
   if constexpr (AS) {
-    const float* sc = p.ascale + (int64_t)img * p.ascale_bs;
-    for (int i = threadIdx.x; i < p.Cin; i += 512) sGate[i] = sc[i];
+    if (gs.part) {
+      pool_gate_to_lds(gs, p.Cin, img, threadIdx.x, sGate, sB_);
+    } else {
+      const float* sc = p.ascale + (int64_t)img * p.ascale_bs;
+      for (int i = threadIdx.x; i < p.Cin; i += 512) sGate[i] = sc[i];
+    }
     __syncthreads();
   }
   store_b(0, 0, b_nxt);
@@ -784,8 +806,14 @@
   return grid < 2 * (int64_t)ncu;
 }
 
+static int m32_gate_form(const ConvArgs& a, int TM, int TN, int ks, int64_t grid) {
+  if (!a.ascale || a.tconv || (ks > 1 && a.ws && a.ws_bytes >= m32_ksplit_bytes(a, ks))) return 0;
+  if (TM == 1 && TN >= 5 && m32_w8(a, grid)) return 2;
+  return (a.Cin <= kGateLds && (!a.x2 || a.x2_stride == 1)) ? 1 : 0;
+}
+
 template <int TM, int TN, bool KXK, bool AS>
-static int launch_m32_as(const ConvArgs& a, int ks, hipStream_t st) {
+static int launch_m32_as(const ConvArgs& a, int ks, const PoolGate& gs, hipStream_t st) {
   constexpr int BM = 4 * 32 * TM;
   const int64_t OHW = (int64_t)a.OH * a.OW;
   const int per_img = a.ascale != nullptr;
@@ -807,6 +835,17 @@
   }
   const int64_t grid = m32_grid(a, TM, TN);
   JABD_REQUIRE(grid < (int64_t)0x7fffffff, "conv32: grid too large");
+  if constexpr (AS && !KXK) {
+    if (m32_gate_form(a, TM, TN, ks, grid) == 1) {
+      auto gk = a.x2 ? conv1x1_m32_kernel<TM, TN, false, true, false, false, kEpiRt, kSrcTwo>
+                     : conv1x1_m32_kernel<TM, TN, false, true, false, false, kEpiRt, kSrcOne>;
+      gk<<<(unsigned)grid, 256, 0, st>>>(a, (int)mt_img, per_img, -1, 1, nullptr,
+                                         pool_gate_arg(gs));
+      return check_launch(gs.part ? "conv1x1_m32 (pool gate)" : "conv1x1_m32", 100 * TM + TN);
+    }
+  }
+  JABD_REQUIRE(!gs.part || m32_gate_form(a, TM, TN, ks, grid) == 2,
+               "conv32: this launch cannot take its gate from the pool partials");
   if (ks > 1 && a.ws && a.ws_bytes >= m32_ksplit_bytes(a, ks)) {
     float* part = static_cast<float*>(a.ws);
     conv1x1_m32_kernel<TM, TN, KXK, AS><<<dim3((unsigned)grid, (unsigned)ks), 256, 0, st>>>(
@@ -819,10 +858,12 @@
   if constexpr (TM == 1 && TN >= 5 && !KXK) {
     if (m32_w8(a, grid)) {
       if (a.x2)
-        conv1x1_m32w8_kernel<TN, AS, true><<<(unsigned)grid, 512, 0, st>>>(a, (int)mt_img, per_img);
+        conv1x1_m32w8_kernel<TN, AS, true><<<(unsigned)grid, 512, 0, st>>>(a, (int)mt_img, per_img,
+                                                                          gs);
       else
-        conv1x1_m32w8_kernel<TN, AS, false><<<(unsigned)grid, 512, 0, st>>>(a, (int)mt_img, per_img);
-      return check_launch("conv1x1_m32", 100 * TM + TN);
+        conv1x1_m32w8_kernel<TN, AS, false><<<(unsigned)grid, 512, 0, st>>>(a, (int)mt_img,
+                                                                           per_img, gs);
+      return check_launch(gs.part ? "conv1x1_m32 (pool gate)" : "conv1x1_m32", 100 * TM + TN);
     }
   }
   auto kern = conv1x1_m32_kernel<TM, TN, KXK, AS>;
@@ -831,19 +872,14 @@
       kern = a.res ? conv1x1_m32_kernel<1, TN, KXK, false, false, false, kEpiRes>
                    : conv1x1_m32_kernel<1, TN, KXK, false, false, false, kEpiNone>;
   }
-  if constexpr (AS && !KXK) {
-    if (a.Cin <= kGateLds && (!a.x2 || a.x2_stride == 1))
-      kern = a.x2 ? conv1x1_m32_kernel<TM, TN, false, true, false, false, kEpiRt, kSrcTwo>
-                  : conv1x1_m32_kernel<TM, TN, false, true, false, false, kEpiRt, kSrcOne>;
-  }
   kern<<<(unsigned)grid, 256, 0, st>>>(a, (int)mt_img, per_img, -1, 1, nullptr, BnEpi{});
   return check_launch("conv1x1_m32", 100 * TM + TN);
 }
 
 template <int TM, int TN, bool KXK>
-static int launch_m32(const ConvArgs& a, int ks, hipStream_t st) {
-  if (a.ascale) return launch_m32_as<TM, TN, KXK, true>(a, ks, st);
-  return launch_m32_as<TM, TN, KXK, false>(a, ks, st);
+static int launch_m32(const ConvArgs& a, int ks, const PoolGate& gs, hipStream_t st) {
+  if (a.ascale) return launch_m32_as<TM, TN, KXK, true>(a, ks, gs, st);
+  return launch_m32_as<TM, TN, KXK, false>(a, ks, gs, st);
 }
 
 static bool m32s_on() {
@@ -971,12 +1007,27 @@
   return m32s_launch(L.view32(), r.tn, r.ks, 0, nullptr, BnEpi{}, st);
 }
 
-int conv_m32_tile_launch(const ConvLayer& L, const ConvRoute& r, hipStream_t st) {
+bool conv_m32_pool_gate_serves(const ConvLayer& L, const ConvRoute& r, const jabd_pool_gate& g) {
+  static const bool off = env_digit("JABD_M32_POOL_GATE") == 0;
+  const ConvArgs& a = L.a;
+  if (off || r.family != kFamM32Tile || !L.is1x1 || !a.ascale || !g.part || !g.w1d) return false;
+  if (a.Cin % 4 || g.k < 1 || g.k > 9 || !(g.k & 1) || g.nblk < 1 || g.hw < 1 ||
+      g.nblk * a.Cin * 4 > 64 * 1024 || (g.gate != ACT_SIGMOID && g.gate != ACT_HSIGMOID) ||
+      (reinterpret_cast<uintptr_t>(g.part) & 15))
+    return false;
+  return m32_gate_form(a, r.tm, r.tn, r.ks, m32_grid(a, r.tm, r.tn)) != 0;
+}
+
+int conv_m32_tile_launch(const ConvLayer& L, const ConvRoute& r, hipStream_t st,
+                         const jabd_pool_gate* g) {
   const ConvArgs a = L.view32();
   const bool kxk = !L.is1x1;
-#define M32(TM_, TN_)             \
-  if (r.tm == TM_ && r.tn == TN_) \
-    return kxk ? launch_m32<TM_, TN_, true>(a, r.ks, st) : launch_m32<TM_, TN_, false>(a, r.ks, st);
+  PoolGate gs{};
+  if (g) gs = PoolGate{g->part, g->w1d, (int)g->nblk, g->k, g->gate, 1.f / (float)g->hw};
+#define M32(TM_, TN_)                                           \
+  if (r.tm == TM_ && r.tn == TN_)                               \
+    return kxk ? launch_m32<TM_, TN_, true>(a, r.ks, gs, st)    \
+               : launch_m32<TM_, TN_, false>(a, r.ks, gs, st);
   M32(1, 1) M32(1, 2) M32(1, 3) M32(1, 4) M32(2, 1) M32(2, 2) M32(2, 3) M32(2, 4)
   M32(1, 5) M32(1, 6) M32(1, 7)
 #undef M32
diff --git a/jabd-joint-attention-based-detector-for-small-face-detection_amd/csrc/eca_gate_shared.h b/jabd-joint-attention-based-detector-for-small-face-detection_amd/csrc/eca_gate_shared.h
--- /dev/null
+++ b/jabd-joint-attention-based-detector-for-small-face-detection_amd/csrc/eca_gate_shared.h
@@ -0,0 +1,191 @@
+#pragma once
+#include "common.h"
+#include "conv_args.h"
+
+namespace jabd {
+
+constexpr int kGateOC = 248;
+constexpr int kGateRed4 = 256;
+constexpr int kGateMeanF = kGateOC + 8;
+
+__device__ __forceinline__ void eca_gate4_window(const float* __restrict__ part, int nblk, int C,
+                                                 float inv_hw, const float* __restrict__ w1d,
+                                                 int k, int gate, float* __restrict__ scale,
+                                                 float* __restrict__ mean_out, int b, int ob,
+                                                 int win, int t, float4* red, float* mean) {
+  const int cs = win * kGateOC;
+  const int ce = min(C, cs + kGateOC);
+  const int nq = (ce - cs + 8) >> 2;
+  const int RG = 256 / nq;
+  const int rg = t / nq, q = t - rg * nq;
+  const int c = cs - 4 + 4 * q;
+  float4 s = make_float4(0.f, 0.f, 0.f, 0.f);
+  if (rg < RG && c >= 0 && c < C) {
+    const float* pb = part + (int64_t)b * nblk * C + c;
+    float4 a[8];
+#pragma unroll
+    for (int u = 0; u < 8; ++u) a[u] = make_float4(0.f, 0.f, 0.f, 0.f);
+    int r = rg;
+    for (; r + 7 * RG < nblk; r += 8 * RG) {
+#pragma unroll
+      for (int u = 0; u < 8; ++u) {
+        const float4 v = *reinterpret_cast<const float4*>(pb + (int64_t)(r + u * RG) * C);
+        a[u].x += v.x; a[u].y += v.y; a[u].z += v.z; a[u].w += v.w;
+      }
+    }
+    for (; r < nblk; r += RG) {
+      const float4 v = *reinterpret_cast<const float4*>(pb + (int64_t)r * C);
+      a[0].x += v.x; a[0].y += v.y; a[0].z += v.z; a[0].w += v.w;
+    }
+#pragma unroll
+    for (int u = 0; u < 8; ++u) {
+      s.x += a[u].x; s.y += a[u].y; s.z += a[u].z; s.w += a[u].w;
+    }
+  }
+  red[t] = s;
+  __syncthreads();
+  if (t < nq) {
+    float4 m = make_float4(0.f, 0.f, 0.f, 0.f);
+    for (int g = 0; g < RG; ++g) {
+      const float4 v = red[g * nq + t];
+      m.x += v.x; m.y += v.y; m.z += v.z; m.w += v.w;
+    }
+    const bool in = c >= 0 && c < C;
+    mean[4 * t + 0] = in ? m.x * inv_hw : 0.f;
+    mean[4 * t + 1] = in ? m.y * inv_hw : 0.f;
+    mean[4 * t + 2] = in ? m.z * inv_hw : 0.f;
+    mean[4 * t + 3] = in ? m.w * inv_hw : 0.f;
+  }
+  __syncthreads();
+  const int h = (k - 1) / 2;
+  const int co = cs + t;
+  if (co < ce) {
+    float y = 0.f;
+    for (int j = 0; j < k; ++j) y = fmaf(w1d[j], mean[t + 4 - h + j], y);
+    const float g = gate == ACT_SIGMOID ? 1.f / (1.f + expf(-y))
+                                        : fminf(fmaxf(y + 3.f, 0.f), 6.f) * (1.f / 6.f);
+    scale[(int64_t)ob * C + co] = g;
+    if (mean_out) mean_out[(int64_t)ob * C + co] = mean[t + 4];
+  }
+}
+
+struct GateWin {
+  int cs, ce, nq, RG, rg, q, c;
+};
+__device__ __forceinline__ GateWin gate4_win(int C, int win, int t) {
+  GateWin w;
+  w.cs = win * kGateOC;
+  w.ce = min(C, w.cs + kGateOC);
+  w.nq = (w.ce - w.cs + 8) >> 2;
+  w.RG = 256 / w.nq;
+  w.rg = t / w.nq;
+  w.q = t - w.rg * w.nq;
+  w.c = w.cs - 4 + 4 * w.q;
+  return w;
+}
+__device__ __forceinline__ float4 gate4_rows(const float* __restrict__ part, int nblk, int C, int b,
+                                             const GateWin w, bool on) {
+  const int RG = w.RG, rg = w.rg, c = w.c;
+  float4 s = make_float4(0.f, 0.f, 0.f, 0.f);
+  if (on && rg < RG && c >= 0 && c < C) {
+    const float* pb = part + (int64_t)b * nblk * C + c;
+    float4 a[8];
+#pragma unroll
+    for (int u = 0; u < 8; ++u) a[u] = make_float4(0.f, 0.f, 0.f, 0.f);
+    int r = rg;
+    for (; r + 7 * RG < nblk; r += 8 * RG) {
+#pragma unroll
+      for (int u = 0; u < 8; ++u) {
+        const float4 v = *reinterpret_cast<const float4*>(pb + (int64_t)(r + u * RG) * C);
+        a[u].x += v.x; a[u].y += v.y; a[u].z += v.z; a[u].w += v.w;
+      }
+    }
+    for (; r < nblk; r += 4 * RG) {
+      float4 v[4];
+#pragma unroll
+      for (int u = 0; u < 4; ++u)
+        v[u] = *reinterpret_cast<const float4*>(pb + (int64_t)min(r + u * RG, nblk - 1) * C);
+#pragma unroll
+      for (int u = 0; u < 4; ++u)
+        if (r + u * RG < nblk) {
+          a[0].x += v[u].x; a[0].y += v[u].y; a[0].z += v[u].z; a[0].w += v[u].w;
+        }
+    }
+#pragma unroll
+    for (int u = 0; u < 8; ++u) {
+      s.x += a[u].x; s.y += a[u].y; s.z += a[u].z; s.w += a[u].w;
+    }
+  }
+  return s;
+}
+__device__ __forceinline__ void gate4_means(const float4* red, float* mean, int C, float inv_hw,
+                                            const GateWin w, int t, bool on) {
+  const int nq = w.nq, RG = w.RG, c = w.c;
+  if (on && t < nq) {
+    float4 m = make_float4(0.f, 0.f, 0.f, 0.f);
+    for (int g = 0; g < RG; ++g) {
+      const float4 v = red[g * nq + t];
+      m.x += v.x; m.y += v.y; m.z += v.z; m.w += v.w;
+    }
+    const bool in = c >= 0 && c < C;
+    mean[4 * t + 0] = in ? m.x * inv_hw : 0.f;
+    mean[4 * t + 1] = in ? m.y * inv_hw : 0.f;
+    mean[4 * t + 2] = in ? m.z * inv_hw : 0.f;
+    mean[4 * t + 3] = in ? m.w * inv_hw : 0.f;
+  }
+}
+__device__ __forceinline__ void gate4_out(const float* mean, int C, const float* __restrict__ w1d,
+                                          int k, int gate, float* __restrict__ scale,
+                                          float* __restrict__ mean_out, int ob, const GateWin w,
+                                          int t, bool on) {
+  const int h = (k - 1) / 2;
+  const int co = w.cs + t;
+  if (on && co < w.ce) {
+    float y = 0.f;
+    for (int j = 0; j < k; ++j) y = fmaf(w1d[j], mean[t + 4 - h + j], y);
+    const float g = gate == ACT_SIGMOID ? 1.f / (1.f + expf(-y))
+                                        : fminf(fmaxf(y + 3.f, 0.f), 6.f) * (1.f / 6.f);
+    scale[(int64_t)ob * C + co] = g;
+    if (mean_out) mean_out[(int64_t)ob * C + co] = mean[t + 4];
+  }
+}
+
+struct PoolGate {
+  const float* part;
+  const float* w1d;
+  int nblk, k, gate;
+  float inv_hw;
+};
+
+inline BnEpi pool_gate_arg(const PoolGate& g) {
+  BnEpi e{};
+  e.x = g.part;
+  e.mean = g.w1d;
+  e.x_ps = g.nblk;
+  e.act = g.gate;
+  e.slope = g.inv_hw;
+  e.mask_ps = g.k;
+  return e;
+}
+__device__ __forceinline__ PoolGate pool_gate_of(const BnEpi& e) {
+  return PoolGate{e.x, e.mean, e.x_ps, e.mask_ps, e.act, e.slope};
+}
+
+constexpr int kGateWin4 = kGateRed4 + kGateMeanF / 4;
+__device__ __forceinline__ void pool_gate_to_lds(const PoolGate& gs, int Cin, int b, int t,
+                                                 float* sGate, float4* scratch) {
+  const bool on = t < 256;
+  float* mean = reinterpret_cast<float*>(scratch + kGateRed4);
+  const int nwin = (Cin + kGateOC - 1) / kGateOC;
+  for (int win = 0; win < nwin; ++win) {
+    const GateWin w = gate4_win(Cin, win, t);
+    const float4 s = gate4_rows(gs.part, gs.nblk, Cin, b, w, on);
+    if (on) scratch[t] = s;
+    __syncthreads();
+    gate4_means(scratch, mean, Cin, gs.inv_hw, w, t, on);
+    __syncthreads();
+    gate4_out(mean, Cin, gs.w1d, gs.k, gs.gate, sGate, nullptr, 0, w, t, on);
+  }
+}
+
+}
diff --git a/jabd-joint-attention-based-detector-for-small-face-detection_amd/csrc/head.hip b/jabd-joint-attention-based-detector-for-small-face-detection_amd/csrc/head.hip
--- a/jabd-joint-attention-based-detector-for-small-face-detection_amd/csrc/head.hip
+++ b/jabd-joint-attention-based-detector-for-small-face-detection_amd/csrc/head.hip
@@ -4,6 +4,7 @@
 
 #include "common.h"
 #include "conv_args.h"
+#include "eca_gate_shared.h"
 
 namespace jabd {
 
@@ -102,67 +103,13 @@
   }
 }
 
-constexpr int kGateOC = 248;
 __device__ __forceinline__ void eca_gate4_body(const float* __restrict__ part, int nblk, int C,
                                                float inv_hw, const float* __restrict__ w1d,
                                                int k, int gate, float* __restrict__ scale,
                                                float* __restrict__ mean_out, float4* red,
                                                float* mean) {
-  const int b = blockIdx.y, t = threadIdx.x;
-  const int cs = blockIdx.x * kGateOC;
-  const int ce = min(C, cs + kGateOC);
-  const int nq = (ce - cs + 8) >> 2;
-  const int RG = 256 / nq;
-  const int rg = t / nq, q = t - rg * nq;
-  const int c = cs - 4 + 4 * q;
-  float4 s = make_float4(0.f, 0.f, 0.f, 0.f);
-  if (rg < RG && c >= 0 && c < C) {
-    const float* pb = part + (int64_t)b * nblk * C + c;
-    float4 a[8];
-#pragma unroll
-    for (int u = 0; u < 8; ++u) a[u] = make_float4(0.f, 0.f, 0.f, 0.f);
-    int r = rg;
-    for (; r + 7 * RG < nblk; r += 8 * RG) {
-#pragma unroll
-      for (int u = 0; u < 8; ++u) {
-        const float4 v = *reinterpret_cast<const float4*>(pb + (int64_t)(r + u * RG) * C);
-        a[u].x += v.x; a[u].y += v.y; a[u].z += v.z; a[u].w += v.w;
-      }
-    }
-    for (; r < nblk; r += RG) {
-      const float4 v = *reinterpret_cast<const float4*>(pb + (int64_t)r * C);
-      a[0].x += v.x; a[0].y += v.y; a[0].z += v.z; a[0].w += v.w;
-    }
-#pragma unroll
-    for (int u = 0; u < 8; ++u) {
-      s.x += a[u].x; s.y += a[u].y; s.z += a[u].z; s.w += a[u].w;
-    }
-  }
-  red[t] = s;
-  __syncthreads();
-  if (t < nq) {
-    float4 m = make_float4(0.f, 0.f, 0.f, 0.f);
-    for (int g = 0; g < RG; ++g) {
-      const float4 v = red[g * nq + t];
-      m.x += v.x; m.y += v.y; m.z += v.z; m.w += v.w;
-    }
-    const bool in = c >= 0 && c < C;
-    mean[4 * t + 0] = in ? m.x * inv_hw : 0.f;
-    mean[4 * t + 1] = in ? m.y * inv_hw : 0.f;
-    mean[4 * t + 2] = in ? m.z * inv_hw : 0.f;
-    mean[4 * t + 3] = in ? m.w * inv_hw : 0.f;
-  }
-  __syncthreads();
-  const int h = (k - 1) / 2;
-  const int co = cs + t;
-  if (co < ce) {
-    float y = 0.f;
-    for (int j = 0; j < k; ++j) y = fmaf(w1d[j], mean[t + 4 - h + j], y);
-    const float g = gate == ACT_SIGMOID ? 1.f / (1.f + expf(-y))
-                                        : fminf(fmaxf(y + 3.f, 0.f), 6.f) * (1.f / 6.f);
-    scale[(int64_t)b * C + co] = g;
-    if (mean_out) mean_out[(int64_t)b * C + co] = mean[t + 4];
-  }
+  eca_gate4_window(part, nblk, C, inv_hw, w1d, k, gate, scale, mean_out, blockIdx.y, blockIdx.y,
+                   blockIdx.x, threadIdx.x, red, mean);
 }
 
 __global__ __launch_bounds__(256) void eca_gate4_kernel(const float* __restrict__ part,
diff --git a/jabd-joint-attention-based-detector-for-small-face-detection_amd/jabd_amd/_lib.py b/jabd-joint-attention-based-detector-for-small-face-detection_amd/jabd_amd/_lib.py
--- a/jabd-joint-attention-based-detector-for-small-face-detection_amd/jabd_amd/_lib.py
+++ b/jabd-joint-attention-based-detector-for-small-face-detection_amd/jabd_amd/_lib.py
@@ -80,6 +80,15 @@
         ("off2", c_i32), ("fill", c_f32), ("scale", c_f32), ("reserved", c_i32),
     ]
 
+
+class PoolGate(ctypes.Structure):
+    _fields_ = [
+        ("part", c_vp), ("nblk", c_i64), ("hw", c_i64),
+        ("w1d", c_vp), ("k", c_i32), ("gate", c_i32),
+    ]
+
+
+STRUCT_MIRRORS = (ConvArgs, DwArgs, ExpDwArgs, WindowCopy, PoolGate)
 
 WINDOW_MAX = 32
 
@@ -177,6 +186,8 @@
     "jabd_conv1x1_bn_stats_nblk": [ctypes.POINTER(ConvArgs)],
     "jabd_conv1x1_bn_stats_f32": [ctypes.POINTER(ConvArgs), c_vp, c_i64, c_vp, c_vp],
     "jabd_conv_workspace_size": [ctypes.POINTER(ConvArgs)],
+    "jabd_conv_pool_gate_served": [ctypes.POINTER(ConvArgs), ctypes.POINTER(PoolGate)],
+    "jabd_conv2d_pool_gate_nhwc_f32": [ctypes.POINTER(ConvArgs), ctypes.POINTER(PoolGate), c_vp],
     "jabd_conv_bn_stats_part_floats": [ctypes.POINTER(ConvArgs)],
     "jabd_conv_bn_bwd_part_floats": [ctypes.POINTER(ConvArgs)],
     "jabd_conv_bn_bwd_sums_f32": [ctypes.POINTER(ConvArgs), c_vp, c_i32, c_vp, c_vp, c_vp, c_vp,
diff --git a/jabd-joint-attention-based-detector-for-small-face-detection_amd/jabd_amd/engine.py b/jabd-joint-attention-based-detector-for-small-face-detection_amd/jabd_amd/engine.py
--- a/jabd-joint-attention-based-detector-for-small-face-detection_amd/jabd_amd/engine.py
+++ b/jabd-joint-attention-based-detector-for-small-face-detection_amd/jabd_amd/engine.py
@@ -330,16 +330,19 @@
             e = F.conv(x, self.expand, act=self.act)
             d, part = F.dwconv(e, self.dw_w, self.dw_b, self.k, self.stride, act=self.act,
                                partials=self.gate == "eca")
-        sc = self._scale(d, part)
+        if self.gate == "eca" and part is not None:
+            g = dict(pool=(part, d.shape[1] * d.shape[2], self.eca, "hsigmoid"))
+        else:
+            g = dict(ascale=self._scale(d, part))
         if self.kind == "identity":
-            return F.conv(d, self.project, act=self.act, ascale=sc, res=x)
+            return F.conv(d, self.project, act=self.act, res=x, **g)
         if self.kind == "concat":
-            return F.conv(d, self.project, act=self.act, ascale=sc, x2=x)
+            return F.conv(d, self.project, act=self.act, x2=x, **g)
         if t is None:
             t, _ = F.dwconv(x, self.skip_dw[0], self.skip_dw[1], 3, 2)
         if self.kind == "dw_concat":
-            return F.conv(d, self.project, act=self.act, ascale=sc, x2=t)
-        return F.conv(d, self.project, act=self.act, ascale=sc, res=t)
+            return F.conv(d, self.project, act=self.act, x2=t, **g)
+        return F.conv(d, self.project, act=self.act, res=t, **g)
 
 
 class _R50Block:
diff --git a/jabd-joint-attention-based-detector-for-small-face-detection_amd/jabd_amd/functional.py b/jabd-joint-attention-based-detector-for-small-face-detection_amd/jabd_amd/functional.py
--- a/jabd-joint-attention-based-detector-for-small-face-detection_amd/jabd_amd/functional.py
+++ b/jabd-joint-attention-based-detector-for-small-face-detection_amd/jabd_amd/functional.py
@@ -3,7 +3,7 @@
 
 import torch
 
-from ._lib import ConvArgs, DwArgs, ExpDwArgs, call, lib
+from ._lib import ConvArgs, DwArgs, ExpDwArgs, PoolGate, call, lib
 
 ACT = {"none": 0, "relu": 1, "leaky": 2, "hswish": 3, "hsigmoid": 4, "sigmoid": 5}
 
@@ -174,7 +174,7 @@
 
 def conv(x, pk, stride=1, pad=0, act="none", slope=0.0, ascale=None, x2=None, x2_stride=1,
          res=None, out=None, out_c0=0, nchw_in=False, x_c0=0, y2=None, y2_c0=0, nsplit=0,
-         act2="none", slope2=0.0):
+         act2="none", slope2=0.0, pool=None):
     _check("conv.x", x)
     if nchw_in:
         B, cin, H, W = x.shape
@@ -193,8 +193,6 @@
     if x2 is not None:
         a.x2, a.x2_bs, a.x2_ps, a.Cin2 = x2.data_ptr(), x2.stride(0), x2.shape[3], pk.Cin2
         a.x2_W, a.x2_stride = x2.shape[2], x2_stride
-    if ascale is not None:
-        a.ascale, a.ascale_bs = ascale.data_ptr(), ascale.shape[1]
     a.w = pk.w.data_ptr()
     a.bias = _ptr(pk.bias)
     if res is not None:
@@ -207,6 +205,23 @@
     a.act, a.slope = ACT[act], float(slope)
     a.nchw_in = 1 if nchw_in else 0
     a.reserved1 = _CONV_DBG
+    if pool is not None:
+        if ascale is not None:
+            raise ValueError("conv: ascale and pool are exclusive")
+        part, hw, w1d, gate = pool
+        g = PoolGate(part.data_ptr(), part.shape[1], hw, w1d.data_ptr(), w1d.numel(), ACT[gate])
+        served = y2 is None and part.is_contiguous() and part.shape[2] == pk.Cin and \
+            bool(lib().jabd_conv_pool_gate_served(ctypes.byref(a), ctypes.byref(g)))
+        if served and ksplit_enabled():
+            a.ascale, a.ascale_bs = part.data_ptr(), pk.Cin
+            served = int(lib().jabd_conv_workspace_size(ctypes.byref(a))) == 0
+            a.ascale, a.ascale_bs = None, 0
+        if served:
+            call("jabd_conv2d_pool_gate_nhwc_f32", ctypes.byref(a), ctypes.byref(g), _stream())
+            return out
+        ascale = eca_gate(part, hw, w1d, gate)
+    if ascale is not None:
+        a.ascale, a.ascale_bs = ascale.data_ptr(), ascale.shape[1]
     ws = None
     if ksplit_enabled() and pk.w32 is not None and not nchw_in and y2 is None:
         nbytes = int(lib().jabd_conv_workspace_size(ctypes.byref(a)))
```
